# google-research/semivl

Measured on AMD Instinct MI355X. Metric: train images/sec (512^2, ViT-B/16), higher is better.
Workload: dtype f32 (fp32 in / out / accumulate everywhere; the MFMA products as split 16-bit terms with fp32 accumulation: the ViT's linears, in_proj weight gradients and fused attention and the decoder's 3x3 convolutions (tiled: forward, input and weight gradient; dilated: forward, input gradient) on fp16 x 2 ope; 1 GPU; SemiVL step, pascal N=21, vlm-vlg-aspp-s2p4-sk04-ftap-mcvitb, 512x512, bs=16/GPU labeled + 16/GPU unlabeled (BASELINE configs[1]); global_batch=32, parallelism=dp1

## Files before the change

include/semivl_hip.h:

```cpp
#ifndef SEMIVL_HIP_H_
#define SEMIVL_HIP_H_

#include <stddef.h>
#include <stdint.h>

#ifdef __cplusplus
extern "C" {
#endif

typedef void* svl_stream_t;

typedef enum svl_status {
  SVL_OK = 0,
  SVL_ERR_INVALID_ARG = -1,
  SVL_ERR_LAUNCH = -2,
  SVL_ERR_UNSUPPORTED = -3
} svl_status;

int svl_version(void);
int svl_stream_release(svl_stream_t stream);
int svl_stream_prepare(svl_stream_t stream);
int svl_stream_helper(svl_stream_t stream, void** helper);
int svl_shutdown(void);
int svl_num_stream_contexts(void);
int svl_last_error(char* buf, size_t len);
int svl_clock_probe(unsigned long long* out, int n_waves, unsigned long long ticks_100mhz, svl_stream_t stream);

enum {
  SVL_A_KCONTIG = 0,
  SVL_A_MCONTIG = 1,
  SVL_A_CONV = 2,
  SVL_A_PATCH = 3
};
enum {
  SVL_B_KCONTIG = 0,
  SVL_B_NCONTIG = 1,
  SVL_B_CONVW = 2,
  SVL_B_NC_GELU = 3,
  SVL_B_NC_LN = 4,
  SVL_B_PATCHT = 5
};
enum {
  SVL_ACT_NONE = 0,
  SVL_ACT_GELU = 1,
  SVL_ACT_RELU = 2,
  SVL_ACT_MUL_DGELU = 3,
  SVL_ACT_MUL_DRELU = 4
};
enum {
  SVL_OUT_STRIDED = 0,
  SVL_OUT_CONVT2X = 1,
  SVL_OUT_PATCH = 2
};

typedef struct svl_operand {
  const float* ptr;
  int64_t ld;
  int64_t bs_outer;
  int64_t bs_inner;
} svl_operand;

typedef struct svl_conv_geom {
  int H, W;
  int Ho, Wo;
  int stride;
  int C1, C2;
  int rep;
  int KH, KW, dil, pad, sign;
  const float* src2;
  int64_t ld2;
  int patch;
} svl_conv_geom;

typedef struct svl_gemm_desc {
  int a_mode, b_mode;
  int M, N, K;
  int batch;
  int batch_inner;
  int ksplit;
  svl_operand A, B;
  svl_conv_geom conv;
  float* C;
  int out_mode;
  int64_t ldc_m, ldc_n, c_bs_outer, c_bs_inner;
  int ct_H, ct_W, ct_Cout;
  float alpha;
  const float* bias;
  int bias_mod;
  int act;
  float* preact;
  const float* resid;
  int64_t ldr_m, ldr_n, r_bs_outer, r_bs_inner;
  int accumulate;
  const void* conv_w_planes;
  void* emu_ws;
  const float* b_stats;
  const float* b_gamma;
  const float* b_beta;
  const unsigned* a_amax;
  const unsigned* b_amax;
} svl_gemm_desc;

int svl_gemm_f32(const svl_gemm_desc* d, svl_stream_t stream);

int svl_set_gemm_emulation(int mode);
int svl_get_gemm_emulation(void);
int svl_set_conv_tiled(int on);
int svl_last_gemm_path(void);
int64_t svl_absmax_launches(void);

typedef struct svl_pgemm_desc {
  const void* A;
  const void* B;
  int64_t a_rows, b_rows;
  int m_off, M, N, K;
  float* C;
  int64_t ldc;
  void* planes_out;
  int64_t p_rows;
  const float* bias;
  int act;
  float* preact;
  const float* resid;
  int64_t ldr;
  int accumulate;
  int fmt;
  int p_fmt;
  const int32_t* a_sexp;
  const int32_t* b_sexp;
  const float* a_rnorm;
  const float* b_bound;
  int32_t* p_sexp;
} svl_pgemm_desc;
int64_t svl_planes_rows(int64_t rows);
int64_t svl_planes_bytes(int64_t rows, int K);
int svl_split_planes_bf16x3(const float* x, int64_t ld, int64_t k_stride, int64_t rows, int K, void* planes,
                            int64_t planes_rows, int64_t row_off, svl_stream_t stream);
int64_t svl_planes_bytes_fmt(int64_t rows, int K, int fmt);
int svl_split_planes_f16x2(const float* x, int64_t ld, int64_t k_stride, int64_t rows, int K, void* planes,
                           int64_t planes_rows, int64_t row_off, int32_t* sexp, float* rnorm, unsigned* tensor_amax,
                           svl_stream_t stream);
int svl_gemm_planes_f32(const svl_pgemm_desc* d, svl_stream_t stream);
int svl_conv3x3_wgrad_tiled_groups(int imgs, int H, int W, int Ct, int Co);
int svl_conv3x3_wgrad_tiled(const float* dy, int64_t lddy, int Co, const float* src1, int64_t ld1, int C1,
                            const float* src2, int64_t ld2, int C2, int rep, int imgs, int H, int W, float* slabs,
                            int groups, const float* gn_in, svl_stream_t stream);

int svl_reduce_slabs_f32(float* out, const float* slabs, int nslab, int64_t count, int accumulate,
                         svl_stream_t stream);


int svl_softmax_max_f32(const float* logits, int B, int N, int64_t HW, float* conf, int64_t* label,
                        svl_stream_t stream);

int svl_cutmix_f32(float* out, const float* a, const float* b, const float* box, int B, int C, int64_t HW,
                   svl_stream_t stream);
int svl_cutmix_i64(int64_t* out, const int64_t* a, const int64_t* b, const float* box, int B, int64_t HW,
                   svl_stream_t stream);

typedef struct svl_ce_desc {
  const float* logits;
  int B, N;
  int64_t HW;
  const int64_t* target;
  int use_ignore_t;
  const float* conf;
  const int64_t* ign;
  float conf_thresh;
  int all_pixels;
  const int64_t* mc_target;
  float* partials;
  float* dlogits;
  const float* gscale;
  const float* img_weight;
} svl_ce_desc;
int64_t svl_ce_num_blocks(int B, int N, int64_t HW);
int svl_ce_fused_f32(const svl_ce_desc* d, svl_stream_t stream);
int svl_ce_finalize(const float* partials, int64_t nblocks, double* sums , svl_stream_t stream);

typedef struct svl_ce_up_desc {
  const float* logits;
  int B, N;
  int h, w, H, W;
  int align_corners;
  const int64_t* target;
  int use_ignore_t;
  const float* conf;
  const int64_t* ign;
  float conf_thresh;
  int all_pixels;
  const int64_t* mc_target;
  float* partials;
  float* dlogits;
  const float* gscale;
  const float* img_weight;
} svl_ce_up_desc;
int64_t svl_ce_up_num_blocks(int B, int N, int h, int w, int H, int W, int align_corners);
int svl_ce_up_fused_f32(const svl_ce_up_desc* d, svl_stream_t stream);
int svl_softmax_max_up_f32(const float* logits, int B, int N, int h, int w, int H, int W, int align_corners, float* conf,
                           int64_t* label, svl_stream_t stream);

int svl_semivl_gscale(const int64_t* counts, double numel_u, float lam, const double* factors, const int64_t* mc_counts,
                      float* gscale, svl_stream_t stream);
int svl_inv_count_f32(const int64_t* count, float* out, svl_stream_t stream);
int64_t svl_conf_avg_ws_doubles(int B);
int svl_conf_avg_factor(const float* conf, const int64_t* ign, int B, int64_t HW, double* factor, double* workspace,
                        svl_stream_t stream);
int svl_conf_ratio_f32(const float* conf, const int64_t* ign, int B, int64_t HW, float thresh, float* ratio,
                       double* workspace, svl_stream_t stream);
int svl_semivl_loss(const double* sums, double numel_u, float lam, const double* factors, const int64_t* mc_counts,
                    float* out, svl_stream_t stream);
int svl_softmax_planes_f32(const float* logits, int B, int N, int64_t HW, float* out, svl_stream_t stream);

int svl_target_prob_f32(const float* logits, int B, int N, int64_t HW, const int64_t* target, float* prob,
                        svl_stream_t stream);
int svl_target_prob_up_f32(const float* logits, int B, int N, int h, int w, int H, int W, int align_corners,
                           const int64_t* target, float* prob, svl_stream_t stream);
int64_t svl_ohem_ws_bytes(int64_t n);
int svl_ohem_threshold_f32(const float* prob, int64_t n, int64_t k, const int64_t* num_valid, int64_t min_kept,
                           float thresh, void* ws, float* threshold, svl_stream_t stream);
int svl_ohem_relabel_i64(const int64_t* target, const float* prob, int64_t n, const float* threshold, int64_t* out,
                         int64_t* count, svl_stream_t stream);

int svl_count_valid_i64(const int64_t* map, int64_t n, int64_t* count, svl_stream_t stream);

int svl_maskclip_labels(const float* dense, int B, int N, int h, int w, int H, int W, float scale,
                        float thresh, const int64_t* ign, int64_t* out, svl_stream_t stream);

int svl_concept_max_f32(const float* pred, int B, int NC, int64_t HW, const int* concept_offsets, int N,
                        float* out, svl_stream_t stream);

int svl_iou_hist_i64(const int64_t* pred, const int64_t* target, int64_t n, int K, int ignore_index, int64_t* hist,
                     svl_stream_t stream);


int svl_layernorm_fwd(const float* x, const float* gamma, const float* beta, float eps, int64_t rows, int C,
                      float* y, float* stats, svl_stream_t stream);
int svl_layernorm_fwd_planes(const float* x, const float* gamma, const float* beta, float eps, int64_t rows, int C,
                             float* y, float* stats, void* planes, int64_t planes_rows, svl_stream_t stream);
int svl_layernorm_fwd_planes_f16x2(const float* x, const float* gamma, const float* beta, float eps, int64_t rows, int C,
                                   float* y, float* stats, void* planes, int64_t planes_rows, int32_t* sexp, float* rnorm,
                                   svl_stream_t stream);
int svl_layernorm_fwd_pack_f16x2(const float* x, const float* gamma, const float* beta, float eps, int64_t rows, int C,
                                 float* y, float* stats, void* planes, int64_t planes_rows, int64_t row_off, int32_t* sexp,
                                 float* rnorm, int row_rnorm, unsigned* tensor_amax, svl_stream_t stream);
int svl_layernorm_bwd_pack_f16x2(const float* dy, const float* x, const float* stats, const float* gamma, int64_t rows, int C,
                                 const float* dx_add, float* dx, void* planes, int64_t planes_rows, int64_t row_off,
                                 int32_t* sexp, float* rnorm, unsigned* tensor_amax, svl_stream_t stream);
int svl_layernorm_bwd_parts(int64_t rows);
int svl_layernorm_bwd(const float* dy, const float* x, const float* stats, const float* gamma, int64_t rows,
                      int C, const float* dx_add, float* dx, float* dgamma_part, float* dbeta_part,
                      svl_stream_t stream);
int svl_softmax_rows_fwd(float* s, int64_t rows, int cols, int64_t ld, float scale, svl_stream_t stream);
int svl_softmax_rows_bwd(float* dp, const float* p, int64_t rows, int cols, int64_t ld, float scale,
                         svl_stream_t stream);

int svl_l2norm_fwd(const float* x, int64_t rows, int C, float eps, float* y, float* inv_norm, svl_stream_t stream);
int svl_l2norm_bwd(const float* dy, const float* y, const float* inv_norm, int64_t rows, int C, float* dx,
                   svl_stream_t stream);

int64_t svl_colsum_ws_floats(int64_t rows, int C);
int svl_colsum_f32(const float* x, int64_t rows, int C, int64_t ld, float* out, int accumulate, float* ws,
                   svl_stream_t stream);

int svl_eltwise_f32(int mode, const float* a, const float* b, float* out, int64_t n, svl_stream_t stream);
int svl_chanmask_f32(const float* x, const float* mask, float scale, int64_t rows, int rows_per_img, int C,
                     float* out, svl_stream_t stream);
int svl_fill_f32(float* p, float v, int64_t n, svl_stream_t stream);
int svl_bernoulli_f32(float* p, int64_t n, float keep_prob, uint64_t seed, uint64_t offset, svl_stream_t stream);
int svl_affine_planes_f32(const float* x, int64_t planes, int C, int64_t HW, const float* k4, float* y, svl_stream_t stream);
int svl_copy2d_f32(const float* src, int64_t sgrp, int64_t src_go, int64_t src_ld, float* dst, int64_t dgrp,
                   int64_t dst_go, int64_t dst_ld, int64_t rows, int C, int accumulate, svl_stream_t stream);
int svl_permute4_f32(const float* src, float* dst, int64_t n0, int64_t n1, int64_t n2, int64_t n3, int64_t s0, int64_t s1,
                     int64_t s2, int64_t s3, svl_stream_t stream);
int svl_bound2_f32(const float* rnorm, int64_t rows, const float* bias, int64_t nbias, float* out2, svl_stream_t stream);
int svl_permute_rows_f32(const float* src, int64_t outer, int A, int B, int C, float* dst, svl_stream_t stream);

int svl_groupnorm_fwd(const float* x, int64_t ldx, const float* gamma, const float* beta, float eps, int imgs,
                      int64_t HW, int C, int G, int relu, float* y, int64_t ldy, float* stats, svl_stream_t stream);
int64_t svl_conv3x3_gn_ws_doubles(int imgs, int H, int W, int N);
int svl_conv3x3_gn_f32(const float* src1, int64_t ld1, int C1, const float* src2, int64_t ld2, int C2, int rep,
                       const float* w, int imgs, int H, int W, int N, float* out, int64_t ldo, float eps, double* ws,
                       float* stats, const float* gn_in, const void* w_planes, svl_stream_t stream);
int64_t svl_conv3x3_weight_planes_bytes(int N, int Ct);
int svl_conv3x3_weight_planes(const float* w, int N, int Ct, void* planes, svl_stream_t stream);
int svl_groupnorm_scale_shift(const float* stats, const float* gamma, const float* beta, int imgs, int C, int G, float* scsh,
                              svl_stream_t stream);
int svl_groupnorm_apply(const float* x, int64_t ldx, const float* gamma, const float* beta, int imgs, int64_t HW, int C, int G,
                        int relu, const float* stats, float* y, int64_t ldy, svl_stream_t stream);
int svl_groupnorm_bwd(const float* dy, int64_t lddy, const float* x, int64_t ldx, const float* y, int64_t ldy,
                      const float* stats, const float* gamma, const float* beta, int imgs, int64_t HW, int C, int G,
                      int relu, float* dx, int64_t lddx, float* chan_sums, svl_stream_t stream);
int64_t svl_conv3x3_gnb_ws_doubles(int imgs, int H, int W, int N);
int svl_conv3x3_dgrad_gnb_f32(const float* dy, int64_t lddy, int C1, const float* w, int imgs, int H, int W, int N, float* out,
                              int64_t ldo, int accumulate, const float* gnb_x, const float* gnb_table, const float* gnb_stats,
                              double* ws, float* chan_sums, const void* w_planes, svl_stream_t stream);
int svl_groupnorm_bwd_apply(const float* dy, int64_t lddy, const float* x, int64_t ldx, const float* stats, const float* gamma,
                            const float* beta, int imgs, int64_t HW, int C, int G, int relu, const float* chan_sums, float* dx,
                            int64_t lddx, svl_stream_t stream);


int svl_attention_fwd(const float* qkv, int B, int T, int H, float* out, float* lse, void* out_planes,
                      int64_t planes_rows, svl_stream_t stream);
int svl_attention_bwd(const float* qkv, const float* out, const float* dout, const float* lse, int B, int T, int H,
                      float* dsum_ws, float* dqkv, void* dqkv_planes, int64_t planes_rows, svl_stream_t stream);
int64_t svl_attention_h2_ws_bytes(int B, int T, int H, int backward);
int svl_attention_h2_tr_sets(int on);
int svl_attention_bwd_h2_sets(const float* qkv, const float* out, const float* dout, const float* lse, int B, int T, int H,
                              float* dsum_ws, float* dqkv, const void* sets, int64_t sets_bytes, void* ws, int64_t ws_bytes,
                              svl_stream_t stream);
int svl_attention_fwd_h2(const float* qkv, int B, int T, int H, float* out, float* lse, void* out_planes,
                         int64_t planes_rows, void* ws, int64_t ws_bytes, svl_stream_t stream);
int svl_attention_bwd_h2(const float* qkv, const float* out, const float* dout, const float* lse, int B, int T, int H,
                         float* dsum_ws, float* dqkv, void* dqkv_planes, int64_t planes_rows, void* ws, int64_t ws_bytes,
                         svl_stream_t stream);

typedef struct svl_seqattn_desc {
  int groups, inner, seq, heads;
  int64_t outer_stride, inner_stride, seq_stride;
  const float* qkv;
  float* out;
  float* probs;
  const float* dout;
  float* dqkv;
  float* dscores;
} svl_seqattn_desc;
int svl_seqattn_fwd(const svl_seqattn_desc* d, svl_stream_t stream);
int svl_seqattn_bwd(const svl_seqattn_desc* d, svl_stream_t stream);

int svl_conv_cout1_fwd(const float* x, int64_t ldx, int imgs, int H, int W, int C, int KH, int KW, int dil, int pad,
                       const float* w, const float* bias, const float* gn_in, float* y, svl_stream_t stream);
int svl_conv_cout1_wgrad_blocks(int imgs, int H, int W);
int svl_conv_cout1_wgrad(const float* dy, const float* x, int64_t ldx, int imgs, int H, int W, int C, int dil, int pad,
                         const float* gn_in, float* slabs, svl_stream_t stream);
int svl_tap_gather(const float* T, int imgs, int H, int W, int KH, int KW, int dil, int pad, int sign, float* out,
                   svl_stream_t stream);

int svl_bilinear_nhwc_fwd(const float* x, int64_t ldx, int imgs, int h, int w, int C, int align_corners, int rep,
                          int H, int W, float* y, int64_t ldy, int accumulate, svl_stream_t stream);
int svl_sum_rep_f32(const float* src, int64_t ld, int64_t groups, int rep, int64_t rows, int C, float* out,
                    svl_stream_t stream);
int svl_bilinear_nhwc_bwd(const float* dy, int64_t lddy, int imgs, int h, int w, int C, int align_corners, int rep,
                          int H, int W, float* dx, int64_t lddx, int accumulate, svl_stream_t stream);
int svl_bilinear_planes_fwd(const float* x, int64_t planes, int h, int w, int align_corners, int H, int W, float* y,
                            svl_stream_t stream);
int svl_bilinear_planes_bwd(const float* dy, int64_t planes, int h, int w, int align_corners, int H, int W,
                            float* dx, svl_stream_t stream);
int svl_avgpool_cat_fwd(const float* x, int imgs, int H, int W, int C, int PH, int PW, const float* text, int Ct,
                        int nclass, float* y, svl_stream_t stream);
int svl_avgpool_cat_bwd(const float* dy, int imgs, int H, int W, int C, int PH, int PW, int Ct, float* dx,
                        int accumulate, svl_stream_t stream);
int svl_avgpool_cat_bwd_text(const float* dy, int imgs, int64_t HWp, int C, int Ct, int nclass, float* part, float* dtext,
                             svl_stream_t stream);

int svl_adamw_step(float* p, const float* g, float* m, float* v, const int64_t* seg_off, const float* seg_lr,
                   const float* seg_wd, int nseg, int64_t total, float beta1, float beta2, float eps, int step,
                   float gscale, float* ema, float ema_decay, svl_stream_t stream);
int svl_sgd_step(float* p, const float* g, float* m, const int64_t* seg_off, const float* seg_lr, const float* seg_wd,
                 int nseg, int64_t total, float momentum, float dampening, int nesterov, int step, float gscale,
                 float* ema, float ema_decay, svl_stream_t stream);

int64_t svl_bn_ws_doubles(int64_t rows, int C);
int svl_bn_stats(const float* x, int64_t ldx, int64_t rows, int C, double* sums, double* ws, svl_stream_t stream);
int svl_bn_finalize(const double* sums, double count, float eps, float momentum, float* running_mean, float* running_var,
                    int C, float* mean, float* invstd, svl_stream_t stream);
int svl_bn_eval_invstd(const float* running_var, float eps, int C, float* invstd, svl_stream_t stream);
int svl_bn_apply(const float* x, int64_t ldx, int64_t rows, int C, const float* mean, const float* invstd,
                 const float* gamma, const float* beta, const float* resid, int64_t ldr, int relu, float* y, int64_t ldy,
                 svl_stream_t stream);
int svl_bn_bwd_reduce(const float* dy, int64_t lddy, const float* x, int64_t ldx, const float* y, int64_t ldy,
                      const float* mean, const float* invstd, const float* remask_gamma, const float* remask_beta,
                      int64_t rows, int C, double* sums, double* ws, svl_stream_t stream);
int svl_bn_bwd_apply(const float* dy, int64_t lddy, const float* x, int64_t ldx, const float* y, int64_t ldy,
                     const float* mean, const float* invstd, const float* gamma, const float* remask_beta,
                     const double* sums, double count, int64_t rows, int C, float* dx, int64_t lddx, float* dres,
                     int64_t lddr, svl_stream_t stream);
int svl_maxpool3x3s2_fwd(const float* x, int imgs, int H, int W, int C, float* y, unsigned char* idx,
                         svl_stream_t stream);
int svl_maxpool3x3s2_bwd(const float* dy, const unsigned char* idx, int imgs, int H, int W, int C, float* dx,
                         svl_stream_t stream);

int svl_gap_tokens_fwd(const float* x, int64_t ldx, int imgs, int64_t HW, int C, float* pool, int64_t ldp,
                       svl_stream_t stream);
int svl_gap_tokens_bwd(const float* dpool, int64_t ldp, int imgs, int64_t HW, int C, float* dx, int64_t lddx,
                       int accumulate, svl_stream_t stream);
int svl_bcast_rows_fwd(const float* v, int64_t ldv, int imgs, int64_t HW, int C, float* dst, int64_t ldd, int c_off,
                       svl_stream_t stream);
int svl_bcast_rows_bwd(const float* dy, int64_t lddy, int c_off, int imgs, int64_t HW, int C, float* dv, int64_t ldv,
                       svl_stream_t stream);

int svl_aug_resample_u8(const unsigned char* src, int H, int W, int C, int rh, int rw, int x0, int y0, int OH, int OW,
                        int flip, int mode, int fill, unsigned char* dst, svl_stream_t stream);
int svl_aug_to_float(const unsigned char* src, int npix, const float* mean3, const float* std3, float* dst,
                     svl_stream_t stream);
int svl_aug_mask_i64(const unsigned char* src, int npix, int from, int to, int64_t* dst, svl_stream_t stream);
int svl_aug_photometric_u8(unsigned char* img, int npix, int op, float factor, unsigned long long* scratch,
                           svl_stream_t stream);
int svl_aug_gaussian_blur_u8(const unsigned char* src, int H, int W, float sigma, unsigned char* tmp, unsigned char* dst,
                             svl_stream_t stream);

int svl_lora_merge_f32(const float* W, int64_t ldw, float* Weff, int64_t ldo, int nblk, int rows, int E, int r, float s,
                       const float* const* A, const float* const* B, int64_t ldb, svl_stream_t stream);
int64_t svl_lora_wgrad_ws_floats(int rows, int E, int r);
int svl_lora_wgrad_f32(const float* dW, int64_t lddw, const float* A, const float* B, int64_t ldb, int rows, int E, int r,
                       float s, float* dB, int accumulate_b, float* dA, int accumulate_a, float* ws, svl_stream_t stream);

int svl_prompt_rows_fwd_f32(const float* src, float* dst, const float* emb, const float* mask, float scale, int B, int T,
                            int P, int E, svl_stream_t stream);
int svl_prompt_rows_bwd_f32(float* dx, float* dx_out, float* demb, const float* mask, float scale, int accumulate, int B,
                            int T, int P, int E, svl_stream_t stream);

int svl_droppath_fwd_f32(const float* branch, const float* resid, const float* mask, float scale, float* out, int B, int T,
                         int E, svl_stream_t stream);
int svl_droppath_bwd_f32(const float* dout, const float* mask, float scale, float* dbranch, int B, int T, int E,
                         svl_stream_t stream);

#ifdef __cplusplus
}
#endif
#endif
```

semivl_amd/csrc/attention.hip:

```cpp
#include "attn_shared.h"
#include "attn_h2.h"

namespace {

__device__ __forceinline__ void tile_gload(float4 (&rg)[4], const float* base, long ld, int row0, int T, int tid) {
#pragma unroll
  for (int p = 0; p < 4; ++p) {
    const int f = tid + 256 * p;
    const int row = row0 + (f >> 4), c4 = (f & 15) << 2;
    rg[p] = (row < T) ? *reinterpret_cast<const float4*>(base + (long)row * ld + c4) : make_float4(0.f, 0.f, 0.f, 0.f);
  }
}
template <int LD>
__device__ __forceinline__ void tile_sstore(float* S, const float4 (&rg)[4], int tid, float mul) {
#pragma unroll
  for (int p = 0; p < 4; ++p) {
    const int f = tid + 256 * p;
    const int row = f >> 4, c = (f & 15) << 2;
    *reinterpret_cast<float4*>(S + row * LD + c) = make_float4(rg[p].x * mul, rg[p].y * mul, rg[p].z * mul, rg[p].w * mul);
  }
}

__device__ __forceinline__ float4 ld4(const float* p) { return *reinterpret_cast<const float4*>(p); }
__device__ __forceinline__ void row_gload32(float (&r)[32], const float* p, float mul) {
// ... 443 lines not shown
__global__ __launch_bounds__(256) void attn_bwd_dkv_rows_kernel(const AttnP p, int row0) {
  __shared__ __attribute__((aligned(16))) float kv[D];
  __shared__ __attribute__((aligned(16))) float vv[D];
  __shared__ float wp[ROWS_MAX_T];
  __shared__ float wd[ROWS_MAX_T];
  __shared__ float red[256];
  const int tid = threadIdx.x, sub = tid & 15, grp = tid >> 4;
  const int z = blockIdx.y, b = z / p.H, h = z - b * p.H, kj = row0 + blockIdx.x;
  const float* head = p.qkv + (long)b * p.T * p.ld + h * D;
  const float* dhead = p.dout + (long)b * p.T * p.E + h * D;
  if (tid < D) {
    kv[tid] = head[p.E + (long)kj * p.ld + tid] * p.scale;
    vv[tid] = head[2 * p.E + (long)kj * p.ld + tid];
  }
  __syncthreads();
  for (int i0 = 0; i0 < p.T; i0 += 16) {
    const int i = i0 + grp, ic = min(i, p.T - 1);
    const float sc = dot16(kv, head + (long)ic * p.ld, sub), dp = dot16(vv, dhead + (long)ic * p.E, sub);
    if (i < p.T && sub == 0) {
      const float pv = expf(sc - p.lse[(long)z * p.T + i]);
      wp[i] = pv;
      wd[i] = pv * (dp - p.dsum[(long)z * p.T + i]);
    }
  }
  __syncthreads();
  const float dv = weighted_rowsum(wp, dhead, p.E, p.T, red, tid);
  const float dk = weighted_rowsum(wd, head, p.ld, p.T, red, tid);
  if (tid < D) {
    float* row = p.dqkv + ((long)b * p.T + kj) * p.ld + h * D;
    row[p.E + tid] = dk * p.scale;
    row[2 * p.E + tid] = dv;
  }
}

__host__ inline int rows_split(int T, int* nb, int BQ = 128) {
  const int full = T / BQ, r = T - full * BQ;
  const bool use = r > 0 && r <= 4 && full > 0 && T <= ROWS_MAX_T;
  *nb = use ? full : (T + BQ - 1) / BQ;
  return use ? r : 0;
}

int check(const float* qkv, int B, int T, int H, const char* who) {
  SVL_CHECK_ARG(qkv && B > 0 && T > 0 && H > 0 && (long)B * H <= 65535, "%s: bad args", who);
  SVL_CHECK_ARG(((uintptr_t)qkv & 15) == 0, "%s: qkv must be 16-byte aligned", who);
  return SVL_OK;
}

int no_planes(const void* planes, const char* who) {
  if (!planes) return SVL_OK;
  svl_set_error("%s: planes outputs were retired with the bf16 x 6 attention kernels (pass null; pack the fp32 result)", who);
  return SVL_ERR_UNSUPPORTED;
}

}

extern "C" int svl_attention_fwd(const float* qkv, int B, int T, int H, float* out, float* lse, void* out_planes,
                                 int64_t planes_rows, svl_stream_t stream) {
  int rc = check(qkv, B, T, H, "svl_attention_fwd");
  if (rc) return rc;
  SVL_CHECK_ARG(out, "svl_attention_fwd: out missing");
  (void)planes_rows;
  rc = no_planes(out_planes, "svl_attention_fwd");
  if (rc) return rc;
  AttnP p;
  memset(&p, 0, sizeof(p));
  p.qkv = qkv; p.out = out; p.lse = lse; p.B = B; p.T = T; p.H = H; p.E = (long)H * D; p.ld = 3 * p.E; p.scale = 0.125f;
  hipStream_t st = (hipStream_t)stream;
  int nb = 0;
  const int r = rows_split(T, &nb, 128);
  if (r > 0) {
    hipStream_t aux = nullptr;
    rc = svl_fork(st, &aux);
    if (rc) return rc;
    hipLaunchKernelGGL(attn_fwd_rows_kernel, dim3(r, B * H), dim3(256), 0, aux, p, nb * 128);
    SVL_LAUNCH_CHECK("svl_attention_fwd/rows");
  }
  hipLaunchKernelGGL(attn_fwd_kernel, dim3(nb, B * H), dim3(256), 0, st, p);
  SVL_LAUNCH_CHECK("svl_attention_fwd");
  return r > 0 ? svl_join(st) : SVL_OK;
}

extern "C" int svl_attention_bwd(const float* qkv, const float* out, const float* dout, const float* lse, int B, int T,
                                 int H, float* dsum_ws, float* dqkv, void* dq_planes, int64_t planes_rows,
                                 svl_stream_t stream) {
  int rc = check(qkv, B, T, H, "svl_attention_bwd");
  if (rc) return rc;
  SVL_CHECK_ARG(out && dout && lse && dsum_ws && dqkv, "svl_attention_bwd: null args");
  (void)planes_rows;
  rc = no_planes(dq_planes, "svl_attention_bwd");
  if (rc) return rc;
  hipStream_t st = (hipStream_t)stream;
  AttnP p;
  memset(&p, 0, sizeof(p));
  p.qkv = qkv; p.dout = dout; p.lse = const_cast<float*>(lse); p.dsum = dsum_ws; p.dqkv = dqkv;
  p.B = B; p.T = T; p.H = H; p.E = (long)H * D; p.ld = 3 * p.E; p.scale = 0.125f;
  const long groups = (long)B * T * H;
  hipLaunchKernelGGL(attn_dsum_kernel, dim3((unsigned)((groups * 16 + 255) / 256)), dim3(256), 0, st, dout, out, dsum_ws,
                     B, T, H, p.E);
  SVL_LAUNCH_CHECK("svl_attention_bwd/dsum");
  int nb = 0;
  const int r = rows_split(T, &nb, 128);
  if (r > 0) {
    hipStream_t aux = nullptr;
    rc = svl_fork(st, &aux);
    if (rc) return rc;
    hipLaunchKernelGGL(attn_bwd_dkv_rows_kernel, dim3(r, B * H), dim3(256), 0, aux, p, nb * 128);
    SVL_LAUNCH_CHECK("svl_attention_bwd/dkv_rows");
    hipLaunchKernelGGL(attn_bwd_dq_rows_kernel, dim3(r, B * H), dim3(256), 0, aux, p, nb * 128);
    SVL_LAUNCH_CHECK("svl_attention_bwd/dq_rows");
  }
  hipLaunchKernelGGL(attn_bwd_dkv_kernel, dim3(nb, B * H), dim3(256), 0, st, p);
  SVL_LAUNCH_CHECK("svl_attention_bwd/dkv");
  hipLaunchKernelGGL(attn_bwd_dq_kernel, dim3(nb, B * H), dim3(256), 0, st, p);
  SVL_LAUNCH_CHECK("svl_attention_bwd/dq");
  return r > 0 ? svl_join(st) : SVL_OK;
}

extern "C" int64_t svl_attention_h2_ws_bytes(int B, int T, int H, int backward) {
  if (B <= 0 || T <= 0 || H <= 0 || backward < 0 || backward > 2) return 0;
  return svl_attn_h2::ws_bytes(B, T, H, backward, svl_attn_h2::tr_sets(-1));
}

extern "C" int svl_attention_h2_tr_sets(int on) { return svl_attn_h2::tr_sets(on); }

extern "C" int svl_attention_fwd_h2(const float* qkv, int B, int T, int H, float* out, float* lse, void* out_planes,
                                    int64_t planes_rows, void* ws, int64_t ws_bytes, svl_stream_t stream) {
  int rc = check(qkv, B, T, H, "svl_attention_fwd_h2");
  if (rc) return rc;
  SVL_CHECK_ARG(out, "svl_attention_fwd_h2: out missing");
  (void)planes_rows;
  rc = no_planes(out_planes, "svl_attention_fwd_h2");
  if (rc) return rc;
  AttnP p;
  memset(&p, 0, sizeof(p));
  p.qkv = qkv; p.out = out; p.lse = lse; p.B = B; p.T = T; p.H = H; p.E = (long)H * D; p.ld = 3 * p.E; p.scale = 0.125f;
  hipStream_t st = (hipStream_t)stream;
  int nb = 0;
  const int r = rows_split(T, &nb, FQ);
  const int tr = svl_attn_h2::tr_sets(-1);
  rc = svl_attn_h2::fwd_pack(p, ws, ws_bytes, tr, st);
  if (rc) return rc;
  if (r > 0) {
    hipStream_t aux = nullptr;
    rc = svl_fork(st, &aux);
    if (rc) return rc;
    rc = svl_attn_h2::fwd_tail(p, nb * FQ, ws, tr, aux);
    if (rc) return rc;
  }
  rc = svl_attn_h2::fwd(p, nb, ws, ws_bytes, tr, st);
  if (rc) return rc;
  return r > 0 ? svl_join(st) : SVL_OK;
}

namespace {
int bwd_h2(const char* who, const float* qkv, const float* out, const float* dout, const float* lse, int B, int T, int H,
           float* dsum_ws, float* dqkv, void* dq_planes, const void* sets, int64_t sets_bytes, void* ws, int64_t ws_bytes,
           svl_stream_t stream) {
  int rc = check(qkv, B, T, H, who);
  if (rc) return rc;
  SVL_CHECK_ARG(out && dout && lse && dsum_ws && dqkv, "%s: null args", who);
  rc = no_planes(dq_planes, who);
  if (rc) return rc;
  hipStream_t st = (hipStream_t)stream;
  AttnP p;
  memset(&p, 0, sizeof(p));
  p.qkv = qkv; p.dout = dout; p.lse = const_cast<float*>(lse); p.dsum = dsum_ws; p.dqkv = dqkv;
  p.B = B; p.T = T; p.H = H; p.E = (long)H * D; p.ld = 3 * p.E; p.scale = 0.125f;
  const int tr = svl_attn_h2::tr_sets(-1);
  rc = svl_attn_h2::bwd_prepare(p, out, dsum_ws, ws, ws_bytes, sets, sets_bytes, tr, st);
  if (rc) return rc;
  int nb = 0;
  const int r = rows_split(T, &nb, FQ);
  if (r > 0) {
    hipStream_t aux = nullptr;
    rc = svl_fork(st, &aux);
    if (rc) return rc;
    rc = svl_attn_h2::bwd_tail(p, nb * FQ, ws, sets, tr, aux);
    if (rc) return rc;
  }
  rc = svl_attn_h2::bwd_main(p, nb, ws, sets, tr, st);
  if (rc) return rc;
  return r > 0 ? svl_join(st) : SVL_OK;
}
}

extern "C" int svl_attention_bwd_h2(const float* qkv, const float* out, const float* dout, const float* lse, int B, int T,
                                    int H, float* dsum_ws, float* dqkv, void* dq_planes, int64_t planes_rows, void* ws,
                                    int64_t ws_bytes, svl_stream_t stream) {
  (void)planes_rows;
  return bwd_h2("svl_attention_bwd_h2", qkv, out, dout, lse, B, T, H, dsum_ws, dqkv, dq_planes, nullptr, 0, ws, ws_bytes, stream);
}

extern "C" int svl_attention_bwd_h2_sets(const float* qkv, const float* out, const float* dout, const float* lse, int B, int T,
                                         int H, float* dsum_ws, float* dqkv, const void* sets, int64_t sets_bytes, void* ws,
                                         int64_t ws_bytes, svl_stream_t stream) {
  SVL_CHECK_ARG(sets, "svl_attention_bwd_h2_sets: sets missing");
  return bwd_h2("svl_attention_bwd_h2_sets", qkv, out, dout, lse, B, T, H, dsum_ws, dqkv, nullptr, sets, sets_bytes, ws, ws_bytes,
                stream);
}
```

semivl_amd/csrc/attn_h2.h:

```cpp
#pragma once
#include "attn_shared.h"

namespace svl_attn_h2 {

int tr_sets(int on);
long ws_bytes(int B, int T, int H, int mode, int tr);
int fwd(const AttnP& p, int nb, void* ws, long wsb, int tr, hipStream_t st);
int bwd_prepare(const AttnP& p, const float* out, float* dsum_ws, void* ws, long wsb, const void* sets, long setsb, int tr,
                hipStream_t st);
int bwd_main(const AttnP& p, int nb, void* ws, const void* sets, int tr, hipStream_t st);
int fwd_pack(const AttnP& p, void* ws, long wsb, int tr, hipStream_t st);
int fwd_tail(const AttnP& p, int row0, void* ws, int tr, hipStream_t aux);
int bwd_tail(const AttnP& p, int row0, void* ws, const void* sets, int tr, hipStream_t aux);

}
```

semivl_amd/csrc/attn_h2.hip:

```cpp
#include "attn_h2.h"
#include <atomic>

namespace {

typedef _Float16 f16x8 __attribute__((ext_vector_type(8)));
typedef _Float16 f16x2 __attribute__((ext_vector_type(2)));

struct H2W {
  const char *q_rm, *k_rm, *v_rm, *do_rm, *q_tr, *k_tr, *v_tr, *do_tr;
  const int* exps;
  const float* nrm;
  const float* ld;
  int Tp;
};

__device__ __forceinline__ void glds16(const char* base_, unsigned lane_off, unsigned lds_dst_) {
  const unsigned long long bv = (unsigned long long)base_;
  const unsigned b_hi = (unsigned)__builtin_amdgcn_readfirstlane((int)(bv >> 32));
  const unsigned b_lo = (unsigned)__builtin_amdgcn_readfirstlane((int)(unsigned)bv);
  const char* base = (const char*)(((unsigned long long)b_hi << 32) | (unsigned long long)b_lo);
  const unsigned lds_dst = __builtin_amdgcn_readfirstlane(lds_dst_);
  unsigned keep;
  asm volatile("s_mov_b32 %0, m0\n\ts_mov_b32 m0, %3\n\ts_nop 3\n\tglobal_load_lds_dwordx4 %2, %1\n\ts_mov_b32 m0, %0"
               : "=&s"(keep)
// ... 57 lines not shown
  h[0] = __builtin_bit_cast(f16x8, w0);
  h[1] = __builtin_bit_cast(f16x8, w1);
}
__device__ __forceinline__ void frag2(f16x8 (&a)[2], const char* chunk0) {
  a[0] = *reinterpret_cast<const f16x8*>(chunk0);
  a[1] = *reinterpret_cast<const f16x8*>(chunk0 + 1024);
}
typedef short s16x4 __attribute__((__vector_size__(4 * sizeof(short))));
typedef short s16x8 __attribute__((__vector_size__(8 * sizeof(short))));
struct TrLane {
  unsigned rm[2];
  unsigned tr[2];
};
__device__ __forceinline__ TrLane tr_lane(int lane) {
  const int hh = lane >> 5, r = lane & 31, g = (lane >> 4) & 1, q = (lane >> 2) & 3, p = lane & 3;
  TrLane t;
  t.rm[0] = (unsigned)(hh * 32 + (r ^ (4 * hh))) * 16u;
  t.rm[1] = (unsigned)(hh * 32 + (r ^ (4 * hh + 8))) * 16u;
  t.tr[0] = (unsigned)(g * 2048 + ((p & 1) * 32 + ((4 * hh + q) ^ (4 * (p & 1) + 8 * g))) * 16 + (p >> 1) * 8);
  t.tr[1] = t.tr[0] ^ 128u;
  return t;
}
typedef __attribute__((address_space(3))) char lchar;
__device__ __forceinline__ const lchar* tr_base(const char* img, unsigned off) {
  const lchar* b = (const lchar*)(img + off);
  asm("" : "+v"(b));
  return b;
}
__device__ __forceinline__ f16x8 tr_read8(const lchar* a0, const lchar* a1) {
  typedef __attribute__((address_space(3))) s16x4 lds4;
  const s16x4 lo = __builtin_amdgcn_ds_read_tr16_b64_v4i16((lds4*)a0);
  const s16x4 hi = __builtin_amdgcn_ds_read_tr16_b64_v4i16((lds4*)a1);
  return __builtin_bit_cast(f16x8, (s16x8)__builtin_shufflevector(lo, hi, 0, 1, 2, 3, 4, 5, 6, 7));
}
__device__ __forceinline__ void frag2(f16x8 (&a)[2], const lchar* chunk0) {
  typedef __attribute__((address_space(3))) f16x8 lds8;
  a[0] = *reinterpret_cast<const lds8*>(chunk0);
  a[1] = *reinterpret_cast<const lds8*>(chunk0 + 1024);
}
__device__ __forceinline__ void frag2_tr(f16x8 (&a)[2], const lchar* t0, const lchar* t1, int kgl, int rbd) {
  const int o = kgl * 256 + rbd * 4096;
  a[0] = tr_read8(t0 + o, t1 + o);
  a[1] = tr_read8(t0 + o + 1024, t1 + o + 1024);
}
__device__ __forceinline__ int ds_exp(float nrm_do, float nrm_v) {
  const float bt = 2.f * nrm_do * nrm_v;
  int g = bt > 0.f ? __builtin_amdgcn_frexp_expf(bt) : 0;
  return g < -100 ? -100 : (g > 100 ? 100 : g);
}

struct PackP {
  const float* src[4];
  long ld[4];
  char* rm[4];
  char* tr[4];
  int which[4];
  int* exps;
  float* nrm;
  const int* exps_in;
  const float* nrm_in;
  int B, T, H, Tp;
};

__global__ __launch_bounds__(256) void attn_pack_kernel(const PackP p) {
  __shared__ __attribute__((aligned(16))) float tile[64 * LDP];
  __shared__ float red[4];
  const int tid = threadIdx.x, z = blockIdx.x, w = p.which[blockIdx.y];
  const int b = z / p.H, h = z - b * p.H;
  const long ld = p.ld[w];
  const float* src = p.src[w] + (long)b * p.T * ld + h * D;
  const int r16 = tid >> 4, c4 = (tid & 15) << 2;
  const int nrb = p.Tp >> 5;
  char* rm = p.rm[w] ? p.rm[w] + (long)z * nrb * 8192 : nullptr;
  char* tr = p.tr[w] ? p.tr[w] + (long)z * p.Tp * 256 : nullptr;
  const int lane = tid & 63, cq = tid >> 6, hh = lane >> 5, r = lane & 31;
  auto rows = [&](int r0, float4 (&v)[4]) __attribute__((always_inline)) {
#pragma unroll
    for (int i = 0; i < 4; ++i) {
      const int row = r0 + 16 * i + r16;
      v[i] = row < p.T ? *reinterpret_cast<const float4*>(src + (long)row * ld + c4) : make_float4(0.f, 0.f, 0.f, 0.f);
    }
  };
  auto amax4 = [](const float4& a) { return fmaxf(fmaxf(fabsf(a.x), fabsf(a.y)), fmaxf(fabsf(a.z), fabsf(a.w))); };
  auto exp_of = [](float mx) {
    const int e = mx > 0.f ? __builtin_amdgcn_frexp_expf(mx) - 15 : 0;
    return e < -100 ? -100 : (e > 100 ? 100 : e);
  };
  float4 v[4];
  rows(0, v);
  float m0 = fmaxf(fmaxf(amax4(v[0]), amax4(v[1])), fmaxf(amax4(v[2]), amax4(v[3])));
  m0 = block_max_256(m0, red);
  int e = exp_of(m0) + 3;
  float mx = 0.f, nr = 0.f;
  for (int attempt = 0; attempt < 2; ++attempt) {
    if (attempt) rows(0, v);
    mx = 0.f;
    nr = 0.f;
    for (int r0 = 0; r0 < p.Tp; r0 += 64) {
#pragma unroll
      for (int i = 0; i < 4; ++i) {
        mx = fmaxf(mx, amax4(v[i]));
        float ss = v[i].x * v[i].x + v[i].y * v[i].y + v[i].z * v[i].z + v[i].w * v[i].w;
#pragma unroll
        for (int o = 8; o > 0; o >>= 1) ss += __shfl_xor(ss, o, 64);
        nr = fmaxf(nr, ss);
        *reinterpret_cast<float4*>(&tile[(16 * i + r16) * LDP + c4]) =
            make_float4(__builtin_amdgcn_ldexpf(v[i].x, -e), __builtin_amdgcn_ldexpf(v[i].y, -e),
                        __builtin_amdgcn_ldexpf(v[i].z, -e), __builtin_amdgcn_ldexpf(v[i].w, -e));
      }
      if (r0 + 64 < p.Tp) rows(r0 + 64, v);
      __syncthreads();
#pragma unroll
      for (int half = 0; half < 2; ++half) {
        const int rb = (r0 >> 5) + half;
        const float* th = tile + half * 32 * LDP;
        if (rm) {
          const float* t = th + r * LDP + 16 * cq + 4 * hh;
          const float4 u = *reinterpret_cast<const float4*>(t), q = *reinterpret_cast<const float4*>(t + 8);
          const float x[8] = {u.x, u.y, u.z, u.w, q.x, q.y, q.z, q.w};
          f16x8 hp[2];
          split2x8<true>(x, hp);
          char* c = rm + (long)((rb * 4 + cq) * 2) * 1024 + lane * 16;
          *reinterpret_cast<f16x8*>(c) = hp[0];
          *reinterpret_cast<f16x8*>(c + 1024) = hp[1];
        }
        if (tr) {
          const int kgl = cq >> 1, rbd = cq & 1;
          const float* t = th + (16 * kgl + 4 * hh) * LDP + 32 * rbd + r;
          float x[8];
#pragma unroll
          for (int j = 0; j < 8; ++j) x[j] = t[((j & 3) + 8 * (j >> 2)) * LDP];
          f16x8 hp[2];
          split2x8<true>(x, hp);
          char* c = tr + (long)(((2 * rb + kgl) * 2 + rbd) * 2) * 1024 + lane * 16;
          *reinterpret_cast<f16x8*>(c) = hp[0];
          *reinterpret_cast<f16x8*>(c + 1024) = hp[1];
        }
      }
      __syncthreads();
    }
    mx = block_max_256(mx, red);
    const int ex = exp_of(mx);
    if (ex <= e && ex >= e - 3) break;
    e = ex;
  }
  nr = block_max_256(nr, red);
  if (tid == 0) {
    p.exps[z * 4 + w] = e;
    p.nrm[z * 4 + w] = sqrtf(nr);
  }
  if (p.exps_in && tid < 3) {
    p.exps[z * 4 + tid] = p.exps_in[z * 4 + tid];
    p.nrm[z * 4 + tid] = p.nrm_in[z * 4 + tid];
  }
}

__global__ __launch_bounds__(256) void attn_ld_kernel(const float* __restrict__ dout, const float* __restrict__ out,
                                                      const float* __restrict__ lse, const float* __restrict__ nrm,
                                                      float* __restrict__ dsum, float* __restrict__ ld, int B, int T, int H,
                                                      int Tp, long E) {
  const long total = (long)B * H * Tp;
  const long g = ((long)blockIdx.x * 256 + threadIdx.x) >> 4;
  const int sub = threadIdx.x & 15;
  if (g >= total) return;
  const int z = (int)(g / Tp), t = (int)(g - (long)z * Tp);
  const int b = z / H, h = z - b * H;
  float s = 0.f;
  if (t < T) {
    const long off = ((long)b * T + t) * E + h * D + sub * 4;
    const float4 a = *reinterpret_cast<const float4*>(dout + off), c = *reinterpret_cast<const float4*>(out + off);
    s = a.x * c.x + a.y * c.y + a.z * c.z + a.w * c.w;
  }
#pragma unroll
  for (int o = 8; o > 0; o >>= 1) s += __shfl_xor(s, o, 64);
  if (sub == 0) {
    float2 v = make_float2(-INFINITY, 0.f);
    if (t < T) {
      dsum[(long)z * T + t] = s;
      v.x = -lse[(long)z * T + t] * LOG2E;
      v.y = __builtin_amdgcn_ldexpf(s, 14 - ds_exp(nrm[z * 4 + 3], nrm[z * 4 + 2]));
    }
    *reinterpret_cast<float2*>(ld + ((long)z * Tp + t) * 2) = v;
  }
}

constexpr int STG_F = 32 * 1024;

template <int V>
__global__ __launch_bounds__(512) void attn_fwd_h2_kernel(const AttnP p, const H2W w) {
  constexpr bool MIX = (V & 1) != 0;
  constexpr bool RM = (V & 4) != 0;
  extern __shared__ __attribute__((aligned(1024))) char sm[];
  const int tid = threadIdx.x, lane = tid & 63, l31 = lane & 31, hi = lane >> 5;
  const int wave = __builtin_amdgcn_readfirstlane(tid >> 6);
  int rb_, z;
  attn_block(p, FQ, rb_, z);
  const int b = z / p.H, h = z - b * p.H;
  const int q0 = rb_ * FQ + wave * 32;
  const int qi = q0 + l31;
  const bool wave_active = q0 < p.T;
  const int off = wave >= 4 ? 1 : 0;
  const int nkt = w.Tp >> 6;
  const long rmz = (long)(w.Tp >> 5) * 8192, trz = (long)w.Tp * 256;
  const char* ksrc = w.k_rm + z * rmz;
  const char* vsrc = RM ? w.v_rm + z * rmz : w.v_tr + z * trz;
  const unsigned lane16 = lane * 16;
  const TrLane tl = tr_lane(lane);
  const unsigned lane_v = RM ? (wave & 1 ? tl.rm[1] : tl.rm[0]) : lane16;
  const unsigned sm_base = (unsigned)(uintptr_t)(__attribute__((address_space(3))) char*)sm;
  f16x8 qf[2][4];
  {
    const char* qs = w.q_rm + z * rmz + (long)(min(q0, w.Tp - 32) >> 5) * 8192 + lane16;
#pragma unroll
    for (int kg = 0; kg < 4; ++kg)
#pragma unroll
      for (int pl = 0; pl < 2; ++pl) qf[pl][kg] = *reinterpret_cast<const f16x8*>(qs + (kg * 2 + pl) * 1024);
  }
  const int eq = w.exps[z * 4], ek = w.exps[z * 4 + 1], ev = w.exps[z * 4 + 2];
  const float c = __builtin_amdgcn_ldexpf(LOG2E, eq + ek - 3);
  auto issue_part = [&](int tile, int part, int stage) __attribute__((always_inline)) {
    const int tc = min(tile, nkt - 1);
    const char* s = (part ? vsrc : ksrc) + (long)tc * 16384 + wave * 2048;
    const unsigned dst = sm_base + stage * STG_F + part * 16384 + wave * 2048;
    const unsigned lo = part ? lane_v : lane16;
    glds16(s, lo, dst);
    glds16(s + 1024, lo, dst + 1024);
  };
  f32x16 o0, o1, s0, s1;
#pragma unroll
  for (int r = 0; r < 16; ++r) { o0[r] = 0.f; o1[r] = 0.f; s0[r] = 0.f; s1[r] = 0.f; }
  float m2s = -INFINITY, l = 0.f;
  issue_part(0, 0, 0);
  issue_part(0, 1, 0);
  issue_part(1, 0, 1);
  issue_part(1, 1, 1);
  wait_vm<6>();
  interval_barrier();

  const bool short_last = p.T - (nkt - 1) * 64 <= 32;
  auto phase1 = [&](int kt, auto last_c) __attribute__((always_inline)) {
    constexpr bool LAST = decltype(last_c)::value;
    const char* Ks = sm + (kt % 3) * STG_F + lane16;
#pragma unroll
    for (int r = 0; r < 16; ++r) { s0[r] = 0.f; s1[r] = 0.f; }
    if (LAST && short_last) {
#pragma unroll
      for (int kg = 0; kg < 4; ++kg) {
        f16x8 a0[2], bq[2] = {qf[0][kg], qf[1][kg]};
        frag2(a0, Ks + (kg * 2) * 1024);
        s0 = mfma_h(a0[1], bq[0], s0);
        s0 = mfma_h(a0[0], bq[1], s0);
        s0 = mfma_h(a0[0], bq[0], s0);
      }
      return;
    }
#pragma unroll
    for (int kg = 0; kg < 4; ++kg) {
      f16x8 a0[2], a1[2], bq[2] = {qf[0][kg], qf[1][kg]};
      frag2(a0, Ks + (kg * 2) * 1024);
      frag2(a1, Ks + ((4 + kg) * 2) * 1024);
      H2_PAIR(s0, a0, s1, a1, bq)
    }
  };
  auto phase2 = [&](int kt, auto last_c) __attribute__((always_inline)) {
    constexpr bool LAST = decltype(last_c)::value;
    const char* Vt = sm + (kt % 3) * STG_F + 16384 + lane16;
    const lchar* Vt0 = RM ? tr_base(sm + (kt % 3) * STG_F + 16384, tl.tr[0]) : nullptr;
    const lchar* Vt1 = RM ? tr_base(sm + (kt % 3) * STG_F + 16384, tl.tr[1]) : nullptr;
    if (LAST) {
      const int j0 = kt * 64;
#pragma unroll
      for (int r = 0; r < 16; ++r) {
        const int key = j0 + crow(r, hi);
        if (key >= p.T) s0[r] = -INFINITY;
        if (key + 32 >= p.T) s1[r] = -INFINITY;
      }
    }
    auto max3c = [](float a, float b, float c) { return __builtin_fmaxf(__builtin_fmaxf(a, b), c); };
    float ma = max3c(s0[0], s0[1], s0[2]), mb = max3c(s1[0], s1[1], s1[2]);
#pragma unroll
    for (int r = 3; r < 15; r += 2) {
      ma = max3c(ma, s0[r], s0[r + 1]);
      mb = max3c(mb, s1[r], s1[r + 1]);
    }
    float mloc = max3c(ma, mb, fmaxf(s0[15], s1[15]));
    mloc = fmaxf(mloc, __shfl_xor(mloc, 32, 64));
    const float mloc2 = mloc * c;
    const bool raise = mloc2 > m2s + (7.f + RESCALE_LOG2);
    if (__any(raise)) {
      const float mnew = raise ? mloc2 - 7.f : m2s;
      const float alpha = __builtin_amdgcn_exp2f(m2s - mnew);
      l *= alpha;
#pragma unroll
      for (int r = 0; r < 16; ++r) { o0[r] *= alpha; o1[r] *= alpha; }
      m2s = mnew;
    }
    float sum0 = 0.f, sum1 = 0.f;
    const int ntp = (LAST && short_last) ? 2 : 4;
#pragma unroll
    for (int tp = 0; tp < 4; ++tp) {
      if (tp >= ntp) break;
      float x[8];
#pragma unroll
      for (int j = 0; j < 8; ++j) {
        x[j] = __builtin_amdgcn_exp2f(fmaf((tp < 2) ? s0[8 * (tp & 1) + j] : s1[8 * (tp & 1) + j], c, -m2s));
        if (j & 1) sum1 += x[j]; else sum0 += x[j];
// ... 721 lines not shown
      H2_2(dv0, pa[t], o0, dv1, pa[t], o1)
      __builtin_amdgcn_sched_barrier(0);
      frag2(q0f, Qt + lane16 + ((t * 2) * 2) * 1024);
      frag2(q1f, Qt + lane16 + ((t * 2 + 1) * 2) * 1024);
      H2_2(dk0, sa2[t], q0f, dk1, sa2[t], q1f)
      __builtin_amdgcn_sched_barrier(0);
    }
  }
  __shared__ float cmb[TAILW][32][16];
  if (hi == 0 && wave != 0) {
    float* c_ = cmb[wave][l31];
#pragma unroll
    for (int r = 0; r < 4; ++r) { c_[r] = dk0[r]; c_[4 + r] = dk1[r]; c_[8 + r] = dv0[r]; c_[12 + r] = dv1[r]; }
  }
  __syncthreads();
  if (wave != 0) return;
  if (hi == 0) {
#pragma unroll
    for (int w_ = 1; w_ < TAILW; ++w_) {
      const float* c_ = cmb[w_][l31];
#pragma unroll
      for (int r = 0; r < 4; ++r) { dk0[r] += c_[r]; dk1[r] += c_[4 + r]; dv0[r] += c_[8 + r]; dv1[r] += c_[12 + r]; }
    }
  }
  const float fk = __builtin_amdgcn_ldexpf(1.f, gs - 14 + eq - 3);
  const float fv = __builtin_amdgcn_ldexpf(1.f, edo - 14);
#pragma unroll
  for (int r = 0; r < 16; ++r) { dk0[r] *= fk; dk1[r] *= fk; dv0[r] *= fv; dv1[r] *= fv; }
#pragma unroll
  for (int r = 0; r < 16; ++r) {
    const int key = k0 + crow(r, hi);
    if (key < p.T) {
      float* row = p.dqkv + ((long)b * p.T + key) * p.ld + h * D;
      row[p.E + l31] = dk0[r];
      row[p.E + 32 + l31] = dk1[r];
      row[2 * p.E + l31] = dv0[r];
      row[2 * p.E + 32 + l31] = dv1[r];
    }
  }
}

struct Layout {
  long set;
  long exps, nrm, ld, total;
  int Tp;
};
Layout layout(int B, int T, int H, int mode, int tr) {
  Layout l;
  l.Tp = (T + 63) / 64 * 64;
  l.set = (long)B * H * l.Tp * 256;
  const long nset = mode == 0 ? 3 : mode == 2 ? 1 : tr ? 7 : 4;
  l.exps = nset * l.set;
  l.nrm = l.exps + (((long)B * H * 16 + 1023) & ~1023L);
  l.ld = l.nrm + (((long)B * H * 16 + 1023) & ~1023L);
  l.total = l.ld + (mode ? (((long)B * H * l.Tp * 8 + 1023) & ~1023L) + 1024 : 0);
  return l;
}

std::atomic<int> g_tr{-1};

template <typename K>
int set_lds(K kernel, std::atomic<uint64_t>& mask, int bytes) {
  int dev = 0;
  (void)hipGetDevice(&dev);
  const uint64_t bit = 1ull << (dev & 63);
  if (mask.load(std::memory_order_acquire) & bit) return SVL_OK;
  SVL_HIP_CHECK(hipFuncSetAttribute(reinterpret_cast<const void*>(kernel), hipFuncAttributeMaxDynamicSharedMemorySize, bytes));
  mask.fetch_or(bit, std::memory_order_acq_rel);
  return SVL_OK;
}

H2W views(const Layout& l, char* ws, int mode, int tr, const char* sets = nullptr) {
  H2W w;
  memset(&w, 0, sizeof(w));
  w.Tp = l.Tp;
  if (mode == 2) {
    w.q_rm = sets;
    w.k_rm = sets + l.set;
    w.v_rm = sets + 2 * l.set;
    w.do_rm = ws;
  } else {
    w.q_rm = ws;
    w.k_rm = ws + l.set;
    if (mode == 1) {
      w.v_rm = ws + 2 * l.set;
      w.do_rm = ws + 3 * l.set;
      if (tr) {
        w.q_tr = ws + 4 * l.set;
        w.k_tr = ws + 5 * l.set;
        w.do_tr = ws + 6 * l.set;
      }
    } else if (tr) {
      w.v_tr = ws + 2 * l.set;
    } else {
      w.v_rm = ws + 2 * l.set;
    }
  }
  w.exps = reinterpret_cast<const int*>(ws + l.exps);
  w.nrm = reinterpret_cast<const float*>(ws + l.nrm);
  w.ld = reinterpret_cast<const float*>(ws + l.ld);
  return w;
}

int check_ws(const AttnP& p, const void* ws, long wsb, int mode, int tr, const char* who) {
  const Layout l = layout(p.B, p.T, p.H, mode, tr);
  SVL_CHECK_ARG(ws && ((uintptr_t)ws & 1023) == 0 && wsb >= l.total, "%s: workspace of %ld bytes (1 KiB aligned) needed, got %ld",
                who, l.total, wsb);
  return SVL_OK;
}

}

namespace svl_attn_h2 {

int tr_sets(int on) {
  int cur = g_tr.load(std::memory_order_acquire);
  if (cur < 0) {
    const char* e = getenv("SVL_ATTN_TR_SETS");
    int expect = -1;
    g_tr.compare_exchange_strong(expect, e && *e && *e != '0' ? 1 : 0);
    cur = g_tr.load(std::memory_order_acquire);
  }
  if (on >= 0) g_tr.store(on ? 1 : 0, std::memory_order_release);
  return cur;
}

long ws_bytes(int B, int T, int H, int mode, int tr) { return layout(B, T, H, mode, tr).total; }

int fwd_pack(const AttnP& p, void* ws_, long wsb, int tr, hipStream_t st) {
  int rc = check_ws(p, ws_, wsb, 0, tr, "svl_attention_fwd_h2");
  if (rc) return rc;
  const Layout l = layout(p.B, p.T, p.H, 0, tr);
  char* ws = static_cast<char*>(ws_);
  const H2W w = views(l, ws, 0, tr);
  PackP q;
  memset(&q, 0, sizeof(q));
  for (int i = 0; i < 3; ++i) {
    q.src[i] = p.qkv + i * p.E;
    q.ld[i] = p.ld;
    q.which[i] = i;
  }
  q.rm[0] = const_cast<char*>(w.q_rm);
  q.rm[1] = const_cast<char*>(w.k_rm);
  q.rm[2] = const_cast<char*>(w.v_rm);
  q.tr[2] = const_cast<char*>(w.v_tr);
  q.exps = const_cast<int*>(w.exps);
  q.nrm = const_cast<float*>(w.nrm);
  q.B = p.B; q.T = p.T; q.H = p.H; q.Tp = l.Tp;
  hipLaunchKernelGGL(attn_pack_kernel, dim3(p.B * p.H, 3), dim3(256), 0, st, q);
  SVL_LAUNCH_CHECK("svl_attention_fwd_h2/pack");
  return SVL_OK;
}

#define SVL_LAUNCH_V(KERN, VV, LDS)                                   \
    rc = set_lds(KERN<VV>, mask, LDS);                                  \
    if (rc) return rc;                                                  \
    hipLaunchKernelGGL(KERN<VV>, grid, dim3(512), LDS, st, p, w);

int fwd(const AttnP& p, int nb, void* ws_, long wsb, int tr, hipStream_t st) {
  (void)wsb;
  if (nb <= 0) return SVL_OK;
  const Layout l = layout(p.B, p.T, p.H, 0, tr);
  const H2W w = views(l, static_cast<char*>(ws_), 0, tr);
  int rc = SVL_OK;
  const dim3 grid(nb * p.B * p.H);
  if (tr) {
    static std::atomic<uint64_t> mask;
    SVL_LAUNCH_V(attn_fwd_h2_kernel, 3, 3 * STG_F)
  } else {
    static std::atomic<uint64_t> mask;
    SVL_LAUNCH_V(attn_fwd_h2_kernel, 7, 3 * STG_F)
  }
  SVL_LAUNCH_CHECK("svl_attention_fwd_h2");
  return SVL_OK;
}

int bwd_prepare(const AttnP& p, const float* out, float* dsum_ws, void* ws_, long wsb, const void* sets, long setsb, int tr,
                hipStream_t st) {
  const int mode = sets ? 2 : 1;
  int rc = check_ws(p, ws_, wsb, mode, tr, "svl_attention_bwd_h2");
  if (rc) return rc;
  if (sets) {
    SVL_CHECK_ARG(!tr, "svl_attention_bwd_h2_sets: kept sets are row-major sets only (the tr switch is on)");
    rc = check_ws(p, sets, setsb, 0, 0, "svl_attention_bwd_h2_sets (sets)");
    if (rc) return rc;
  }
  const Layout l = layout(p.B, p.T, p.H, mode, tr);
  char* ws = static_cast<char*>(ws_);
  const H2W w = views(l, ws, mode, tr, static_cast<const char*>(sets));
  PackP q;
  memset(&q, 0, sizeof(q));
  for (int i = 0; i < 3; ++i) {
    q.src[i] = p.qkv + i * p.E;
    q.ld[i] = p.ld;
  }
  q.src[3] = p.dout;
  q.ld[3] = p.E;
  q.rm[3] = const_cast<char*>(w.do_rm);
  q.tr[3] = const_cast<char*>(w.do_tr);
  if (sets) {
    const Layout lf = layout(p.B, p.T, p.H, 0, 0);
    q.which[0] = 3;
    q.exps_in = reinterpret_cast<const int*>(static_cast<const char*>(sets) + lf.exps);
    q.nrm_in = reinterpret_cast<const float*>(static_cast<const char*>(sets) + lf.nrm);
  } else {
    for (int i = 0; i < 4; ++i) q.which[i] = i;
    q.rm[0] = const_cast<char*>(w.q_rm);
    q.rm[1] = const_cast<char*>(w.k_rm);
    q.rm[2] = const_cast<char*>(w.v_rm);
    q.tr[0] = const_cast<char*>(w.q_tr);
    q.tr[1] = const_cast<char*>(w.k_tr);
  }
  q.exps = const_cast<int*>(w.exps);
  q.nrm = const_cast<float*>(w.nrm);
  q.B = p.B; q.T = p.T; q.H = p.H; q.Tp = l.Tp;
  hipLaunchKernelGGL(attn_pack_kernel, dim3(p.B * p.H, sets ? 1 : 4), dim3(256), 0, st, q);
  SVL_LAUNCH_CHECK("svl_attention_bwd_h2/pack");
  const long groups = (long)p.B * p.H * l.Tp;
  hipLaunchKernelGGL(attn_ld_kernel, dim3((unsigned)((groups * 16 + 255) / 256)), dim3(256), 0, st, p.dout, out, p.lse, w.nrm,
                     dsum_ws, const_cast<float*>(w.ld), p.B, p.T, p.H, l.Tp, p.E);
  SVL_LAUNCH_CHECK("svl_attention_bwd_h2/dsum");
  return SVL_OK;
}

int fwd_tail(const AttnP& p, int row0, void* ws_, int tr, hipStream_t aux) {
  const Layout l = layout(p.B, p.T, p.H, 0, tr);
  const H2W w = views(l, static_cast<char*>(ws_), 0, tr);
  const dim3 grid(p.B * p.H, (p.T - row0 + 31) / 32);
  if (tr) hipLaunchKernelGGL((attn_fwd_tail_h2_kernel<true, false>), grid, dim3(64 * TAILW), 0, aux, p, w, row0);
  else hipLaunchKernelGGL((attn_fwd_tail_h2_kernel<true, true>), grid, dim3(64 * TAILW), 0, aux, p, w, row0);
  SVL_LAUNCH_CHECK("svl_attention_fwd_h2/tail");
  return SVL_OK;
}

int bwd_tail(const AttnP& p, int row0, void* ws_, const void* sets, int tr, hipStream_t aux) {
  const int mode = sets ? 2 : 1;
  const Layout l = layout(p.B, p.T, p.H, mode, tr);
  const H2W w = views(l, static_cast<char*>(ws_), mode, tr, static_cast<const char*>(sets));
  const dim3 grid(p.B * p.H, (p.T - row0 + 31) / 32);
  if (tr) {
    hipLaunchKernelGGL((attn_dkv_tail_h2_kernel<true, false>), grid, dim3(64 * TAILW), 0, aux, p, w, row0);
    hipLaunchKernelGGL((attn_dq_tail_h2_kernel<true, false>), grid, dim3(64 * TAILW), 0, aux, p, w, row0);
  } else {
    hipLaunchKernelGGL((attn_dkv_tail_h2_kernel<true, true>), grid, dim3(64 * TAILW), 0, aux, p, w, row0);
    hipLaunchKernelGGL((attn_dq_tail_h2_kernel<true, true>), grid, dim3(64 * TAILW), 0, aux, p, w, row0);
  }
  SVL_LAUNCH_CHECK("svl_attention_bwd_h2/tail");
  return SVL_OK;
}

int bwd_main(const AttnP& p, int nb, void* ws_, const void* sets, int tr, hipStream_t st) {
  if (nb <= 0) return SVL_OK;
  const int mode = sets ? 2 : 1;
  const Layout l = layout(p.B, p.T, p.H, mode, tr);
  const H2W w = views(l, static_cast<char*>(ws_), mode, tr, static_cast<const char*>(sets));
  int rc = SVL_OK;
  const dim3 grid(nb * p.B * p.H);
  if (tr) {
    static std::atomic<uint64_t> mask;
    SVL_LAUNCH_V(attn_dkv_h2_kernel, 3, 3 * STG_K)
  } else {
    static std::atomic<uint64_t> mask;
    SVL_LAUNCH_V(attn_dkv_h2_kernel, 7, 3 * STG_K_RM)
  }
  SVL_LAUNCH_CHECK("svl_attention_bwd_h2/dkv");
  if (tr) {
    static std::atomic<uint64_t> mask;
    SVL_LAUNCH_V(attn_dq_h2_kernel, 3, 3 * STG_Q)
  } else {
    static std::atomic<uint64_t> mask;
    SVL_LAUNCH_V(attn_dq_h2_kernel, 7, 3 * STG_Q_RM)
  }
  SVL_LAUNCH_CHECK("svl_attention_bwd_h2/dq");
  return SVL_OK;
}

}
```

semivl_amd/csrc/gemm_planes.hip:

```cpp
#include "gemm_planes_impl.h"

int svl_planes_launch_h2(const PlanesP& p, hipStream_t st);

namespace {

__global__ __launch_bounds__(256) void pack_planes_kernel(const float* __restrict__ x, long ld, long ks, long rows, int K,
                                                          char* __restrict__ planes, long p_ks, long row_off) {
  const long nkg = K >> 4;
  const long rows32 = (rows + 31) & ~31L;
  const long total = rows32 * nkg * 2;
  const bool fast = ks == 1 && (ld & 3) == 0 && ((reinterpret_cast<uintptr_t>(x) & 15) == 0);
  for (long i = (long)blockIdx.x * blockDim.x + threadIdx.x; i < total; i += (long)gridDim.x * blockDim.x) {
    const int r31 = (int)(i & 31), h = (int)((i >> 5) & 1);
    const long t = i >> 6;
    const long kg = t % nkg, rb = t / nkg;
    const long r = rb * 32 + r31;
    float v[8];
    if (r < rows) {
      const float* src = x + r * ld + (kg * 16 + 4 * h) * ks;
      if (fast) {
        const float4 f0 = *reinterpret_cast<const float4*>(src), f1 = *reinterpret_cast<const float4*>(src + 8);
        v[0] = f0.x; v[1] = f0.y; v[2] = f0.z; v[3] = f0.w; v[4] = f1.x; v[5] = f1.y; v[6] = f1.z; v[7] = f1.w;
      } else {
#pragma unroll
        for (int q = 0; q < 4; ++q) { v[q] = src[q * ks]; v[4 + q] = src[(8 + q) * ks]; }
      }
    } else {
#pragma unroll
      for (int q = 0; q < 8; ++q) v[q] = 0.f;
    }
    bf16x8 h0, h1, h2;
    split3x8(v, h0, h1, h2);
    const long rr = row_off + r;
    char* q = planes + kg * p_ks + (rr >> 5) * (3 * CH) + (h * 32 + (int)(rr & 31)) * 16;
    *reinterpret_cast<bf16x8*>(q) = h0;
    *reinterpret_cast<bf16x8*>(q + CH) = h1;
    *reinterpret_cast<bf16x8*>(q + 2 * CH) = h2;
  }
}

}


extern "C" int64_t svl_planes_rows(int64_t rows) { return rows <= 0 ? -1 : (rows + 255) / 256 * 256; }

extern "C" int64_t svl_planes_bytes(int64_t rows, int K) {
  if (rows <= 0 || K <= 0 || (K & 15)) return -1;
  return (int64_t)(K >> 4) * svl_planes_rows(rows) * 96;
}

extern "C" int64_t svl_planes_bytes_fmt(int64_t rows, int K, int fmt) {
  if (rows <= 0 || K <= 0 || (K & 15) || fmt < 0 || fmt > 1) return -1;
  return (int64_t)(K >> 4) * svl_planes_rows(rows) * (fmt == 1 ? 64 : 96);
}

extern "C" int svl_split_planes_bf16x3(const float* x, int64_t ld, int64_t k_stride, int64_t rows, int K, void* planes,
                                       int64_t planes_rows, int64_t row_off, svl_stream_t stream) {
  SVL_CHECK_ARG(x && planes && rows > 0 && K > 0 && (K & 15) == 0 && k_stride >= 1 && planes_rows >= row_off + rows &&
                    row_off >= 0 && (planes_rows & 255) == 0 && (row_off & 31) == 0,
                "svl_split_planes_bf16x3: bad args (K %% 16, planes_rows %% 256, row_off %% 32 must be 0)");
  const long total = ((rows + 31) & ~31L) * (K >> 4) * 2;
  long grid = (total + 255) / 256;
  if (grid > 256 * 64) grid = 256 * 64;
  hipLaunchKernelGGL(pack_planes_kernel, dim3((unsigned)grid), dim3(256), 0, (hipStream_t)stream, x, (long)ld,
                     (long)k_stride, (long)rows, K, (char*)planes, (long)planes_rows * 96, (long)row_off);
  SVL_LAUNCH_CHECK("svl_split_planes_bf16x3");
  return SVL_OK;
}

extern "C" int svl_gemm_planes_f32(const svl_pgemm_desc* d, svl_stream_t stream) {
  SVL_CHECK_ARG(d, "svl_gemm_planes_f32: null desc");
  SVL_CHECK_ARG(d->A && d->B && d->M > 0 && d->N > 0 && d->K > 0 && (d->K & 15) == 0 && d->m_off >= 0 &&
                    (d->m_off & 31) == 0 && (d->a_rows & 255) == 0 && (d->b_rows & 255) == 0 &&
                    d->a_rows >= d->m_off + d->M && d->b_rows >= d->N,
                "svl_gemm_planes_f32: bad operands (K %% 16 == 0, m_off %% 32 == 0, plane buffers padded to 256 rows)");
  SVL_CHECK_ARG(d->C || d->planes_out, "svl_gemm_planes_f32: no output");
  SVL_CHECK_ARG(!d->planes_out || ((d->N & 15) == 0 && (d->p_rows & 255) == 0 && d->p_rows >= d->m_off + d->M),
                "svl_gemm_planes_f32: planes_out needs N %% 16 == 0 and p_rows (%% 256 == 0) >= rows");
  SVL_CHECK_ARG(d->act >= SVL_ACT_NONE && d->act <= SVL_ACT_MUL_DRELU, "svl_gemm_planes_f32: bad act");
  SVL_CHECK_ARG(!(d->act == SVL_ACT_MUL_DGELU || d->act == SVL_ACT_MUL_DRELU) || d->resid,
                "svl_gemm_planes_f32: MUL_D* needs the saved pre-activation in resid");
  SVL_CHECK_ARG(!d->accumulate || d->C, "svl_gemm_planes_f32: accumulate needs C");
  SVL_CHECK_ARG((d->fmt == 0 || d->fmt == 1) && (d->p_fmt == 0 || d->p_fmt == 1), "svl_gemm_planes_f32: fmt / p_fmt must be 0 (bf16 x 3) or 1 (fp16 x 2)");
  SVL_CHECK_ARG(!(d->planes_out && d->p_fmt == 1) || (d->fmt == 1 && d->a_rnorm && d->b_bound && d->p_sexp && !d->resid) ||
                    (d->fmt == 1 && d->a_rnorm && d->b_bound && d->p_sexp && (d->act == SVL_ACT_MUL_DGELU || d->act == SVL_ACT_MUL_DRELU)),
                "svl_gemm_planes_f32: an fp16 x 2 planes output needs fp16 x 2 operands, a_rnorm, b_bound, p_sexp and no residual add "
                "(its row scales come from the bound |A_m| max|B_n| + max|bias|)");
  SVL_CHECK_ARG(d->a_rows - d->m_off >= (int64_t)(d->M + 255) / 256 * 256 || (d->m_off % 256) == 0,
                "svl_gemm_planes_f32: A plane buffer too short for the last row band");
  PlanesP p;
  const long mo = d->m_off;
  const int np = d->fmt == 1 ? 2 : 3, pnp = d->p_fmt == 1 ? 2 : 3;
  p.A = (const char*)d->A + (mo >> 5) * (np * CH);
  p.B = (const char*)d->B;
  p.a_ks = d->a_rows * 32 * np; p.b_ks = d->b_rows * 32 * np;
  p.a_se = d->a_sexp ? d->a_sexp + mo : nullptr; p.b_se = d->b_sexp;
  p.a_rn = d->a_rnorm ? d->a_rnorm + mo : nullptr; p.b_bd = d->b_bound;
  p.p_se = d->p_sexp ? d->p_sexp + mo : nullptr; p.p_np = pnp;
  p.epi_fast = 1;
  p.b_rb = (int)(d->b_rows / 32);
  p.M = d->M; p.N = d->N; p.K = d->K;
  p.C = d->C ? d->C + mo * d->ldc : nullptr; p.ldc = d->ldc;
  p.P = d->planes_out ? (char*)d->planes_out + (mo >> 5) * (pnp * CH) : nullptr; p.p_ks = d->p_rows * 32 * pnp;
  p.bias = d->bias; p.act = d->act;
  p.preact = d->preact ? d->preact + mo * d->ldc : nullptr;
  p.resid = d->resid ? d->resid + mo * d->ldr : nullptr; p.ldr = d->ldr;
  p.accumulate = d->accumulate;
  return np == 2 ? svl_planes_launch_h2(p, (hipStream_t)stream) : launch<3>(p, (hipStream_t)stream);
}
```

semivl_amd/csrc/gemm_planes_impl.h:

```cpp
#pragma once
#include "svl_common.h"
#include "planes_split_h2.h"
#include <atomic>
#include <type_traits>

struct PlanesP {
  const char* A;
  const char* B;
  long a_ks, b_ks;
  const int* a_se;
  const int* b_se;
  const float* a_rn;
  const float* b_bd;
  int* p_se;
  int p_np;
  int epi_fast;
  int b_rb;
  int M, N, K;
  float* C;
  long ldc;
  char* P;
  long p_ks;
  const float* bias;
  int act;
  float* preact;
  const float* resid;
  long ldr;
  int accumulate;
  int tiles_n, full_m, tail_rows;
  int rcnt[8], fstart[8];
  int panel;
#ifdef SVL_X6P_TIMING
  unsigned long long* dbg;
#endif
};
#ifdef SVL_X6P_TIMING
#define X6P_STAMP(slot)                                                                      \
  do {                                                                                       \
    if (p.dbg && lane == 0 && (wave & 3) == 0) {                                             \
      p.dbg[((long)blockIdx.x * 2 + (wave >> 2)) * 8 + (slot)] = wall_clock64();            \
      p.dbg[((long)blockIdx.x * 2 + (wave >> 2)) * 8 + 4 + (slot)] = clock64();             \
    }                                                                                        \
  } while (0)
#else
#define X6P_STAMP(slot) do {} while (0)
#endif

namespace {

typedef __bf16 bf16x8 __attribute__((ext_vector_type(8)));
typedef int i32x4 __attribute__((ext_vector_type(4)));
typedef unsigned int u32x4 __attribute__((ext_vector_type(4)));

constexpr int BM = 256;
constexpr int CH = 1024;
constexpr int NSTAGE = 3;

template <int I, int N_, typename F>
__device__ __forceinline__ void static_for(F&& f) {
  if constexpr (I < N_) {
    f(std::integral_constant<int, I>{});
    static_for<I + 1, N_>(f);
  }
}

template <int NP> struct FragOf;
template <> struct FragOf<3> { typedef bf16x8 T; };
template <> struct FragOf<2> { typedef f16x8 T; };
template <int NP>
__device__ __forceinline__ f32x16 mfma16(const typename FragOf<NP>::T& x, const typename FragOf<NP>::T& y, const f32x16& c) {
  if constexpr (NP == 3) return __builtin_amdgcn_mfma_f32_32x32x16_bf16(x, y, c, 0, 0, 0);
  else return __builtin_amdgcn_mfma_f32_32x32x16_f16(x, y, c, 0, 0, 0);
}


__device__ __forceinline__ void glds16(const char* base_, unsigned lane_off, unsigned lds_dst_) {
  const unsigned long long bv = (unsigned long long)base_;
  const unsigned b_hi = (unsigned)__builtin_amdgcn_readfirstlane((int)(bv >> 32));
  const unsigned b_lo = (unsigned)__builtin_amdgcn_readfirstlane((int)(unsigned)bv);
  const char* base = (const char*)(((unsigned long long)b_hi << 32) | (unsigned long long)b_lo);
  const unsigned lds_dst = __builtin_amdgcn_readfirstlane(lds_dst_);
  unsigned keep;
  asm volatile("s_mov_b32 %0, m0\n\ts_mov_b32 m0, %3\n\ts_nop 3\n\tglobal_load_lds_dwordx4 %2, %1\n\ts_mov_b32 m0, %0"
               : "=&s"(keep)
               : "s"(base), "v"(lane_off), "s"(lds_dst)
               : "memory");
}

template <int N_>
__device__ __forceinline__ void wait_vm() {
  static_assert(N_ >= 0 && N_ < 64, "vmcnt");
  asm volatile("s_waitcnt vmcnt(%0)" ::"n"(N_) : "memory");
}

__device__ __forceinline__ void split3x8(const float (&x)[8], bf16x8& h0, bf16x8& h1, bf16x8& h2) {
#pragma unroll
  for (int j = 0; j < 8; ++j) {
    float v = x[j];
    h0[j] = (__bf16)v;
    v -= (float)h0[j];
    h1[j] = (__bf16)v;
    v -= (float)h1[j];
    h2[j] = (__bf16)v;
  }
}


struct TileRef { int m0, rows, tn; };
__device__ __forceinline__ TileRef tile_of_block(const PlanesP& p) {
  TileRef t;
  const int lin = (int)blockIdx.x, x = lin & 7, idx = lin >> 3;
  const int rc = p.rcnt[x];
  if (idx < rc) {
    t.m0 = p.full_m * BM;
    t.rows = p.tail_rows;
    t.tn = idx * 8 + x;
  } else {
    const int f = p.fstart[x] + idx - rc;
    const int gsz = p.full_m * p.panel;
    const int cg = f / gsz, r = f - cg * gsz;
    const int w = min(p.panel, p.tiles_n - cg * p.panel);
    const int tm = r / w;
    t.tn = cg * p.panel + (r - tm * w);
    t.m0 = tm * BM;
    t.rows = BM;
  }
  return t;
}

enum { EPI_LIGHT = 0, EPI_GELU = 1, EPI_DGELU = 2 };

template <int NP, int TM, int TN, int EPI>
__device__ __forceinline__ void x6p_epilogue(const PlanesP& p, f32x16 (&acc)[TM][TN], int m0, int mvalid, int wm, int nw,
                                             char* wl, int lane) {
  const int l31 = lane & 31, hi = lane >> 5;
  constexpr int WC = TN * 32;
  constexpr int RS = WC * 4 + 16;
  constexpr int LPR = WC / 4;
  static_assert((32 * LPR) % 64 == 0, "readback steps must be whole wave instructions");
  const bool vec = (p.ldc % 4 == 0) && (reinterpret_cast<uintptr_t>(p.C) % 16 == 0) &&
                   (reinterpret_cast<uintptr_t>(p.preact) % 16 == 0);
  const bool rvec = p.resid && (p.ldr % 4 == 0) && (reinterpret_cast<uintptr_t>(p.resid) % 16 == 0);

  auto store_rows = [&](float* dst, const f32x16 (&o)[TN], int mloc, bool accumulate) __attribute__((always_inline)) {
    static_for<0, TN>([&](auto J) {
      constexpr int j = decltype(J)::value;
      static_for<0, 4>([&](auto G) {
        constexpr int g = decltype(G)::value;
        f32x4 q = {o[j][4 * g], o[j][4 * g + 1], o[j][4 * g + 2], o[j][4 * g + 3]};
        *reinterpret_cast<f32x4*>(wl + l31 * RS + (j * 32 + 8 * g + 4 * hi) * 4) = q;
      });
    });
#pragma unroll
    for (int it = 0; it < 32 * LPR / 64; ++it) {
      const int idx = it * 64 + lane, row = idx / LPR, rc4 = (idx - row * LPR) * 4;
      const f32x4 q = *reinterpret_cast<const f32x4*>(wl + row * RS + rc4 * 4);
      const int n = nw + rc4;
      if (mloc + row < mvalid && n < p.N) {
        float* d = dst + (long)(m0 + mloc + row) * p.ldc + n;
        if (vec && n + 4 <= p.N) {
          f32x4 v = q;
          if (accumulate) v += *reinterpret_cast<const f32x4*>(d);
          *reinterpret_cast<f32x4*>(d) = v;
        } else {
#pragma unroll
          for (int e = 0; e < 4; ++e)
            if (n + e < p.N) d[e] = accumulate ? d[e] + q[e] : q[e];
        }
      }
    }
  };

  static_for<0, TM>([&](auto I) {
    constexpr int i = decltype(I)::value;
    const int mloc = (wm * TM + i) * 32;
    if (mloc < mvalid) {
      const int m = m0 + mloc + l31;
      const bool mok = mloc + l31 < mvalid;
      if constexpr (NP == 2) {
        const int ea = p.a_se ? p.a_se[m] : 0;
        static_for<0, TN>([&](auto J) {
          constexpr int j = decltype(J)::value;
          static_for<0, 4>([&](auto G) {
            constexpr int g = decltype(G)::value;
            const int n = nw + j * 32 + 8 * g + 4 * hi;
            i32x4 eb = {0, 0, 0, 0};
            if (p.b_se && n < p.N) eb = *reinterpret_cast<const i32x4*>(p.b_se + n);
#pragma unroll
            for (int e = 0; e < 4; ++e) acc[i][j][4 * g + e] = __builtin_amdgcn_ldexpf(acc[i][j][4 * g + e], ea + eb[e]);
          });
        });
      }
      if (p.bias) {
        static_for<0, TN>([&](auto J) {
          constexpr int j = decltype(J)::value;
          static_for<0, 4>([&](auto G) {
            constexpr int g = decltype(G)::value;
            const int n = nw + j * 32 + 8 * g + 4 * hi;
#pragma unroll
            for (int e = 0; e < 4; ++e) acc[i][j][4 * g + e] += n + e < p.N ? p.bias[n + e] : 0.f;
          });
        });
      }
      if (p.preact) store_rows(p.preact, acc[i], mloc, false);
      static_for<0, TN>([&](auto J) {
        constexpr int j = decltype(J)::value;
        static_for<0, 4>([&](auto G) {
          constexpr int g = decltype(G)::value;
          const int n = nw + j * 32 + 8 * g + 4 * hi;
          float rv[4] = {0.f, 0.f, 0.f, 0.f};
          if (p.resid && mok && n < p.N) {
            const float* rp = p.resid + (long)m * p.ldr + n;
            if (rvec && n + 4 <= p.N) {
              const f32x4 q = *reinterpret_cast<const f32x4*>(rp);
              rv[0] = q[0]; rv[1] = q[1]; rv[2] = q[2]; rv[3] = q[3];
            } else {
#pragma unroll
              for (int e = 0; e < 4; ++e) rv[e] = n + e < p.N ? rp[e] : 0.f;
            }
          }
#pragma unroll
          for (int e = 0; e < 4; ++e) {
            float v = acc[i][j][4 * g + e];
            if constexpr (EPI == EPI_GELU) v = gelu_erf(v) + rv[e];
            else if constexpr (EPI == EPI_DGELU) v *= gelu_erf_grad(rv[e]);
            else {
              if (p.act == SVL_ACT_RELU) v = fmaxf(v, 0.f);
              if (p.act == SVL_ACT_MUL_DRELU) v = rv[e] > 0.f ? v : 0.f;
              else v += rv[e];
            }
            acc[i][j][4 * g + e] = v;
          }
        });
      });
      if (p.C) store_rows(p.C, acc[i], mloc, p.accumulate != 0);
      if (p.P) {
        int eo = 0;
        if (p.p_np == 2) {
          float bound = p.a_rn[m] * p.b_bd[0] + p.b_bd[1];
          if constexpr (EPI == EPI_DGELU) bound *= 1.13f;
          eo = scale_exp_of(bound);
          if (nw == 0 && hi == 0) p.p_se[m] = eo;
        }
        static_for<0, TN>([&](auto J) {
          constexpr int j = decltype(J)::value;
          static_for<0, 2>([&](auto G2) {
            constexpr int g2 = decltype(G2)::value;
            const int nb = nw + j * 32 + 16 * g2;
            if (nb < p.N) {
              float o8[8];
#pragma unroll
              for (int e = 0; e < 8; ++e) o8[e] = acc[i][j][8 * g2 + e];
              if (p.p_np == 2) {
                f16x8 h0, h1;
                split2x8(o8, eo, h0, h1);
                char* q = p.P + (long)(nb >> 4) * p.p_ks + (long)((m0 + mloc) >> 5) * (2 * CH) + lane * 16;
                *reinterpret_cast<f16x8*>(q) = h0;
                *reinterpret_cast<f16x8*>(q + CH) = h1;
              } else {
                bf16x8 h0, h1, h2;
                split3x8(o8, h0, h1, h2);
                char* q = p.P + (long)(nb >> 4) * p.p_ks + (long)((m0 + mloc) >> 5) * (3 * CH) + lane * 16;
                *reinterpret_cast<bf16x8*>(q) = h0;
                *reinterpret_cast<bf16x8*>(q + CH) = h1;
                *reinterpret_cast<bf16x8*>(q + 2 * CH) = h2;
              }
            }
          });
        });
      }
    }
  });
}


template <int NP, int TM, int TN, int EPI>
__device__ __forceinline__ void x6p_epilogue_fast(const PlanesP& p, f32x16 (&acc)[TM][TN], int m0, int mvalid, int wm, int nw,
                                                  char* wl, int lane) {
  const int l31 = lane & 31, hi = lane >> 5;
  constexpr int WC = TN * 32, RS = WC * 4 + 16, LPR = WC / 4, NIT = 32 * LPR / 64;
  const int mw = m0 + wm * TM * 32;
  const int rows_w = mvalid - wm * TM * 32;
  float* lb = reinterpret_cast<float*>(wl + 32 * RS);
  int* le = reinterpret_cast<int*>(lb + WC);
#pragma unroll
  for (int c = lane; c < WC; c += 64) {
    const bool ok = nw + c < p.N;
    lb[c] = (p.bias && ok) ? p.bias[nw + c] : 0.f;
    if constexpr (NP == 2) le[c] = (p.b_se && ok) ? p.b_se[nw + c] : 0;
  }
  int ea[TM];
  static_for<0, TM>([&](auto I) { ea[decltype(I)::value] = (NP == 2 && p.a_se) ? p.a_se[mw + decltype(I)::value * 32 + l31] : 0; });
  int eo[TM];
  static_for<0, TM>([&](auto I) { eo[decltype(I)::value] = 0; });
  if (p.P && p.p_np == 2) {
    const float bd0 = p.b_bd[0], bd1 = p.b_bd[1];
    static_for<0, TM>([&](auto I) {
      constexpr int i = decltype(I)::value;
      float bound = p.a_rn[mw + i * 32 + l31] * bd0 + bd1;
      if constexpr (EPI == EPI_DGELU) bound *= 1.13f;
      eo[i] = scale_exp_of(bound);
    });
  }
  auto resid4 = [&](int i, int j, int g) __attribute__((always_inline)) {
    f32x4 r = {0.f, 0.f, 0.f, 0.f};
    const int n = nw + 4 * hi + j * 32 + 8 * g;
    if (i * 32 + l31 < rows_w && n < p.N) r = *reinterpret_cast<const f32x4*>(p.resid + (long)(mw + i * 32 + l31) * p.ldr + n);
    return r;
  };
  auto store_rows = [&](float* dst, const f32x16 (&o)[TN], int i, bool accumulate) __attribute__((always_inline)) {
    static_for<0, TN>([&](auto J) {
      constexpr int j = decltype(J)::value;
      static_for<0, 4>([&](auto G) {
        constexpr int g = decltype(G)::value;
        f32x4 q = {o[j][4 * g], o[j][4 * g + 1], o[j][4 * g + 2], o[j][4 * g + 3]};
        *reinterpret_cast<f32x4*>(wl + l31 * RS + (j * 32 + 8 * g + 4 * hi) * 4) = q;
      });
    });
    constexpr int HB = NIT > 4 ? 4 : NIT;
    static_for<0, NIT / HB>([&](auto H) {
      constexpr int h0 = decltype(H)::value * HB;
      f32x4 q[HB];
      float* d[HB];
      bool ok[HB];
#pragma unroll
      for (int it = 0; it < HB; ++it) {
        const int idx = (h0 + it) * 64 + lane, row = idx / LPR, c4 = (idx - row * LPR) * 4;
        q[it] = *reinterpret_cast<const f32x4*>(wl + row * RS + c4 * 4);
        d[it] = dst + (long)(mw + i * 32 + row) * p.ldc + nw + c4;
        ok[it] = nw + c4 < p.N && i * 32 + row < rows_w;
      }
      if (accumulate) {
#pragma unroll
        for (int it = 0; it < HB; ++it)
          if (ok[it]) q[it] += *reinterpret_cast<const f32x4*>(d[it]);
      }
#pragma unroll
      for (int it = 0; it < HB; ++it)
        if (ok[it]) *reinterpret_cast<f32x4*>(d[it]) = q[it];
    });
  };

  constexpr bool RES = EPI != EPI_GELU;
  f32x4 rv[TN][4];
  static_for<0, TN>([&](auto J) {
    static_for<0, 4>([&](auto G) {
      rv[decltype(J)::value][decltype(G)::value] = (RES && p.resid) ? resid4(0, decltype(J)::value, decltype(G)::value) : f32x4{0.f, 0.f, 0.f, 0.f};
    });
  });
  static_for<0, TM>([&](auto I) {
    constexpr int i = decltype(I)::value;
    if (i * 32 < rows_w) {
      __builtin_amdgcn_sched_barrier(0);
      static_for<0, TN>([&](auto J) {
        constexpr int j = decltype(J)::value;
        static_for<0, 4>([&](auto G) {
          constexpr int g = decltype(G)::value;
          const int c = j * 32 + 8 * g + 4 * hi;
          if constexpr (NP == 2) {
            const i32x4 eb = *reinterpret_cast<const i32x4*>(le + c);
#pragma unroll
            for (int e = 0; e < 4; ++e) acc[i][j][4 * g + e] = __builtin_amdgcn_ldexpf(acc[i][j][4 * g + e], ea[i] + eb[e]);
          }
          const f32x4 b4 = *reinterpret_cast<const f32x4*>(lb + c);
#pragma unroll
          for (int e = 0; e < 4; ++e) acc[i][j][4 * g + e] += b4[e];
        });
      });
      __builtin_amdgcn_sched_barrier(0);
      if (p.preact) store_rows(p.preact, acc[i], i, false);
      __builtin_amdgcn_sched_barrier(0);
      static_for<0, TN>([&](auto J) {
        constexpr int j = decltype(J)::value;
        static_for<0, 4>([&](auto G) {
          constexpr int g = decltype(G)::value;
          const f32x4 r4 = RES ? rv[j][g] : f32x4{0.f, 0.f, 0.f, 0.f};
          if constexpr (RES && i + 1 < TM) {
            if (p.resid) rv[j][g] = resid4(i + 1, j, g);
          }
#pragma unroll
          for (int e = 0; e < 4; ++e) {
            float v = acc[i][j][4 * g + e];
            const float r = r4[e];
            if constexpr (EPI == EPI_GELU) v = gelu_erf(v) + r;
            else if constexpr (EPI == EPI_DGELU) v *= gelu_erf_grad(r);
            else {
              if (p.act == SVL_ACT_RELU) v = fmaxf(v, 0.f);
              if (p.act == SVL_ACT_MUL_DRELU) v = r > 0.f ? v : 0.f;
              else v += r;
            }
            acc[i][j][4 * g + e] = v;
          }
          if constexpr (EPI == EPI_DGELU) __builtin_amdgcn_sched_barrier(0);
        });
      });
      __builtin_amdgcn_sched_barrier(0);
      if (p.C) store_rows(p.C, acc[i], i, p.accumulate != 0);
      __builtin_amdgcn_sched_barrier(0);
      if (p.P) {
        if (p.p_np == 2 && nw == 0 && hi == 0) p.p_se[mw + i * 32 + l31] = eo[i];
        static_for<0, TN>([&](auto J) {
          constexpr int j = decltype(J)::value;
          static_for<0, 2>([&](auto G2) {
            constexpr int g2 = decltype(G2)::value;
            const int nb = nw + j * 32 + 16 * g2;
            if (nb < p.N) {
              float o8[8];
#pragma unroll
              for (int e = 0; e < 8; ++e) o8[e] = acc[i][j][8 * g2 + e];
              if (p.p_np == 2) {
                f16x8 h0, h1;
                split2x8(o8, eo[i], h0, h1);
                char* q = p.P + (long)(nb >> 4) * p.p_ks + (long)((mw + i * 32) >> 5) * (2 * CH) + lane * 16;
                *reinterpret_cast<f16x8*>(q) = h0;
                *reinterpret_cast<f16x8*>(q + CH) = h1;
              } else {
                bf16x8 h0, h1, h2;
                split3x8(o8, h0, h1, h2);
                char* q = p.P + (long)(nb >> 4) * p.p_ks + (long)((mw + i * 32) >> 5) * (3 * CH) + lane * 16;
                *reinterpret_cast<bf16x8*>(q) = h0;
                *reinterpret_cast<bf16x8*>(q + CH) = h1;
                *reinterpret_cast<bf16x8*>(q + 2 * CH) = h2;
              }
            }
          });
        });
      }
    }
  });
}


template <int NP> constexpr int prod_a(int t) {
  return NP == 3 ? (t == 0 ? 2 : (t == 2 || t == 3) ? 1 : 0) : (t == 0 ? 1 : 0);
}
template <int NP> constexpr int prod_b(int t) {
  return NP == 3 ? (t == 1 ? 2 : (t == 2 || t == 4) ? 1 : 0) : (t == 1 ? 1 : 0);
}

template <int NP, int BN, int EPI, bool EF>
__global__ __launch_bounds__(512) void gemm_x6p_kernel(const PlanesP p) {
  extern __shared__ __attribute__((aligned(1024))) char sm[];
  constexpr int WN = BN == 192 ? 2 : 4, WM = 8 / WN;
  constexpr int TM = BM / 32 / WM, TN = BN / 32 / WN;
  constexpr int NCHA = BM / 32 * NP, NCHB = BN / 32 * NP, NCH = NCHA + NCHB;
  constexpr int STAGE = NCH * CH;
  constexpr int CPW = (NCH + 7) / 8;
  constexpr bool EVEN = NCH % 8 == 0;
  static_assert(NSTAGE * STAGE <= 160 * 1024 && 8 * (32 * (TN * 128 + 16) + TN * 32 * 8) <= 160 * 1024, "LDS");

  const int tid = threadIdx.x, lane = tid & 63, l31 = lane & 31, hi = lane >> 5;
  const int wave = __builtin_amdgcn_readfirstlane(tid >> 6);
  const int grp = wave >> 2, wm = wave / WN, wq = wave % WN;

  X6P_STAMP(0);
  const TileRef tr = tile_of_block(p);
  const int m0 = tr.m0, n0 = tr.tn * BN, mvalid = tr.rows;
  const int nblk = (mvalid + 31) >> 5;
  const int vb = min(TM, max(0, nblk - wm * TM));

  const char* a_src = p.A + (long)(m0 >> 5) * (NP * CH);
  const char* b_src = p.B + (long)tr.tn * (NCHB * CH);
  const unsigned lane16 = lane * 16;
  const unsigned sm_base = (unsigned)(uintptr_t)(__attribute__((address_space(3))) char*)sm;
  const int nk = p.K >> 4;

  auto issue = [&](int kg, int st) __attribute__((always_inline)) {
    const char* ak = a_src + (long)kg * p.a_ks;
    const char* bk = b_src + (long)kg * p.b_ks;
    const unsigned dst = sm_base + st * STAGE;
    static_for<0, CPW>([&](auto I) {
      constexpr int i = decltype(I)::value;
      const int c = wave + 8 * i;
      if (EVEN || i + 1 < CPW || c < NCH) {
        const char* s;
        if constexpr (8 * i + 7 < NCHA) {
          const int rb = c / NP;
          s = ak + (rb < nblk ? c : c - NP * rb) * CH;
        } else {
          static_assert(8 * i >= NCHA, "A / B chunk boundary must fall on a multiple of 8");
          const int cb = c - NCHA, rb = cb / NP;
          s = bk + (tr.tn * (BN / 32) + rb < p.b_rb ? cb : cb - NP * rb) * CH;
        }
        glds16(s, lane16, dst + c * CH);
      }
    });
  };
  const bool short_wave = !EVEN && wave >= NCH % 8;
  auto wait_older = [&]() __attribute__((always_inline)) {
    if constexpr (EVEN) wait_vm<CPW>();
    else {
      if (short_wave) wait_vm<CPW - 1>();
      else wait_vm<CPW>();
    }
  };

  f32x16 acc[TM][TN];
  static_for<0, TM>([&](auto I) {
    static_for<0, TN>([&](auto J) {
#pragma unroll
      for (int r = 0; r < 16; ++r) acc[decltype(I)::value][decltype(J)::value][r] = 0.f;
    });
  });

  const int fa = lane * 16 + wm * (TM * NP * CH);
  const int fb = lane * 16 + NCHA * CH + wq * (TN * NP * CH);

  issue(0, 0);
  if (nk > 1) {
    issue(1, 1);
    wait_older();
  } else {
    wait_vm<0>();
  }
  __builtin_amdgcn_s_barrier();
  X6P_STAMP(1);
  if (grp == 1) __builtin_amdgcn_s_barrier();
  __builtin_amdgcn_sched_barrier(0);

  constexpr int NPROD = NP == 3 ? 6 : 3;
  auto kloop = [&](auto FULLT) __attribute__((always_inline)) {
    constexpr bool FULL = decltype(FULLT)::value;
    typedef typename FragOf<NP>::T frag;
    frag a[NP][TM], b[NP][TN];
    int st = 0;
    for (int kg = 0; kg < nk; ++kg) {
      const char* S = sm + st * STAGE;
      {
        static_for<0, NP>([&](auto P) {
          constexpr int pl = decltype(P)::value;
          static_for<0, TN>([&](auto J) {
            b[pl][decltype(J)::value] = *reinterpret_cast<const frag*>(S + fb + (decltype(J)::value * NP + pl) * CH);
          });
        });
        static_for<0, NP>([&](auto P) {
          constexpr int pl = decltype(P)::value;
          static_for<0, TM>([&](auto I) {
            a[pl][decltype(I)::value] = *reinterpret_cast<const frag*>(S + fa + (decltype(I)::value * NP + pl) * CH);
          });
        });
      }
      if (kg + 2 < nk) {
        int st2 = st + 2;
        if (st2 >= NSTAGE) st2 -= NSTAGE;
        issue(kg + 2, st2);
        wait_older();
      } else {
        wait_vm<0>();
      }
      asm volatile("s_waitcnt lgkmcnt(0)" ::: "memory");
      __builtin_amdgcn_sched_barrier(0);
      __builtin_amdgcn_s_barrier();
      __builtin_amdgcn_sched_barrier(0);
      __builtin_amdgcn_s_setprio(1);
      if constexpr (FULL) {
        static_for<0, NPROD>([&](auto T) {
          constexpr int t = decltype(T)::value;
          constexpr int PA = prod_a<NP>(t), PB = prod_b<NP>(t);
          static_for<0, TM>([&](auto I) {
            static_for<0, TN>([&](auto J) {
              constexpr int i = decltype(I)::value, j = decltype(J)::value;
              acc[i][j] = mfma16<NP>(b[PB][j], a[PA][i], acc[i][j]);
            });
          });
        });
      } else {
        static_for<0, TM>([&](auto I) {
          constexpr int i = decltype(I)::value;
          if (i < vb) {
            static_for<0, NPROD>([&](auto T) {
              constexpr int t = decltype(T)::value;
              constexpr int PA = prod_a<NP>(t), PB = prod_b<NP>(t);
              static_for<0, TN>([&](auto J) {
                constexpr int j = decltype(J)::value;
                acc[i][j] = mfma16<NP>(b[PB][j], a[PA][i], acc[i][j]);
              });
            });
          }
        });
      }
      __builtin_amdgcn_s_setprio(0);
      __builtin_amdgcn_sched_barrier(0);
      __builtin_amdgcn_s_barrier();
      __builtin_amdgcn_sched_barrier(0);
      st = st + 1 == NSTAGE ? 0 : st + 1;
    }
  };
  if (vb == TM) kloop(std::true_type{});
  else kloop(std::false_type{});
  if (grp == 0) __builtin_amdgcn_s_barrier();
  X6P_STAMP(2);

  const int nw = n0 + wq * (TN * 32);
  char* wl = sm + wave * (32 * (TN * 128 + 16) + TN * 32 * 8);
  if constexpr (EF) x6p_epilogue_fast<NP, TM, TN, EPI>(p, acc, m0, mvalid, wm, nw, wl, lane);
  else x6p_epilogue<NP, TM, TN, EPI>(p, acc, m0, mvalid, wm, nw, wl, lane);
#ifdef SVL_X6P_TIMING
  asm volatile("s_waitcnt vmcnt(0)" ::: "memory");
#endif
  X6P_STAMP(3);
}


inline uint64_t attr_bit() {
  int dev = 0;
  (void)hipGetDevice(&dev);
  return 1ull << (dev & 63);
}
inline bool attr_needed(std::atomic<uint64_t>& mask) { return !(mask.load(std::memory_order_acquire) & attr_bit()); }

template <int NP, int BN, int EPI, bool EF>
int launch_kernel(const PlanesP& q, long blocks, hipStream_t st) {
  constexpr int TN_ = BN / 32 / (BN == 192 ? 2 : 4);
  constexpr size_t stages = (size_t)NSTAGE * ((BM + BN) / 32 * NP) * CH, scratch = (size_t)8 * (32 * (TN_ * 128 + 16) + TN_ * 32 * 8);
  constexpr size_t lds = stages > scratch ? stages : scratch;
  static std::atomic<uint64_t> mask{0};
  if (attr_needed(mask)) {
    SVL_HIP_CHECK(hipFuncSetAttribute(reinterpret_cast<const void*>(gemm_x6p_kernel<NP, BN, EPI, EF>),
                                      hipFuncAttributeMaxDynamicSharedMemorySize, (int)lds));
    mask.fetch_or(attr_bit(), std::memory_order_acq_rel);
  }
  hipLaunchKernelGGL((gemm_x6p_kernel<NP, BN, EPI, EF>), dim3((unsigned)blocks), dim3(512), lds, st, q);
  SVL_LAUNCH_CHECK("svl_gemm_planes_f32");
  return SVL_OK;
}

template <int NP, int BN, bool EF>
int launch_tile(PlanesP q, hipStream_t st) {
  q.tiles_n = (q.N + BN - 1) / BN;
  q.full_m = q.M / BM;
  q.tail_rows = q.M % BM;
  const long nf = (long)q.full_m * q.tiles_n, nr = q.tail_rows ? q.tiles_n : 0, total = nf + nr;
  if (total <= 0 || total > 0x7fffffffL) {
    svl_set_error("svl_gemm_planes_f32: bad tile count %ld", total);
    return SVL_ERR_INVALID_ARG;
  }
  const int pw = 6;
  q.panel = pw < q.tiles_n ? pw : q.tiles_n;
  long fs = 0;
  for (int x = 0; x < 8; ++x) {
    const long blocks = (total - x + 7) / 8, rag = nr > x ? (nr - x + 7) / 8 : 0;
    q.rcnt[x] = (int)rag;
    q.fstart[x] = (int)fs;
    fs += blocks - rag;
  }
  if (q.act == SVL_ACT_GELU) return launch_kernel<NP, BN, EPI_GELU, EF>(q, total, st);
  if (q.act == SVL_ACT_MUL_DGELU) return launch_kernel<NP, BN, EPI_DGELU, EF>(q, total, st);
  return launch_kernel<NP, BN, EPI_LIGHT, EF>(q, total, st);
}

template <int NP>
int launch(const PlanesP& q, hipStream_t st) {
  auto cost = [&](int bn) {
    const long tiles = (long)(q.M / BM) * ((q.N + bn - 1) / bn);
    const long rounds = tiles > 0 ? (tiles + 255) / 256 : 1;
    return (double)rounds * bn * (bn == 128 ? 1.15 : bn == 192 ? 1.04 : 1.0);
  };
  int bn = 0;
  {
    bn = 256;
    if (q.N <= 128) bn = 128;
    else {
      if (cost(192) < cost(bn)) bn = 192;
      if (cost(128) < cost(bn)) bn = 128;
    }
  }
  const bool al16 = ((reinterpret_cast<uintptr_t>(q.C) | reinterpret_cast<uintptr_t>(q.preact) | reinterpret_cast<uintptr_t>(q.resid)) & 15) == 0;
  const bool ef = q.epi_fast && al16 && (q.N & 3) == 0 && (q.ldc & 3) == 0 && (!q.resid || (q.ldr & 3) == 0) &&
                  !(q.act == SVL_ACT_GELU && q.resid);
  if (!ef) return launch_tile<NP, 128, false>(q, st);
  if (bn == 128) return launch_tile<NP, 128, true>(q, st);
  if (bn == 192) return launch_tile<NP, 192, true>(q, st);
  return launch_tile<NP, 256, true>(q, st);
}

}
```

semivl_amd/lib.py:

```python
import ctypes as C
import os
import subprocess

import torch

_HERE = os.path.dirname(os.path.abspath(__file__))
LIB_PATH = os.path.join(_HERE, "libsemivl_hip.so")
CSRC = os.path.join(_HERE, "csrc")

c_f32p = C.c_void_p
c_i64p = C.c_void_p


class Operand(C.Structure):
    _fields_ = [("ptr", C.c_void_p), ("ld", C.c_int64), ("bs_outer", C.c_int64), ("bs_inner", C.c_int64)]


class ConvGeom(C.Structure):
    _fields_ = [("H", C.c_int), ("W", C.c_int), ("Ho", C.c_int), ("Wo", C.c_int), ("stride", C.c_int),
                ("C1", C.c_int), ("C2", C.c_int), ("rep", C.c_int),
                ("KH", C.c_int), ("KW", C.c_int), ("dil", C.c_int), ("pad", C.c_int), ("sign", C.c_int),
                ("src2", C.c_void_p), ("ld2", C.c_int64), ("patch", C.c_int)]


class GemmDesc(C.Structure):
    _fields_ = [("a_mode", C.c_int), ("b_mode", C.c_int), ("M", C.c_int), ("N", C.c_int), ("K", C.c_int),
                ("batch", C.c_int), ("batch_inner", C.c_int), ("ksplit", C.c_int),
                ("A", Operand), ("B", Operand), ("conv", ConvGeom),
                ("C", C.c_void_p), ("out_mode", C.c_int),
                ("ldc_m", C.c_int64), ("ldc_n", C.c_int64), ("c_bs_outer", C.c_int64), ("c_bs_inner", C.c_int64),
                ("ct_H", C.c_int), ("ct_W", C.c_int), ("ct_Cout", C.c_int),
                ("alpha", C.c_float), ("bias", C.c_void_p), ("bias_mod", C.c_int), ("act", C.c_int),
                ("preact", C.c_void_p), ("resid", C.c_void_p),
                ("ldr_m", C.c_int64), ("ldr_n", C.c_int64), ("r_bs_outer", C.c_int64), ("r_bs_inner", C.c_int64),
                ("accumulate", C.c_int), ("conv_w_planes", C.c_void_p), ("emu_ws", C.c_void_p),
                ("b_stats", C.c_void_p), ("b_gamma", C.c_void_p), ("b_beta", C.c_void_p),
                ("a_amax", C.c_void_p), ("b_amax", C.c_void_p)]


class PGemmDesc(C.Structure):
    _fields_ = [("A", C.c_void_p), ("B", C.c_void_p), ("a_rows", C.c_int64), ("b_rows", C.c_int64),
                ("m_off", C.c_int), ("M", C.c_int), ("N", C.c_int), ("K", C.c_int),
                ("C", C.c_void_p), ("ldc", C.c_int64), ("planes_out", C.c_void_p), ("p_rows", C.c_int64),
                ("bias", C.c_void_p), ("act", C.c_int), ("preact", C.c_void_p), ("resid", C.c_void_p),
                ("ldr", C.c_int64), ("accumulate", C.c_int),
                ("fmt", C.c_int), ("p_fmt", C.c_int), ("a_sexp", C.c_void_p), ("b_sexp", C.c_void_p),
                ("a_rnorm", C.c_void_p), ("b_bound", C.c_void_p), ("p_sexp", C.c_void_p)]


class CeDesc(C.Structure):
    _fields_ = [("logits", C.c_void_p), ("B", C.c_int), ("N", C.c_int), ("HW", C.c_int64),
                ("target", C.c_void_p), ("use_ignore_t", C.c_int), ("conf", C.c_void_p), ("ign", C.c_void_p),
                ("conf_thresh", C.c_float), ("all_pixels", C.c_int), ("mc_target", C.c_void_p), ("partials", C.c_void_p),
                ("dlogits", C.c_void_p), ("gscale", C.c_void_p), ("img_weight", C.c_void_p)]


class CeUpDesc(C.Structure):
    _fields_ = [("logits", C.c_void_p), ("B", C.c_int), ("N", C.c_int), ("h", C.c_int), ("w", C.c_int), ("H", C.c_int),
                ("W", C.c_int), ("align_corners", C.c_int), ("target", C.c_void_p), ("use_ignore_t", C.c_int),
                ("conf", C.c_void_p), ("ign", C.c_void_p), ("conf_thresh", C.c_float), ("all_pixels", C.c_int),
                ("mc_target", C.c_void_p), ("partials", C.c_void_p), ("dlogits", C.c_void_p), ("gscale", C.c_void_p),
                ("img_weight", C.c_void_p)]


class SeqAttnDesc(C.Structure):
    _fields_ = [("groups", C.c_int), ("inner", C.c_int), ("seq", C.c_int), ("heads", C.c_int),
                ("outer_stride", C.c_int64), ("inner_stride", C.c_int64), ("seq_stride", C.c_int64),
                ("qkv", C.c_void_p), ("out", C.c_void_p), ("probs", C.c_void_p),
                ("dout", C.c_void_p), ("dqkv", C.c_void_p), ("dscores", C.c_void_p)]


_I, _L, _F, _D, _P = C.c_int, C.c_int64, C.c_float, C.c_double, C.c_void_p
SIGNATURES = {
    "svl_version": (_I, []),
    "svl_last_error": (_I, [C.c_char_p, C.c_size_t]),
    "svl_gemm_f32": (_I, [C.POINTER(GemmDesc), _P]),
    "svl_set_gemm_emulation": (_I, [_I]),
    "svl_get_gemm_emulation": (_I, []),
    "svl_set_conv_tiled": (_I, [_I]),
    "svl_planes_rows": (_L, [_L]),
    "svl_planes_bytes": (_L, [_L, _I]),
    "svl_split_planes_bf16x3": (_I, [_P, _L, _L, _L, _I, _P, _L, _L, _P]),
    "svl_planes_bytes_fmt": (_L, [_L, _I, _I]),
    "svl_split_planes_f16x2": (_I, [_P, _L, _L, _L, _I, _P, _L, _L, _P, _P, _P, _P]),
    "svl_gemm_planes_f32": (_I, [C.POINTER(PGemmDesc), _P]),
    "svl_conv3x3_wgrad_tiled_groups": (_I, [_I, _I, _I, _I, _I]),
    "svl_conv3x3_wgrad_tiled": (_I, [_P, _L, _I, _P, _L, _I, _P, _L, _I, _I, _I, _I, _I, _P, _I, _P, _P]),
    "svl_reduce_slabs_f32": (_I, [_P, _P, _I, _L, _I, _P]),
    "svl_softmax_max_f32": (_I, [_P, _I, _I, _L, _P, _P, _P]),
    "svl_cutmix_f32": (_I, [_P, _P, _P, _P, _I, _I, _L, _P]),
    "svl_cutmix_i64": (_I, [_P, _P, _P, _P, _I, _L, _P]),
    "svl_ce_num_blocks": (_L, [_I, _I, _L]),
    "svl_ce_fused_f32": (_I, [C.POINTER(CeDesc), _P]),
    "svl_ce_finalize": (_I, [_P, _L, _P, _P]),
    "svl_ce_up_num_blocks": (_L, [_I, _I, _I, _I, _I, _I, _I]),
    "svl_ce_up_fused_f32": (_I, [C.POINTER(CeUpDesc), _P]),
    "svl_softmax_max_up_f32": (_I, [_P, _I, _I, _I, _I, _I, _I, _I, _P, _P, _P]),
    "svl_semivl_gscale": (_I, [_P, _D, _F, _P, _P, _P, _P]),
    "svl_semivl_loss": (_I, [_P, _D, _F, _P, _P, _P, _P]),
    "svl_inv_count_f32": (_I, [_P, _P, _P]),
    "svl_conf_ratio_f32": (_I, [_P, _P, _I, _L, _F, _P, _P, _P]),
    "svl_conf_avg_ws_doubles": (_L, [_I]),
    "svl_conf_avg_factor": (_I, [_P, _P, _I, _L, _P, _P, _P]),
    "svl_stream_release": (_I, [_P]),
    "svl_stream_prepare": (_I, [_P]),
    "svl_stream_helper": (_I, [_P, C.POINTER(C.c_void_p)]),
    "svl_last_gemm_path": (_I, []),
    "svl_absmax_launches": (_L, []),
    "svl_shutdown": (_I, []),
    "svl_num_stream_contexts": (_I, []),
    "svl_clock_probe": (_I, [_P, _I, C.c_uint64, _P]),
    "svl_bernoulli_f32": (_I, [_P, _L, _F, C.c_uint64, C.c_uint64, _P]),
    "svl_softmax_planes_f32": (_I, [_P, _I, _I, _L, _P, _P]),
    "svl_count_valid_i64": (_I, [_P, _L, _P, _P]),
    "svl_target_prob_f32": (_I, [_P, _I, _I, _L, _P, _P, _P]),
    "svl_target_prob_up_f32": (_I, [_P, _I, _I, _I, _I, _I, _I, _I, _P, _P, _P]),
    "svl_ohem_ws_bytes": (_L, [_L]),
    "svl_ohem_threshold_f32": (_I, [_P, _L, _L, _P, _L, _F, _P, _P, _P]),
    "svl_ohem_relabel_i64": (_I, [_P, _P, _L, _P, _P, _P, _P]),
    "svl_maskclip_labels": (_I, [_P, _I, _I, _I, _I, _I, _I, _F, _F, _P, _P, _P]),
    "svl_concept_max_f32": (_I, [_P, _I, _I, _L, _P, _I, _P, _P]),
    "svl_iou_hist_i64": (_I, [_P, _P, _L, _I, _I, _P, _P]),
    "svl_layernorm_fwd": (_I, [_P, _P, _P, _F, _L, _I, _P, _P, _P]),
    "svl_layernorm_fwd_planes": (_I, [_P, _P, _P, _F, _L, _I, _P, _P, _P, _L, _P]),
    "svl_layernorm_fwd_planes_f16x2": (_I, [_P, _P, _P, _F, _L, _I, _P, _P, _P, _L, _P, _P, _P]),
    "svl_layernorm_fwd_pack_f16x2": (_I, [_P, _P, _P, _F, _L, _I, _P, _P, _P, _L, _L, _P, _P, _I, _P, _P]),
    "svl_layernorm_bwd_pack_f16x2": (_I, [_P, _P, _P, _P, _L, _I, _P, _P, _P, _L, _L, _P, _P, _P, _P]),
    "svl_layernorm_bwd_parts": (_I, [_L]),
    "svl_layernorm_bwd": (_I, [_P, _P, _P, _P, _L, _I, _P, _P, _P, _P, _P]),
    "svl_softmax_rows_fwd": (_I, [_P, _L, _I, _L, _F, _P]),
    "svl_softmax_rows_bwd": (_I, [_P, _P, _L, _I, _L, _F, _P]),
    "svl_l2norm_fwd": (_I, [_P, _L, _I, _F, _P, _P, _P]),
    "svl_l2norm_bwd": (_I, [_P, _P, _P, _L, _I, _P, _P]),
    "svl_colsum_ws_floats": (_L, [_L, _I]),
    "svl_colsum_f32": (_I, [_P, _L, _I, _L, _P, _I, _P, _P]),
    "svl_eltwise_f32": (_I, [_I, _P, _P, _P, _L, _P]),
    "svl_chanmask_f32": (_I, [_P, _P, _F, _L, _I, _I, _P, _P]),
    "svl_fill_f32": (_I, [_P, _F, _L, _P]),
    "svl_affine_planes_f32": (_I, [_P, _L, _I, _L, _P, _P, _P]),
    "svl_permute_rows_f32": (_I, [_P, _L, _I, _I, _I, _P, _P]),
    "svl_permute4_f32": (_I, [_P, _P, _L, _L, _L, _L, _L, _L, _L, _L, _P]),
    "svl_bound2_f32": (_I, [_P, _L, _P, _L, _P, _P]),
    "svl_copy2d_f32": (_I, [_P, _L, _L, _L, _P, _L, _L, _L, _L, _I, _I, _P]),
    "svl_groupnorm_fwd": (_I, [_P, _L, _P, _P, _F, _I, _L, _I, _I, _I, _P, _L, _P, _P]),
    "svl_conv3x3_gn_ws_doubles": (_L, [_I, _I, _I, _I]),
    "svl_conv3x3_gn_f32": (_I, [_P, _L, _I, _P, _L, _I, _I, _P, _I, _I, _I, _I, _P, _L, _F, _P, _P, _P, _P, _P]),
    "svl_conv3x3_weight_planes_bytes": (_L, [_I, _I]),
    "svl_conv3x3_weight_planes": (_I, [_P, _I, _I, _P, _P]),
    "svl_groupnorm_scale_shift": (_I, [_P, _P, _P, _I, _I, _I, _P, _P]),
    "svl_groupnorm_apply": (_I, [_P, _L, _P, _P, _I, _L, _I, _I, _I, _P, _P, _L, _P]),
    "svl_groupnorm_bwd": (_I, [_P, _L, _P, _L, _P, _L, _P, _P, _P, _I, _L, _I, _I, _I, _P, _L, _P, _P]),
    "svl_conv3x3_gnb_ws_doubles": (_L, [_I, _I, _I, _I]),
    "svl_conv3x3_dgrad_gnb_f32": (_I, [_P, _L, _I, _P, _I, _I, _I, _I, _P, _L, _I, _P, _P, _P, _P, _P, _P, _P]),
    "svl_groupnorm_bwd_apply": (_I, [_P, _L, _P, _L, _P, _P, _P, _I, _L, _I, _I, _I, _P, _P, _L, _P]),
    "svl_bn_ws_doubles": (_L, [_L, _I]),
    "svl_bn_stats": (_I, [_P, _L, _L, _I, _P, _P, _P]),
    "svl_bn_finalize": (_I, [_P, _D, _F, _F, _P, _P, _I, _P, _P, _P]),
    "svl_bn_eval_invstd": (_I, [_P, _F, _I, _P, _P]),
    "svl_bn_apply": (_I, [_P, _L, _L, _I, _P, _P, _P, _P, _P, _L, _I, _P, _L, _P]),
    "svl_bn_bwd_reduce": (_I, [_P, _L, _P, _L, _P, _L, _P, _P, _P, _P, _L, _I, _P, _P, _P]),
    "svl_bn_bwd_apply": (_I, [_P, _L, _P, _L, _P, _L, _P, _P, _P, _P, _P, _D, _L, _I, _P, _L, _P, _L, _P]),
    "svl_maxpool3x3s2_fwd": (_I, [_P, _I, _I, _I, _I, _P, _P, _P]),
    "svl_maxpool3x3s2_bwd": (_I, [_P, _P, _I, _I, _I, _I, _P, _P]),
    "svl_aug_resample_u8": (_I, [_P, _I, _I, _I, _I, _I, _I, _I, _I, _I, _I, _I, _I, _P, _P]),
    "svl_aug_to_float": (_I, [_P, _I, C.POINTER(C.c_float), C.POINTER(C.c_float), _P, _P]),
    "svl_aug_mask_i64": (_I, [_P, _I, _I, _I, _P, _P]),
    "svl_aug_photometric_u8": (_I, [_P, _I, _I, _F, _P, _P]),
    "svl_aug_gaussian_blur_u8": (_I, [_P, _I, _I, _F, _P, _P, _P]),
    "svl_attention_fwd": (_I, [_P, _I, _I, _I, _P, _P, _P, _L, _P]),
    "svl_attention_bwd": (_I, [_P, _P, _P, _P, _I, _I, _I, _P, _P, _P, _L, _P]),
    "svl_attention_h2_ws_bytes": (_L, [_I, _I, _I, _I]),
    "svl_attention_fwd_h2": (_I, [_P, _I, _I, _I, _P, _P, _P, _L, _P, _L, _P]),
    "svl_attention_bwd_h2": (_I, [_P, _P, _P, _P, _I, _I, _I, _P, _P, _P, _L, _P, _L, _P]),
    "svl_attention_h2_tr_sets": (_I, [_I]),
    "svl_attention_bwd_h2_sets": (_I, [_P, _P, _P, _P, _I, _I, _I, _P, _P, _P, _L, _P, _L, _P]),
    "svl_conv_cout1_fwd": (_I, [_P, _L, _I, _I, _I, _I, _I, _I, _I, _I, _P, _P, _P, _P, _P]),
    "svl_conv_cout1_wgrad_blocks": (_I, [_I, _I, _I]),
    "svl_conv_cout1_wgrad": (_I, [_P, _P, _L, _I, _I, _I, _I, _I, _I, _P, _P, _P]),
    "svl_tap_gather": (_I, [_P, _I, _I, _I, _I, _I, _I, _I, _I, _P, _P]),
    "svl_seqattn_fwd": (_I, [C.POINTER(SeqAttnDesc), _P]),
    "svl_seqattn_bwd": (_I, [C.POINTER(SeqAttnDesc), _P]),
    "svl_bilinear_nhwc_fwd": (_I, [_P, _L, _I, _I, _I, _I, _I, _I, _I, _I, _P, _L, _I, _P]),
    "svl_sum_rep_f32": (_I, [_P, _L, _L, _I, _L, _I, _P, _P]),
    "svl_bilinear_nhwc_bwd": (_I, [_P, _L, _I, _I, _I, _I, _I, _I, _I, _I, _P, _L, _I, _P]),
    "svl_bilinear_planes_fwd": (_I, [_P, _L, _I, _I, _I, _I, _I, _P, _P]),
    "svl_bilinear_planes_bwd": (_I, [_P, _L, _I, _I, _I, _I, _I, _P, _P]),
    "svl_avgpool_cat_fwd": (_I, [_P, _I, _I, _I, _I, _I, _I, _P, _I, _I, _P, _P]),
    "svl_avgpool_cat_bwd": (_I, [_P, _I, _I, _I, _I, _I, _I, _I, _P, _I, _P]),
    "svl_avgpool_cat_bwd_text": (_I, [_P, _I, _L, _I, _I, _I, _P, _P, _P]),
    "svl_gap_tokens_fwd": (_I, [_P, _L, _I, _L, _I, _P, _L, _P]),
    "svl_gap_tokens_bwd": (_I, [_P, _L, _I, _L, _I, _P, _L, _I, _P]),
    "svl_bcast_rows_fwd": (_I, [_P, _L, _I, _L, _I, _P, _L, _I, _P]),
    "svl_bcast_rows_bwd": (_I, [_P, _L, _I, _I, _L, _I, _P, _L, _P]),
    "svl_adamw_step": (_I, [_P, _P, _P, _P, _P, _P, _P, _I, _L, _F, _F, _F, _I, _F, _P, _F, _P]),
    "svl_sgd_step": (_I, [_P, _P, _P, _P, _P, _P, _I, _L, _F, _F, _I, _I, _F, _P, _F, _P]),
    "svl_lora_merge_f32": (_I, [_P, _L, _P, _L, _I, _I, _I, _I, _F, _P, _P, _L, _P]),
    "svl_lora_wgrad_ws_floats": (_L, [_I, _I, _I]),
    "svl_lora_wgrad_f32": (_I, [_P, _L, _P, _P, _L, _I, _I, _I, _F, _P, _I, _P, _I, _P, _P]),
    "svl_prompt_rows_fwd_f32": (_I, [_P, _P, _P, _P, _F, _I, _I, _I, _I, _P]),
    "svl_prompt_rows_bwd_f32": (_I, [_P, _P, _P, _P, _F, _I, _I, _I, _I, _I, _P]),
    "svl_droppath_fwd_f32": (_I, [_P, _P, _P, _F, _P, _I, _I, _I, _P]),
    "svl_droppath_bwd_f32": (_I, [_P, _P, _F, _P, _I, _I, _I, _P]),
}

_lib = None


def build_library(force=False):
    if os.path.exists(LIB_PATH) and not force:
        srcs = [os.path.join(CSRC, f) for f in os.listdir(CSRC) if f.endswith((".hip", ".h"))]
        srcs.append(os.path.join(_HERE, "..", "include", "semivl_hip.h"))
        if all(os.path.getmtime(s) <= os.path.getmtime(LIB_PATH) for s in srcs):
            return LIB_PATH
    subprocess.run(["make", "-C", CSRC, "-j8"], check=True, stdout=subprocess.DEVNULL)
    return LIB_PATH


def load():
    global _lib
    if _lib is not None:
        return _lib
    if not os.path.exists(LIB_PATH):
        raise RuntimeError(
            f"semivl_amd: {LIB_PATH} is missing. Build it with `python -c 'import __graft_entry__ as g; g.build()'` "
            "or `make -C semivl_amd/csrc`. There is no fallback path.")
    lib = C.CDLL(LIB_PATH)
    for name, (res, args) in SIGNATURES.items():
        fn = getattr(lib, name)
        fn.restype = res
        fn.argtypes = args
    _lib = lib
    return lib


def last_error():
    buf = C.create_string_buffer(512)
    load().svl_last_error(buf, 512)
    return buf.value.decode()


def check(rc, what=""):
    if rc != 0:
        raise RuntimeError(f"semivl_hip {what} failed (status {rc}): {last_error()}")
```

semivl_amd/model/vit.py:

```python
import math

import torch
import torch.nn as nn
import torch.nn.functional as F

from .. import gradsync, ops


class _MHAParams(nn.Module):
    def __init__(self, dims):
        super().__init__()
        self.in_proj_weight = nn.Parameter(torch.empty(3 * dims, dims))
        self.in_proj_bias = nn.Parameter(torch.zeros(3 * dims))
        self.out_proj = nn.Linear(dims, dims)
        nn.init.xavier_uniform_(self.in_proj_weight)
        nn.init.constant_(self.out_proj.bias, 0.)


class _AttnParams(nn.Module):
    def __init__(self, dims):
        super().__init__()
        self.attn = _MHAParams(dims)


class _FFNParams(nn.Module):
    def __init__(self, dims, hidden):
        super().__init__()
        self.layers = nn.Sequential(nn.Sequential(nn.Linear(dims, hidden), nn.Identity(), nn.Identity()),
                                    nn.Linear(hidden, dims), nn.Identity())


class _LoRAParams(nn.Module):

    def __init__(self, dim, r, scaling=1., targets="qkvo"):
        super().__init__()
        self.dim, self.r, self.scaling, self.targets = dim, r, float(scaling), targets
        for t in "qkvo":
            if t in targets:
                setattr(self, "a_" + t, nn.Linear(dim, r, bias=False))
                setattr(self, "b_" + t, nn.Linear(r, dim, bias=False))
        self.reset_parameters()

    def reset_parameters(self):
        for t in "qkvo":
            if t in self.targets:
                nn.init.kaiming_uniform_(getattr(self, "a_" + t).weight, a=math.sqrt(5))
                nn.init.zeros_(getattr(self, "b_" + t).weight)

    def pair(self, t):
        if t not in self.targets:
            return None
        return getattr(self, "a_" + t).weight, getattr(self, "b_" + t).weight


class TransformerEncoderLayer(nn.Module):

    def __init__(self, embed_dims, num_heads, feedforward_channels, eps=1e-5, lora=None):
        super().__init__()
        self.embed_dims, self.num_heads, self.eps = embed_dims, num_heads, eps
        self.ln1 = nn.LayerNorm(embed_dims, eps=eps)
        self.attn = _AttnParams(embed_dims)
        self.lora = _LoRAParams(embed_dims, **lora) if lora is not None else None
        self.ln2 = nn.LayerNorm(embed_dims, eps=eps)
        self.ffn = _FFNParams(embed_dims, feedforward_channels)

    def plist(self):
        a, f = self.attn.attn, self.ffn.layers
        return dict(ln1w=self.ln1.weight, ln1b=self.ln1.bias, win=a.in_proj_weight, bin=a.in_proj_bias,
                    wout=a.out_proj.weight, bout=a.out_proj.bias, ln2w=self.ln2.weight, ln2b=self.ln2.bias,
                    w1=f[0][0].weight, b1=f[0][0].bias, w2=f[1].weight, b2=f[1].bias)

    def merged_plist(self):
        lo, a, p = self.lora, self.attn.attn, self.plist()
        pairs = [lo.pair(t) for t in "qkv"]
        with torch.no_grad():
            if any(pr is not None for pr in pairs):
                p["win"] = ops.lora_merge(a.in_proj_weight, pairs, lo.scaling)
            if "o" in lo.targets:
                p["wout"] = ops.lora_merge(a.out_proj.weight, [lo.pair("o")], lo.scaling)
        return p


class _PatchEmbedParams(nn.Module):
    def __init__(self, cin, dims, patch, bias):
        super().__init__()
        self.projection = nn.Conv2d(cin, dims, patch, stride=patch, bias=bias)


def sink_grad(param, grad_fn, shape=None):
    mg = getattr(param, "main_grad", None)
    if mg is not None:
        grad_fn(mg, True)
        return None
    out = ops.empty(*param.shape, device=param.device)
    grad_fn(out, False)
    return out


DROP_PATH_SITES = ("attn", "ffn", "ffn_v")


def block_forward(x, p, heads, eps, Bn, T, want_v, skip_x, save, dp=None):
    E = x.shape[1]
    D = E // heads
    pp = ops.planes_eligible(x.shape[0], E, E)
    if pp:
        y1, st1, y1a = ops.layernorm_fwd(x, p["ln1w"], p["ln1b"], eps, planes=True, want_y=save is not None)
    else:
        y1, st1 = ops.layernorm_fwd(x, p["ln1w"], p["ln1b"], eps)
        y1a = y1
    if skip_x:
        vproj = ops.linear(y1a, p["win"][2 * E:], p["bin"][2 * E:])
        qkv = None
    else:
        qkv = ops.linear(y1a, p["win"], p["bin"])
        vproj = qkv[:, 2 * E:]
    v = None
    if save is not None:
        save.update(x=x, y1=y1, st1=st1, qkv=qkv, vproj=vproj, want_v=want_v, skip_x=skip_x, eps=eps,
                    y1_amax=y1a.amax if pp else None,
                    dp=dp)
    dp = dp or {}

    def ffn(pre, want_pre, mask=None):
        if pp:
            _, st2_, y2a = ops.layernorm_fwd(pre, p["ln2w"], p["ln2b"], eps, planes=True, want_y=False)
        else:
            y2a, st2_ = ops.layernorm_fwd(pre, p["ln2w"], p["ln2b"], eps)
        h_pre_ = ops.empty(pre.shape[0], p["w1"].shape[0], device=x.device) if want_pre else None
        h_ = ops.linear(y2a, p["w1"], p["b1"], act=ops.ACT_GELU, preact=h_pre_, planes_only=True)
        if mask is not None:
            return ops.droppath_add(ops.linear(h_, p["w2"], p["b2"]), pre, mask, dp["keep"], Bn, T), st2_, h_pre_
        return ops.linear(h_, p["w2"], p["b2"], resid=pre), st2_, h_pre_

    if want_v:
        vo = ops.linear(ops.split_planes(vproj) if pp else vproj, p["wout"], p["bout"], resid=x)
        v, st2v, hv_pre = ffn(vo, save is not None, dp.get("ffn_v"))
        if save is not None:
            save.update(vo=vo, st2v=st2v, hv_pre=hv_pre)
    xo = None
    if not skip_x:
        o_p = None
        if D == 64 and pp and ops.attention_planes_ok():
            o, P, o_p, *sets = ops.attention_fwd(qkv, Bn, T, heads, want_lse=save is not None, planes=True,
                                                 want_out=save is not None, keep_sets=save is not None)
        elif D == 64:
            o, P, *sets = ops.attention_fwd(qkv, Bn, T, heads, want_lse=save is not None, keep_sets=save is not None)
        else:
            o, P = ops.vit_attention_fwd(qkv, Bn, T, heads, D)
            sets = []
        o_a = o_p if o_p is not None else (ops.split_planes(o) if pp else o)
        if dp.get("attn") is not None:
            x2 = ops.droppath_add(ops.linear(o_a, p["wout"], p["bout"]), x, dp["attn"], dp["keep"], Bn, T)
        else:
            x2 = ops.linear(o_a, p["wout"], p["bout"], resid=x)
        xo, st2, h_pre = ffn(x2, save is not None, dp.get("ffn"))
        if save is not None:
            save.update(o=o, P=P, x2=x2, st2=st2, h_pre=h_pre, sets=sets[0] if sets else None)
    return xo, v


FFN_LN_KEYS = ("ln1w", "ln1b", "ln2w", "ln2b", "w1", "b1", "w2", "b2")


def block_backward(dxo, dv, p, s, heads, Bn, T, want=frozenset(), dxo_p=None):
    x, y1 = s["x"], s["y1"]
    E = x.shape[1]
    D = E // heads
    pp = ops.planes_eligible(x.shape[0], E, E)
    g = {}
    dx_res = None
    dqkv = dqkv_p = dqkv_amax = None
    wout_parts = []
    need_h = "w1" in want or "b1" in want
    dp = s.get("dp") or {}

    def ffn_ln_bwd(dout, dout_p, pre_ln_in, st2, h_pre, mask=None):
        res = dout
        if mask is not None:
            dout = ops.droppath_scale(dout, mask, dp["keep"], Bn, T)
            dout_p = ops.split_planes(dout) if pp else None
        a_ = dout_p if dout_p is not None else dout
        dhp = ops.matmul_nn(a_, p["w2"], dact=ops.ACT_MUL_DGELU, z=h_pre, planes_only=not need_h)
        dy2 = ops.matmul_nn(dhp, p["w1"])
        if "w2" in want:
            g.setdefault("w2", []).append(("gelu", dout, h_pre))
        if "b2" in want:
            g.setdefault("b2", []).append(("sum", dout))
        if "w1" in want:
            g.setdefault("w1", []).append(("ln", dhp, pre_ln_in, st2))
        if "b1" in want:
            g.setdefault("b1", []).append(("sum", dhp))
        if "ln2w" in want or "ln2b" in want:
            r_ = ops.layernorm_bwd(dy2, pre_ln_in, st2, p["ln2w"], dx_add=res, want_wgrad=True, planes=pp)
            g.setdefault("ln2w", []).append(("add", r_[1]))
            g.setdefault("ln2b", []).append(("add", r_[2]))
            return r_[0], (r_[3] if pp else None)
        if pp:
            return ops.layernorm_bwd(dy2, pre_ln_in, st2, p["ln2w"], dx_add=res, planes=True)
        return ops.layernorm_bwd(dy2, pre_ln_in, st2, p["ln2w"], dx_add=res), None

    if not s["skip_x"] and dxo is not None:
        dx2, dx2p = ffn_ln_bwd(dxo, dxo_p, s["x2"], s["st2"], s["h_pre"], dp.get("ffn"))
        dbr, dbrp = dx2, dx2p
        if dp.get("attn") is not None:
            dbr = ops.droppath_scale(dx2, dp["attn"], dp["keep"], Bn, T)
            dbrp = ops.split_planes(dbr) if pp else None
        do = ops.matmul_nn(dbrp if dbrp is not None else dbr, p["wout"])
        wout_parts.append((dbr, s["o"]))
        if D == 64 and pp and ops.attention_planes_ok() and not (s["want_v"] and dv is not None):
            dqkv, dqkv_p = ops.attention_bwd(do, s["qkv"], s["o"], s["P"], Bn, T, heads, planes=True, sets=s.get("sets"))
            dqkv_amax = dqkv_p.amax
        elif D == 64:
            dqkv = ops.attention_bwd(do, s["qkv"], s["o"], s["P"], Bn, T, heads, sets=s.get("sets"))
        else:
            dqkv = ops.vit_attention_bwd(do, s["qkv"], s["P"], Bn, T, heads, D)
        dx_res = dx2
    dvproj = None
    if s["want_v"] and dv is not None:
        dvo, dvop = ffn_ln_bwd(dv, None, s["vo"], s["st2v"], s["hv_pre"], dp.get("ffn_v"))
        dvproj = ops.matmul_nn(dvop if dvop is not None else dvo, p["wout"])
        wout_parts.append((dvo, s["vproj"]))
        dx_res = dvo if dx_res is None else ops.add(dx_res, dvo)
    if dqkv is not None and dvproj is not None:
        rows = dqkv.shape[0]
        ops.copy2d(dvproj, 0, rows, 0, E, dqkv, 2 * E, rows, 0, 3 * E, rows, E, accumulate=True)
        dvproj = dqkv_amax = None
    g["wout_parts"] = wout_parts
    if dqkv is not None:
        g["in_full"] = (dqkv, y1, dqkv_amax, s.get("y1_amax"))
        dy1 = ops.matmul_nn(dqkv_p if dqkv_p is not None else dqkv, p["win"])
    elif dvproj is not None:
        g["in_v"] = (dvproj, y1)
        dy1 = ops.matmul_nn(dvproj, p["win"][2 * E:])
    else:
        return dx_res, None, g
    if "ln1w" in want or "ln1b" in want:
        r_ = ops.layernorm_bwd(dy1, x, s["st1"], p["ln1w"], dx_add=dx_res, want_wgrad=True, planes=pp)
        g["ln1w"], g["ln1b"] = [("add", r_[1])], [("add", r_[2])]
        return r_[0], (r_[3] if pp else None), g
    if pp:
        dx_in, dx_in_p = ops.layernorm_bwd(dy1, x, s["st1"], p["ln1w"], dx_add=dx_res, planes=True)
        return dx_in, dx_in_p, g
    return ops.layernorm_bwd(dy1, x, s["st1"], p["ln1w"], dx_add=dx_res), None, g


def ffn_ln_wgrads(p, g):
    out = {}
    for key, parts in g.items():
        if key not in FFN_LN_KEYS:
            continue

        def fn(dst, acc, parts=parts):
            for j, part in enumerate(parts):
                a_ = acc or j > 0
                if part[0] == "gelu":
                    ops.matmul_tn_gelu(part[1], part[2], out=dst, accumulate=a_)
                elif part[0] == "ln":
                    ops.matmul_tn_ln(part[1], part[2], part[3], p["ln2w"], p["ln2b"], out=dst, accumulate=a_)
                elif part[0] == "sum":
                    ops.colsum(part[1], out=dst, accumulate=a_)
                elif a_:
                    ops.add(dst, part[1], out=dst)
                else:
                    ops.eltwise(4, part[1], None, out=dst)
        out[key] = sink_grad(p[key], fn)
# ... 575 lines not shown
```

semivl_amd/ops.py:

```python
import collections
import ctypes as C
import os
import math
import weakref

import torch

from . import lib as L

A_KC, A_MC, A_CONV, A_PATCH = 0, 1, 2, 3
B_KC, B_NC, B_CONVW = 0, 1, 2
B_NC_GELU, B_NC_LN, B_PATCHT = 3, 4, 5
ACT_NONE, ACT_GELU, ACT_RELU, ACT_MUL_DGELU, ACT_MUL_DRELU = 0, 1, 2, 3, 4
OUT_STRIDED, OUT_CONVT2X, OUT_PATCH = 0, 1, 2


def _st():
    return C.c_void_p(torch.cuda.current_stream().cuda_stream)


PROFILE = None
PROFILE_SCOPE = None


# ... 248 lines not shown

PLANES_FMT = os.environ.get("SVL_PLANES_FMT", "h2")
assert PLANES_FMT in ("h2", "b3")


class Planes:
    __slots__ = ("buf", "rows", "K", "prow", "fmt", "sexp", "rnorm", "amax", "_bd")

    def __init__(self, rows, K, device=None, buf=None, fmt=None, sexp=None, rnorm=None):
        assert K % 16 == 0
        self.fmt = fmt or PLANES_FMT
        self.rows, self.K, self.prow = rows, K, planes_rows(rows)
        dev = device if device is not None else (buf.device if buf is not None else torch.cuda.current_device())
        self._bd = self.amax = None
        if self.fmt == "h2":
            self.buf = buf if buf is not None else torch.empty(K // 16 * self.prow * 32, dtype=torch.float16, device=dev)
            self.sexp = sexp if sexp is not None else torch.empty(self.prow, dtype=torch.int32, device=dev)
            self.rnorm = rnorm
        else:
            self.buf = buf if buf is not None else torch.empty(K // 16 * self.prow * 48, dtype=torch.bfloat16, device=dev)
            self.sexp = self.rnorm = None

    @property
    def shape(self):
        return (self.rows, self.K)

    def kslice(self, k0, k1):
        assert k0 % 16 == 0 and k1 % 16 == 0 and 0 <= k0 < k1 <= self.K
        per = self.prow * (32 if self.fmt == "h2" else 48)
        return Planes(self.rows, k1 - k0, buf=self.buf[k0 // 16 * per:k1 // 16 * per], fmt=self.fmt, sexp=self.sexp,
                      rnorm=self.rnorm)


ONEPASS = not os.environ.get("SVL_NO_ONEPASS")


def split_planes(x2d, out=None, row_off=0, transpose=False, fmt=None, want_amax=False):
    assert x2d.dim() == 2 and x2d.dtype == torch.float32
    if transpose:
        K, rows = x2d.shape
        assert x2d.stride(1) == 1
        ld, ks = 1, x2d.stride(0)
    else:
        rows, K = x2d.shape
        assert x2d.stride(1) == 1
        ld, ks = x2d.stride(0), 1
    if out is None:
        out = Planes(rows, K, device=x2d.device, fmt=fmt)
    assert out.K == K and out.rows >= row_off + rows and row_off % 32 == 0
    if out.fmt == "h2":
        if out.rnorm is None:
            out.rnorm = torch.empty(out.prow, dtype=torch.float32, device=x2d.device)
        if want_amax and ONEPASS and row_off == 0 and out.rows == rows:
            out.amax = torch.empty(1, dtype=torch.int32, device=x2d.device)
        L.check(L.load().svl_split_planes_f16x2(_p(x2d), ld, ks, rows, K, _p(out.buf), out.prow, row_off, _p(out.sexp),
                                                _p(out.rnorm), _p(out.amax), _st()), "svl_split_planes_f16x2")
        return out
    L.check(L.load().svl_split_planes_bf16x3(_p(x2d), ld, ks, rows, K, _p(out.buf), out.prow, row_off, _st()),
            "svl_split_planes_bf16x3")
    return out


WEIGHT_EPOCH = 0
_WPLANES = {}


class StreamCached:
    __slots__ = ("val", "ev", "seen")

    def __init__(self, val):
        self.val, self.ev, self.seen = val, None, None
        if torch.cuda.is_available():
            s = torch.cuda.current_stream()
            self.ev = torch.cuda.Event()
            self.ev.record(s)
            self.seen = {s.cuda_stream}

    @staticmethod
    def _tensors(v):
        if isinstance(v, torch.Tensor):
            yield v
        elif isinstance(v, (tuple, list)):
            for x in v:
                yield from StreamCached._tensors(x)
        elif hasattr(v, "buf"):
            yield v.buf
            for extra in (getattr(v, "sexp", None), getattr(v, "rnorm", None)):
                if extra is not None:
                    yield extra

    def get(self):
        if self.ev is not None:
            s = torch.cuda.current_stream()
            if s.cuda_stream not in self.seen:
                s.wait_event(self.ev)
                for t in self._tensors(self.val):
                    if t.is_cuda:
                        t.record_stream(s)
                self.seen.add(s.cuda_stream)
        return self.val


def weights_changed():
    global WEIGHT_EPOCH
    WEIGHT_EPOCH += 1


def weight_planes(W, transpose=False, fmt=None):
    fmt = fmt or PLANES_FMT

    def build():
        return split_planes(W.detach(), transpose=transpose, fmt=fmt)

    base = W._base if W._base is not None else W
    if not isinstance(base, torch.nn.Parameter):
        return build()
    key = (W.data_ptr(), tuple(W.shape), W.stride(0), transpose, fmt)
    ver = (base._version, WEIGHT_EPOCH if base.requires_grad else 0)
    hit = _WPLANES.get(key)
    if hit is not None and hit[0] == ver and hit[2]() is base:
        return hit[1].get()
    pl = build()
    if len(_WPLANES) > 4096:
        _WPLANES.clear()
    _WPLANES[key] = (ver, StreamCached(pl), weakref.ref(base))
    return pl


def _out_bound(B, bias):
    key = (None if bias is None else (bias.data_ptr(), bias._version, WEIGHT_EPOCH if bias.requires_grad else 0),
           torch.cuda.current_stream().cuda_stream)
    if B._bd is None:
        B._bd = {}
    hit = B._bd.get(key)
    if hit is not None:
        return hit
    bd = torch.empty(2, dtype=torch.float32, device=B.buf.device)
    bflat = bias.detach().view(-1) if bias is not None else None
    L.check(L.load().svl_bound2_f32(_p(B.rnorm), B.rows, _p(bflat), bflat.numel() if bflat is not None else 0, _p(bd), _st()),
            "svl_bound2_f32")
    if len(B._bd) > 8:
        B._bd.clear()
    B._bd[key] = bd
    return bd


def planes_eligible(M, N, K):
    return get_gemm_emulation() == 6 and PLANES_PATH and M >= 256 and N >= 256 and K >= 512 and K % 16 == 0


PLANES_PATH = not os.environ.get("SVL_GEMM_NO_PLANES")


def pgemm(A, B, M, N, out=None, planes_out=None, bias=None, act=ACT_NONE, preact=None, resid=None, accumulate=False,
          m_off=0):
    K = A.K
    assert B.K == K and A.rows >= m_off + M and B.rows >= N and A.fmt == B.fmt
    d = L.PGemmDesc()
    d.A, d.B, d.a_rows, d.b_rows = _p(A.buf), _p(B.buf), A.prow, B.prow
    d.m_off, d.M, d.N, d.K = m_off, M, N, K
    if out is not None:
        assert out.stride(1) == 1
        d.C, d.ldc = _p(out), out.stride(0)
    elif preact is not None:
        d.ldc = preact.stride(0)
    keep = None
    if A.fmt == "h2":
        d.fmt, d.a_sexp, d.b_sexp = 1, _p(A.sexp), _p(B.sexp)
    if planes_out is not None:
        d.planes_out, d.p_rows = _p(planes_out.buf), planes_out.prow
        if planes_out.fmt == "h2":
            assert A.fmt == "h2" and A.rnorm is not None
            keep = _out_bound(B, bias)
            d.p_fmt, d.a_rnorm, d.b_bound, d.p_sexp = 1, _p(A.rnorm), _p(keep), _p(planes_out.sexp)
    d.bias, d.act, d.preact = _p(bias), act, _p(preact)
    if resid is not None:
        assert resid.stride(1) == 1
        d.resid, d.ldr = _p(resid), resid.stride(0)
    d.accumulate = 1 if accumulate else 0
    e0 = _prof_begin()
    L.check(L.load().svl_gemm_planes_f32(C.byref(d), _st()), "svl_gemm_planes_f32")
    _prof_end("gemm_bf16x", e0, 2.0 * M * N * K, ("planes" if A.fmt == "b3" else "planes_h2", M, N, K, act))


def _planes_out_for(xa, M, N, resid, act):
    h2 = xa.fmt == "h2" and xa.rnorm is not None and (resid is None or act in (ACT_MUL_DGELU, ACT_MUL_DRELU))
    return Planes(M, N, device=xa.buf.device, fmt="h2" if h2 else "b3")


def linear(x, W, bias=None, act=ACT_NONE, resid=None, out=None, accumulate=False, preact=None, planes_only=False):
    M, K = x.shape
    N = W.shape[0]
    assert W.shape[1] == K and W.stride(1) == 1
    if isinstance(x, Planes) or planes_eligible(M, N, K):
        xa = x if isinstance(x, Planes) else split_planes(x)
        wb = weight_planes(W, fmt=xa.fmt)
        if preact is not None:
            assert out is None or preact.stride(0) == out.stride(0)
        if planes_only and N % 16 == 0 and out is None and not accumulate:
            po = _planes_out_for(xa, M, N, resid, act)
            pgemm(xa, wb, M, N, None, po, bias, act, preact, resid)
            return po
        if out is None:
            out = empty(M, N, device=xa.buf.device)
        pgemm(xa, wb, M, N, out, None, bias, act, preact, resid, accumulate)
        return out
    assert x.stride(1) == 1 and W.is_contiguous()
    if out is None:
        out = empty(M, N, device=x.device)
    gemm(A_KC, B_KC, M, N, K, Op(x, x.stride(0)), Op(W, K), out, ldc_m=out.stride(0), bias=bias, act=act,
         resid=resid, ldr_m=resid.stride(0) if resid is not None else None, accumulate=accumulate, preact=preact)
    return out


def copy2d(src, s_off, sgrp, src_go, src_ld, dst, d_off, dgrp, dst_go, dst_ld, rows, Cc, accumulate=False):
    if accumulate:
        assert dst_go != 0 or rows <= dgrp, "copy2d: accumulating rows of different groups land on one destination (dst_go 0)"
        assert dst_ld != 0 or dgrp == 1, "copy2d: accumulating rows of one group land on one destination (dst_ld 0)"
    L.check(L.load().svl_copy2d_f32(C.c_void_p(src.data_ptr() + 4 * s_off), sgrp, src_go, src_ld,
                                    C.c_void_p(dst.data_ptr() + 4 * d_off), dgrp, dst_go, dst_ld, rows, Cc,
                                    1 if accumulate else 0, _st()), "svl_copy2d_f32")


def matmul_nn(a, b, out=None, accumulate=False, dact=ACT_NONE, z=None, planes_only=False):
    M, K = a.shape
    N = b.shape[1]
    assert b.shape[0] == K and b.stride(1) == 1
    if isinstance(a, Planes) or planes_eligible(M, N, K):
        xa = a if isinstance(a, Planes) else split_planes(a)
        wb = weight_planes(b, transpose=True, fmt=xa.fmt)
        if dact != ACT_NONE:
            assert z is not None and z.shape == (M, N) and z.stride(1) == 1 and not accumulate
        if planes_only and N % 16 == 0 and out is None and not accumulate:
            po = _planes_out_for(xa, M, N, z if dact != ACT_NONE else None, dact)
            pgemm(xa, wb, M, N, None, po, None, dact, None, z if dact != ACT_NONE else None)
            return po
        if out is None:
            out = empty(M, N, device=xa.buf.device)
        pgemm(xa, wb, M, N, out, None, None, dact, None, z if dact != ACT_NONE else None, accumulate)
        return out
    assert a.stride(1) == 1
    if out is None:
        out = empty(M, N, device=a.device)
    if dact != ACT_NONE:
        assert z is not None and z.shape == (M, N) and z.stride(1) == 1 and not accumulate
        gemm(A_KC, B_NC, M, N, K, Op(a, a.stride(0)), Op(b, b.stride(0)), out, ldc_m=out.stride(0), act=dact, resid=z,
             ldr_m=z.stride(0))
        return out
    gemm(A_KC, B_NC, M, N, K, Op(a, a.stride(0)), Op(b, b.stride(0)), out, ldc_m=out.stride(0), accumulate=accumulate)
    return out


def _ksplit_plan(M, N, K, dense=False, emu_tiles=False):
    bm = 32 if M <= 32 else (64 if M <= 64 else 128)
    bn = 128 if (M <= 64 and N > 64) else (32 if N <= 32 else (64 if N <= 64 else 128))
    tiles = math.ceil(M / bm) * math.ceil(N / bn)
    slots = 768
    if emu_tiles or (dense and M >= 256 and N >= 96 and get_gemm_emulation()):
        tiles, slots = math.ceil(M / 128) * math.ceil(N / 128), 512
    s = max(1, min(slots // tiles if tiles <= slots else 1, K // 512 if K >= 1024 else 1, 512))
    ks = math.ceil(math.ceil(K / s) / 16) * 16
    s = math.ceil(K / ks)
    return s, ks


def matmul_tn(a, b, out=None, accumulate=False, a_amax=None, b_amax=None):
    K, M = a.shape
    N = b.shape[1]
    assert b.shape[0] == K and a.stride(1) == 1 and b.stride(1) == 1
    if out is None:
        out = empty(M, N, device=a.device)
        accumulate = False
    assert out.is_contiguous()
    s, ks = _ksplit_plan(M, N, K, dense=True)
    if s == 1:
        gemm(A_MC, B_NC, M, N, K, Op(a, a.stride(0)), Op(b, b.stride(0)), out, accumulate=accumulate, amax=(a_amax, b_amax))
        return out
    slabs = empty(s, M, N, device=a.device)
    gemm(A_MC, B_NC, M, N, K, Op(a, a.stride(0)), Op(b, b.stride(0)), slabs, batch=s, ksplit=ks, c_bso=M * N,
         amax=(a_amax, b_amax))
    reduce_slabs(out, slabs, accumulate)
    return out


def _matmul_tn_prod(a, N, b_op, b_mode, out, accumulate, conv=None, b_aux=None, a_amax=None):
    K, M = a.shape
    assert a.stride(1) == 1
    if out is None:
        out = empty(M, N, device=a.device)
        accumulate = False
    assert out.is_contiguous() and out.numel() == M * N
    s, ks = _ksplit_plan(M, N, K, dense=True)
    if s == 1:
        gemm(A_MC, b_mode, M, N, K, Op(a, a.stride(0)), b_op, out, accumulate=accumulate, conv=conv, b_aux=b_aux,
             amax=(a_amax, None))
        return out
    slabs = empty(s, M, N, device=a.device)
    gemm(A_MC, b_mode, M, N, K, Op(a, a.stride(0)), b_op, slabs, batch=s, ksplit=ks, c_bso=M * N, conv=conv, b_aux=b_aux,
         amax=(a_amax, None))
    reduce_slabs(out, slabs, accumulate)
    return out


def matmul_tn_gelu(a, h_pre, out=None, accumulate=False, a_amax=None):
    assert h_pre.shape[0] == a.shape[0] and h_pre.stride(1) == 1
    return _matmul_tn_prod(a, h_pre.shape[1], Op(h_pre, h_pre.stride(0)), B_NC_GELU, out, accumulate, a_amax=a_amax)


def matmul_tn_ln(a, x, stats, gamma, beta, out=None, accumulate=False):
    assert x.shape[0] == a.shape[0] and x.stride(1) == 1 and stats.is_contiguous()
    return _matmul_tn_prod(a, x.shape[1], Op(x, x.stride(0)), B_NC_LN, out, accumulate,
                           b_aux=(stats, gamma.contiguous(), beta.contiguous()))


def matmul_tn_patch(a, img, patch, out=None, accumulate=False):
    img = img.contiguous()
    Bn, Cin, H, W = img.shape
    g = conv_geom(H, W, Cin, patch, patch, patch=patch)
    assert a.shape[0] == Bn * ((H + patch - 1) // patch) * ((W + patch - 1) // patch)
    return _matmul_tn_prod(a, Cin * patch * patch, Op(img, 0), B_PATCHT, out, accumulate, conv=g)


def reduce_slabs(out, slabs, accumulate=False):
    L.check(L.load().svl_reduce_slabs_f32(_p(out), _p(slabs), slabs.shape[0], out.numel(), 1 if accumulate else 0,
                                          _st()), "svl_reduce_slabs_f32")


def lora_merge(W, pairs, s, out=None):
    n = len(pairs)
    rows, E = W.shape[0] // n, W.shape[1]
    assert W.dim() == 2 and W.shape[0] == rows * n and W.stride(1) == 1
    if out is None:
        out = empty(*W.shape, device=W.device)
    assert out.shape == W.shape and out.stride(1) == 1 and out.dtype == torch.float32
    Ap, Bp = (C.c_void_p * n)(), (C.c_void_p * n)()
    r, ldb = 1, 1
    for i, pr in enumerate(pairs):
        if pr is None:
            continue
        A, B = pr
        assert A.dim() == 2 and A.shape[1] == E and A.is_contiguous() and _chk(A) is A and _chk(B) is B
        assert tuple(B.shape) == (rows, A.shape[0]) and (B.stride(1) == 1 or A.shape[0] == 1)
        assert not any(Ap) or (r, ldb) == (A.shape[0], B.stride(0)), "lora_merge: the adapters of one call share r"
        r, ldb = A.shape[0], B.stride(0)
        Ap[i], Bp[i] = A.data_ptr(), B.data_ptr()
    e0 = _prof_begin()
# ... 194 lines not shown
    if want_wgrad:
        nparts = lib.svl_layernorm_bwd_parts(rows)
        dgp = empty(nparts, Cc, device=x.device)
        dbp = empty(nparts, Cc, device=x.device)
    L.check(lib.svl_layernorm_bwd(_p(dy), _p(x), _p(stats), _p(gamma), rows, Cc, _p(dx_add), _p(dx), _p(dgp), _p(dbp),
                                  _st()), "svl_layernorm_bwd")
    res = (dx, colsum(dgp), colsum(dbp)) if want_wgrad else (dx,)
    if planes:
        res = res + (split_planes(dx),)
    return res if len(res) > 1 else res[0]


def softmax_rows_fwd(s, rows, cols, ld, scale):
    L.check(L.load().svl_softmax_rows_fwd(_p(s), rows, cols, ld, float(scale), _st()), "svl_softmax_rows_fwd")


def softmax_rows_bwd(dp, p, rows, cols, ld, scale):
    L.check(L.load().svl_softmax_rows_bwd(_p(dp), _p(p), rows, cols, ld, float(scale), _st()), "svl_softmax_rows_bwd")


def l2norm_fwd(x, eps=0.0):
    rows, Cc = x.shape
    y = torch.empty_like(x)
    inv = empty(rows, device=x.device)
    L.check(L.load().svl_l2norm_fwd(_p(x), rows, Cc, float(eps), _p(y), _p(inv), _st()), "svl_l2norm_fwd")
    return y, inv


def l2norm_bwd(dy, y, inv):
    rows, Cc = y.shape
    dx = torch.empty_like(y)
    L.check(L.load().svl_l2norm_bwd(_p(dy), _p(y), _p(inv), rows, Cc, _p(dx), _st()), "svl_l2norm_bwd")
    return dx


def groupnorm_fwd(x, ldx, gamma, beta, eps, imgs, HW, Cc, G, relu, y, ldy):
    stats = empty(imgs, G, 2, device=x.device)
    L.check(L.load().svl_groupnorm_fwd(_p(x), ldx, _p(gamma), _p(beta), float(eps), imgs, HW, Cc, G, 1 if relu else 0,
                                       _p(y), ldy, _p(stats), _st()), "svl_groupnorm_fwd")
    return stats


UP_LOSS = not os.environ.get("SVL_NO_UP_LOSS")
GN_DEFER = True


def groupnorm_scale_shift(stats, gamma, beta, imgs, Cc, G):
    t = empty(imgs, 2, Cc, device=stats.device)
    L.check(L.load().svl_groupnorm_scale_shift(_p(stats), _p(gamma), _p(beta), imgs, Cc, G, _p(t), _st()),
            "svl_groupnorm_scale_shift")
    return t


def conv3x3_gn(x, ldx, imgs, H, W, C1, wf, Co, eps, src2=None, ld2=0, C2=0, rep=1, gn_in=None):
    if not (CONV_TILED and Co % 16 == 0):
        return None
    lib = L.load()
    ws = torch.empty(max(1, lib.svl_conv3x3_gn_ws_doubles(imgs, H, W, Co)), dtype=torch.float64, device=x.device)
    pre = empty(imgs * H * W, Co, device=x.device)
    stats = empty(imgs, Co // 16, 2, device=x.device)
    e0 = _prof_begin()
    rc = lib.svl_conv3x3_gn_f32(_p(x), ldx, C1, _p(src2), ld2, C2, rep, _p(wf), imgs, H, W, Co, _p(pre), Co, float(eps),
                                _p(ws), _p(stats), _p(gn_in), _p(w_planes_of(wf)), _st())
    if rc == -3:
        return None
    L.check(rc, "svl_conv3x3_gn_f32")
    if e0 is not None:
        x6 = get_gemm_emulation() == 6 and not os.environ.get("SVL_CONV_TILED_NO_EMU")
        K = 9 * (C1 + C2)
        _prof_end("gemm_bf16x" if x6 else "gemm", e0, 2.0 * imgs * H * W * Co * K, (A_CONV, B_KC, imgs * H * W, Co, K, 1))
    return pre, stats


def groupnorm_apply(x, ldx, gamma, beta, imgs, HW, Cc, G, relu, stats, y, ldy):
    L.check(L.load().svl_groupnorm_apply(_p(x), ldx, _p(gamma), _p(beta), imgs, HW, Cc, G, 1 if relu else 0, _p(stats),
                                         _p(y), ldy, _st()), "svl_groupnorm_apply")
    return y


def groupnorm_bwd(dy, lddy, x, ldx, y, ldy, stats, gamma, imgs, HW, Cc, G, relu, dx, lddx, beta=None):
    cs = empty(imgs, 2, Cc, device=x.device)
    L.check(L.load().svl_groupnorm_bwd(_p(dy), lddy, _p(x), ldx, _p(None if beta is not None else y), ldy, _p(stats),
                                       _p(gamma), _p(beta), imgs, HW, Cc, G, 1 if relu else 0, _p(dx), lddx, _p(cs),
                                       _st()), "svl_groupnorm_bwd")
    flat = cs.view(imgs, 2 * Cc)
    dbeta = colsum(flat, C_=Cc, ld=2 * Cc)
    dgamma = colsum(flat[:, Cc:], C_=Cc, ld=2 * Cc)
    return dgamma, dbeta


GN_BWD_FUSED = True


def conv3x3_dgrad_gnb(dy, lddy, imgs, H, W, Co, wd, Ci, gn_x, gn_stats, gn_gamma, gn_beta, G):
    if not (GN_BWD_FUSED and CONV_TILED and Ci % 16 == 0 and G * 16 == Ci and dy.is_cuda and get_gemm_emulation() == 6):
        return None
    lib = L.load()
    table = groupnorm_scale_shift(gn_stats, gn_gamma, gn_beta, imgs, Ci, G)
    ws = torch.empty(max(1, lib.svl_conv3x3_gnb_ws_doubles(imgs, H, W, Ci)), dtype=torch.float64, device=dy.device)
    dx = empty(imgs * H * W, Ci, device=dy.device)
    cs = empty(imgs, 2, Ci, device=dy.device)
    e0 = _prof_begin()
    rc = lib.svl_conv3x3_dgrad_gnb_f32(_p(dy), lddy, Co, _p(wd), imgs, H, W, Ci, _p(dx), Ci, 0, _p(gn_x), _p(table), _p(gn_stats),
                                       _p(ws), _p(cs), _p(w_planes_of(wd)), _st())
    if rc == -3:
        return None
    L.check(rc, "svl_conv3x3_dgrad_gnb_f32")
    _prof_end("gemm_bf16x", e0, 2.0 * imgs * H * W * Ci * 9 * Co, (A_CONV, B_KC, imgs * H * W, Ci, 9 * Co, 1))
    return dx, cs


def groupnorm_bwd_from_sums(dy, lddy, x, ldx, stats, gamma, beta, imgs, HW, Cc, G, relu, cs, dx, lddx):
    L.check(L.load().svl_groupnorm_bwd_apply(_p(dy), lddy, _p(x), ldx, _p(stats), _p(gamma), _p(beta), imgs, HW, Cc, G,
                                             1 if relu else 0, _p(cs), _p(dx), lddx, _st()), "svl_groupnorm_bwd_apply")
    flat = cs.view(imgs, 2 * Cc)
    dbeta = colsum(flat, C_=Cc, ld=2 * Cc)
    dgamma = colsum(flat[:, Cc:], C_=Cc, ld=2 * Cc)
    return dgamma, dbeta


def attention_h2():
    return get_gemm_emulation() == 6 and not os.environ.get("SVL_ATTN_NO_EMU")


def _attn_family():
    return "attention_bf16x" if (PROFILE is not None and attention_h2()) else "attention"


def attention_planes_ok():
    return attention_h2() and PLANES_PATH


def _attn_ws(Bn, T, H, backward, dev):
    n = L.load().svl_attention_h2_ws_bytes(Bn, T, H, int(backward))
    return torch.empty(n + 1024, dtype=torch.uint8, device=dev), n


def attention_tr_sets(on=None):
    return bool(L.load().svl_attention_h2_tr_sets(-1 if on is None else int(bool(on))))


def _ws_ptr(ws):
    return (ws.data_ptr() + 1023) // 1024 * 1024


def attention_fwd(qkv, Bn, T, H, want_lse=True, planes=False, want_out=True, keep_sets=False):
    E = H * 64
    if planes and not attention_planes_ok():
        raise RuntimeError("attention_fwd: planes outputs need emulation mode 6 (attention_planes_ok())")
    out = empty(Bn * T, E, device=qkv.device)
    lse = empty(Bn * H * T, device=qkv.device) if want_lse else None
    e0 = _prof_begin()
    sets = None
    if attention_h2():
        ws, n = _attn_ws(Bn, T, H, 0, qkv.device)
        L.check(L.load().svl_attention_fwd_h2(_p(qkv), Bn, T, H, _p(out), _p(lse), None, 0, _ws_ptr(ws), n, _st()),
                "svl_attention_fwd_h2")
        if keep_sets and not attention_tr_sets():
            sets = ws
    else:
        L.check(L.load().svl_attention_fwd(_p(qkv), Bn, T, H, _p(out), _p(lse), None, 0, _st()), "svl_attention_fwd")
    _prof_end(_attn_family(), e0, 4.0 * Bn * H * T * T * 64, ("fwd_h2" if attention_h2() else "fwd", Bn, T, H))
    if not planes:
        return (out, lse, sets) if keep_sets else (out, lse)
    op = split_planes(out)
    return ((out if want_out else None), lse, op) + ((sets,) if keep_sets else ())


def attention_bwd(dout, qkv, out, lse, Bn, T, H, planes=False, sets=None):
    if planes and not attention_planes_ok():
        raise RuntimeError("attention_bwd: planes outputs need emulation mode 6 (attention_planes_ok())")
    dqkv = torch.empty_like(qkv)
    ws = empty(Bn * H * T, device=qkv.device)
    e0 = _prof_begin()
    if attention_h2() and sets is not None and not attention_tr_sets():
        wsb, n = _attn_ws(Bn, T, H, 2, qkv.device)
        L.check(L.load().svl_attention_bwd_h2_sets(_p(qkv), _p(out), _p(dout), _p(lse), Bn, T, H, _p(ws), _p(dqkv), _ws_ptr(sets),
                                                   sets.numel() - (_ws_ptr(sets) - sets.data_ptr()), _ws_ptr(wsb), n, _st()),
                "svl_attention_bwd_h2_sets")
    elif attention_h2():
        wsb, n = _attn_ws(Bn, T, H, 1, qkv.device)
        L.check(L.load().svl_attention_bwd_h2(_p(qkv), _p(out), _p(dout), _p(lse), Bn, T, H, _p(ws), _p(dqkv), None, 0,
                                              _ws_ptr(wsb), n, _st()), "svl_attention_bwd_h2")
    else:
        L.check(L.load().svl_attention_bwd(_p(qkv), _p(out), _p(dout), _p(lse), Bn, T, H, _p(ws), _p(dqkv), None, 0, _st()),
                "svl_attention_bwd")
    _prof_end(_attn_family(), e0, 14.0 * Bn * H * T * T * 64, ("bwd_h2" if attention_h2() else "bwd", Bn, T, H))
    return (dqkv, split_planes(dqkv, want_amax=True)) if planes else dqkv


def vit_attention_fwd(qkv, Bn, T, H, D):
    E = H * D
    Tp = (T + 3) // 4 * 4
    dev = qkv.device
    P = empty(Bn * H, T, Tp, device=dev)
    gemm(A_KC, B_KC, T, T, D, Op(qkv, 3 * E, 0, T * 3 * E, D), Op(qkv, 3 * E, E, T * 3 * E, D), P, ldc_m=Tp,
         batch=Bn * H, batch_inner=H, c_bso=H * T * Tp, c_bsi=T * Tp)
    softmax_rows_fwd(P, Bn * H * T, T, Tp, 1.0 / math.sqrt(D))
    out = empty(Bn * T, E, device=dev)
    gemm(A_KC, B_NC, T, D, T, Op(P, Tp, 0, H * T * Tp, T * Tp), Op(qkv, 3 * E, 2 * E, T * 3 * E, D), out, ldc_m=E,
         batch=Bn * H, batch_inner=H, c_bso=T * E, c_bsi=D)
    return out, P


def vit_attention_bwd(dout, qkv, P, Bn, T, H, D):
    E = H * D
    Tp = P.shape[2]
    dev = qkv.device
    dqkv = empty(Bn * T, 3 * E, device=dev)
    bh = dict(batch=Bn * H, batch_inner=H)
    p_op = Op(P, Tp, 0, H * T * Tp, T * Tp)
    do_op = Op(dout, E, 0, T * E, D)
    gemm(A_MC, B_NC, T, D, T, p_op, do_op, dqkv, c_off=2 * E, ldc_m=3 * E, c_bso=T * 3 * E, c_bsi=D, **bh)
    dP = empty(Bn * H, T, Tp, device=dev)
    gemm(A_KC, B_KC, T, T, D, do_op, Op(qkv, 3 * E, 2 * E, T * 3 * E, D), dP, ldc_m=Tp, c_bso=H * T * Tp,
         c_bsi=T * Tp, **bh)
    softmax_rows_bwd(dP, P, Bn * H * T, T, Tp, 1.0 / math.sqrt(D))
    ds_op = Op(dP, Tp, 0, H * T * Tp, T * Tp)
    gemm(A_KC, B_NC, T, D, T, ds_op, Op(qkv, 3 * E, E, T * 3 * E, D), dqkv, c_off=0, ldc_m=3 * E, c_bso=T * 3 * E,
         c_bsi=D, **bh)
    gemm(A_MC, B_NC, T, D, T, ds_op, Op(qkv, 3 * E, 0, T * 3 * E, D), dqkv, c_off=E, ldc_m=3 * E, c_bso=T * 3 * E,
         c_bsi=D, **bh)
    return dqkv


def permute_rows(x, outer, A, Bd, Cc):
    out = empty(outer * A * Bd, Cc, device=x.device)
    L.check(L.load().svl_permute_rows_f32(_p(x), outer, A, Bd, Cc, _p(out), _st()), "svl_permute_rows_f32")
    return out


SEQATTN_MFMA_MIN = int(os.environ.get("SVL_SEQATTN_MFMA_MIN", "64"))


def seqattn_fwd(qkv, groups, inner, seq, heads, outer_stride, inner_stride, seq_stride):
    rows, E3 = qkv.shape
    E = E3 // 3
    out = empty(rows, E, device=qkv.device)
    probs = empty(groups, heads, seq, seq, device=qkv.device)
    d = L.SeqAttnDesc(groups, inner, seq, heads, outer_stride, inner_stride, seq_stride, _p(qkv), _p(out), _p(probs),
                      None, None, None)
    L.check(L.load().svl_seqattn_fwd(C.byref(d), _st()), "svl_seqattn_fwd")
    return out, probs


def seqattn_bwd(dout, qkv, probs, groups, inner, seq, heads, outer_stride, inner_stride, seq_stride):
    dqkv = torch.empty_like(qkv)
    ds = torch.empty_like(probs)
    d = L.SeqAttnDesc(groups, inner, seq, heads, outer_stride, inner_stride, seq_stride, _p(qkv), None, _p(probs),
                      _p(dout), _p(dqkv), _p(ds))
    L.check(L.load().svl_seqattn_bwd(C.byref(d), _st()), "svl_seqattn_bwd")
    return dqkv


_PACKS = {}


def cached_pack(W, tag, fn):
    base = W._base if W._base is not None else W
    if not isinstance(base, torch.nn.Parameter):
        return fn(W.detach())
    key = (W.data_ptr(), tuple(W.shape), tag)
    ver = (base._version, WEIGHT_EPOCH if base.requires_grad else 0)
    hit = _PACKS.get(key)
    if hit is not None and hit[0] == ver and hit[2]() is base:
        return hit[1].get()
    out = fn(W.detach())
    if len(_PACKS) > 4096:
        _PACKS.clear()
    _PACKS[key] = (ver, StreamCached(out), weakref.ref(base))
    return out


def conv3x3_weight_planes(pack, N, Ct):
    if not (pack.is_cuda and N in (32, 64, 128) and Ct % 16 == 0):
        return None
    lib = L.load()
    pl = torch.empty(lib.svl_conv3x3_weight_planes_bytes(N, Ct), dtype=torch.uint8, device=pack.device)
    L.check(lib.svl_conv3x3_weight_planes(_p(pack), N, Ct, _p(pl), _st()), "svl_conv3x3_weight_planes")
    return pl


def w_planes_of(pack):
    return getattr(pack, "_svl_planes", None)


def pack_conv_w(W):
    def build(w):
        Co, Ci, kh, kw = w.shape
        w = w.contiguous()
        cs = (Ci * kh * kw, kh * kw, kw, 1)
        wf = permute4(w, (Co, kh, kw, Ci), (cs[0], cs[2], cs[3], cs[1])).view(Co, kh * kw * Ci)
        wd = permute4(w, (Ci, kh, kw, Co), (cs[1], cs[2], cs[3], cs[0])).view(Ci, kh * kw * Co)
        out = [wf, wd]
        if kh == 3 and kw == 3:
            for pk, n, ct in ((wf, Co, Ci), (wd, Ci, Co)):
                pl = conv3x3_weight_planes(pk, n, ct)
                if pl is not None:
                    pk._svl_planes = pl
                    out.append(pl)
        return tuple(out)
    r = cached_pack(W, "conv", build)
    return r[0], r[1]


def unpack_conv_wgrad(dwf, Co, Ci, kh, kw):
    return permute4(dwf, (Co, Ci, kh, kw), (kh * kw * Ci, 1, kw * Ci, Ci))


CONV_TILED = not os.environ.get("SVL_CONV_NO_TILED")


def conv_out_size(H, W, KH, KW, dil, pad, stride):
    return (H + 2 * pad - dil * (KH - 1) - 1) // stride + 1, (W + 2 * pad - dil * (KW - 1) - 1) // stride + 1


def conv_fwd(x, ldx, imgs, H, W, C1, wf, Co, KH, KW, dil, pad, bias=None, act=ACT_NONE, out=None, ldo=None, src2=None,
             ld2=0, C2=0, rep=1, resid=None, ldr=None, stride=1):
    Ho, Wo = conv_out_size(H, W, KH, KW, dil, pad, stride) if stride != 1 else (H, W)
    M = imgs * Ho * Wo
    K = KH * KW * (C1 + C2)
    if out is None:
        out = empty(M, Co, device=x.device)
        ldo = Co
    g = conv_geom(H, W, C1, KH, KW, dil, pad, 1, C2, rep, src2, ld2, stride=stride, Ho=Ho, Wo=Wo)
    gemm(A_CONV, B_KC, M, Co, K, Op(x, ldx), Op(wf, K), out, ldc_m=ldo, bias=bias, act=act, conv=g, resid=resid,
         ldr_m=ldr, w_planes=w_planes_of(wf) if (KH, KW, pad, stride) == (3, 3, dil, 1) else None, emu_h2=EMU_H2_CONVFWD)
    return out


def conv_dgrad(dy, lddy, imgs, H, W, Co, wd, Ci, KH, KW, dil, pad, out=None, ldo=None, accumulate=False):
    M = imgs * H * W
    K = KH * KW * Co
    if out is None:
# ... 541 lines not shown
```

Baseline: 107.8 images/s.

## Write attention fp16x2 sets directly from the QKV projection GEMM epilogue

Adds an EPI_SETS epilogue to the planes GEMM. The QKV in_proj linear now writes the split fp16 x 2 attention operand sets, already in the attention kernel's packed row-major layout with per-head exponents. A new prepare kernel computes those exponents ahead of time from input row norms and per-slice weight/bias bounds. The attention forward then skips its own pack pass and the fp32 qkv tensor is never materialized, saving a full read and write of qkv. The cost is scale exponents taken from norm bounds rather than actual values, and the backward now receives a null qkv and relies on the sets.

```diff
diff --git a/include/semivl_hip.h b/include/semivl_hip.h
--- a/include/semivl_hip.h
+++ b/include/semivl_hip.h
@@ -131,6 +131,10 @@
   const float* a_rnorm;
   const float* b_bound;
   int32_t* p_sexp;
+  void* sets_out;
+  int sets_T, sets_H;
+  int sets_Tp;
+  const int32_t* sets_exps;
 } svl_pgemm_desc;
 int64_t svl_planes_rows(int64_t rows);
 int64_t svl_planes_bytes(int64_t rows, int K);
@@ -314,6 +318,10 @@
 int svl_attention_bwd_h2(const float* qkv, const float* out, const float* dout, const float* lse, int B, int T, int H,
                          float* dsum_ws, float* dqkv, void* dqkv_planes, int64_t planes_rows, void* ws, int64_t ws_bytes,
                          svl_stream_t stream);
+int svl_attn_slice_bounds_f32(const float* rnorm_w, const float* bias, int nslices, float* out4, svl_stream_t stream);
+int svl_attn_sets_prepare(const float* a_rnorm, const float* slice_bounds, int B, int T, int H, void* ws, int64_t ws_bytes,
+                          svl_stream_t stream);
+int svl_attention_fwd_h2_packed(int B, int T, int H, float* out, float* lse, void* ws, int64_t ws_bytes, svl_stream_t stream);
 
 typedef struct svl_seqattn_desc {
   int groups, inner, seq, heads;
diff --git a/semivl_amd/csrc/attention.hip b/semivl_amd/csrc/attention.hip
--- a/semivl_amd/csrc/attention.hip
+++ b/semivl_amd/csrc/attention.hip
@@ -619,11 +619,48 @@
   return r > 0 ? svl_join(st) : SVL_OK;
 }
 
+extern "C" int svl_attn_slice_bounds_f32(const float* rnorm_w, const float* bias, int nslices, float* out4, svl_stream_t stream) {
+  SVL_CHECK_ARG(rnorm_w && out4 && nslices > 0, "svl_attn_slice_bounds_f32: bad args");
+  return svl_attn_h2::slice_bounds(rnorm_w, bias, nslices, out4, (hipStream_t)stream);
+}
+
+extern "C" int svl_attn_sets_prepare(const float* a_rnorm, const float* slice_bounds, int B, int T, int H, void* ws,
+                                     int64_t ws_bytes, svl_stream_t stream) {
+  SVL_CHECK_ARG(a_rnorm && slice_bounds && B > 0 && T > 0 && H > 0 && (long)B * H <= 65535, "svl_attn_sets_prepare: bad args");
+  return svl_attn_h2::sets_prepare(a_rnorm, slice_bounds, B, T, H, ws, ws_bytes, svl_attn_h2::tr_sets(-1), (hipStream_t)stream);
+}
+
+extern "C" int svl_attention_fwd_h2_packed(int B, int T, int H, float* out, float* lse, void* ws, int64_t ws_bytes,
+                                           svl_stream_t stream) {
+  SVL_CHECK_ARG(B > 0 && T > 0 && H > 0 && (long)B * H <= 65535 && out, "svl_attention_fwd_h2_packed: bad args");
+  AttnP p;
+  memset(&p, 0, sizeof(p));
+  p.out = out; p.lse = lse; p.B = B; p.T = T; p.H = H; p.E = (long)H * D; p.ld = 3 * p.E; p.scale = 0.125f;
+  hipStream_t st = (hipStream_t)stream;
+  const int tr = svl_attn_h2::tr_sets(-1);
+  int rc = svl_attn_h2::fwd_packed_check(p, ws, ws_bytes, tr);
+  if (rc) return rc;
+  int nb = 0;
+  const int r = rows_split(T, &nb, FQ);
+  if (r > 0) {
+    hipStream_t aux = nullptr;
+    rc = svl_fork(st, &aux);
+    if (rc) return rc;
+    rc = svl_attn_h2::fwd_tail(p, nb * FQ, ws, tr, aux);
+    if (rc) return rc;
+  }
+  rc = svl_attn_h2::fwd(p, nb, ws, ws_bytes, tr, st);
+  if (rc) return rc;
+  return r > 0 ? svl_join(st) : SVL_OK;
+}
+
 namespace {
 int bwd_h2(const char* who, const float* qkv, const float* out, const float* dout, const float* lse, int B, int T, int H,
            float* dsum_ws, float* dqkv, void* dq_planes, const void* sets, int64_t sets_bytes, void* ws, int64_t ws_bytes,
            svl_stream_t stream) {
-  int rc = check(qkv, B, T, H, who);
+  int rc = SVL_OK;
+  if (sets && !qkv) SVL_CHECK_ARG(B > 0 && T > 0 && H > 0 && (long)B * H <= 65535, "%s: bad args", who);
+  else rc = check(qkv, B, T, H, who);
   if (rc) return rc;
   SVL_CHECK_ARG(out && dout && lse && dsum_ws && dqkv, "%s: null args", who);
   rc = no_planes(dq_planes, who);
diff --git a/semivl_amd/csrc/attn_h2.h b/semivl_amd/csrc/attn_h2.h
--- a/semivl_amd/csrc/attn_h2.h
+++ b/semivl_amd/csrc/attn_h2.h
@@ -12,5 +12,8 @@
 int fwd_pack(const AttnP& p, void* ws, long wsb, int tr, hipStream_t st);
 int fwd_tail(const AttnP& p, int row0, void* ws, int tr, hipStream_t aux);
 int bwd_tail(const AttnP& p, int row0, void* ws, const void* sets, int tr, hipStream_t aux);
+int slice_bounds(const float* rnorm_w, const float* bias, int nslices, float* out4, hipStream_t st);
+int sets_prepare(const float* a_rnorm, const float* slice_bounds, int B, int T, int H, void* ws, long wsb, int tr, hipStream_t st);
+int fwd_packed_check(const AttnP& p, const void* ws, long wsb, int tr);
 
 }
diff --git a/semivl_amd/csrc/attn_h2.hip b/semivl_amd/csrc/attn_h2.hip
--- a/semivl_amd/csrc/attn_h2.hip
+++ b/semivl_amd/csrc/attn_h2.hip
@@ -233,6 +233,62 @@
   if (p.exps_in && tid < 3) {
     p.exps[z * 4 + tid] = p.exps_in[z * 4 + tid];
     p.nrm[z * 4 + tid] = p.nrm_in[z * 4 + tid];
+  }
+}
+
+__global__ __launch_bounds__(64) void attn_slice_bounds_kernel(const float* __restrict__ rnorm_w, const float* __restrict__ bias,
+                                                               float* __restrict__ out4) {
+  const int s = blockIdx.x, l = threadIdx.x;
+  const float r = rnorm_w[s * 64 + l], bv = bias ? fabsf(bias[s * 64 + l]) : 0.f;
+  float mr = r, mb = bv;
+  double sr = (double)r * r, sb = (double)bv * bv;
+#pragma unroll
+  for (int o = 32; o > 0; o >>= 1) {
+    mr = fmaxf(mr, __shfl_xor(mr, o, 64));
+    mb = fmaxf(mb, __shfl_xor(mb, o, 64));
+    sr += __shfl_xor(sr, o, 64);
+    sb += __shfl_xor(sb, o, 64);
+  }
+  if (l == 0) {
+    out4[s * 4] = mr;
+    out4[s * 4 + 1] = mb;
+    out4[s * 4 + 2] = (float)(sqrt(sr) * (1.0 + 1e-6));
+    out4[s * 4 + 3] = (float)(sqrt(sb) * (1.0 + 1e-6));
+  }
+}
+
+__global__ __launch_bounds__(256) void attn_sets_prepare_kernel(const float* __restrict__ a_rnorm, const float* __restrict__ sb,
+                                                                char* __restrict__ ws, long set, int* __restrict__ exps,
+                                                                float* __restrict__ nrm, int T, int H, int Tp) {
+  __shared__ float red[4];
+  const int b = blockIdx.x, tid = threadIdx.x;
+  float a = 0.f;
+  for (int t = tid; t < T; t += 256) a = fmaxf(a, a_rnorm[(long)b * T + t]);
+  a = block_max_256(a, red);
+  for (int idx = tid; idx < 3 * H; idx += 256) {
+    const int w = idx / H, h = idx - w * H, z = b * H + h;
+    const float* s = sb + (long)idx * 4;
+    const double bound = (double)a * (double)s[0] + (double)s[1];
+    int e = 0;
+    if (bound > 0.0) {
+      (void)frexp(bound, &e);
+      e -= 15;
+    }
+    exps[z * 4 + w] = e < -100 ? -100 : (e > 100 ? 100 : e);
+    nrm[z * 4 + w] = (float)(((double)a * (double)s[2] + (double)s[3]) * (1.0 + 1e-6));
+    if (w == 0) {
+      exps[z * 4 + 3] = 0;
+      nrm[z * 4 + 3] = 0.f;
+    }
+  }
+  const int nz = Tp - T;
+  const long slice = (long)Tp * 256;
+  for (int idx = tid; idx < 3 * H * nz * 16; idx += 256) {
+    const int slot = idx & 15, r = idx >> 4, wh = r / nz, t = T + (r - wh * nz);
+    const int w = wh / H, h = wh - w * H;
+    const int kg = slot >> 2, pl = (slot >> 1) & 1, hh = slot & 1;
+    char* q = ws + w * set + (long)(b * H + h) * slice + (long)(((t >> 5) * 4 + kg) * 2 + pl) * 1024 + (hh * 32 + (t & 31)) * 16;
+    *reinterpret_cast<uint4*>(q) = make_uint4(0u, 0u, 0u, 0u);
   }
 }
 
@@ -1260,7 +1316,33 @@
   return SVL_OK;
 }
 
-#define SVL_LAUNCH_V(KERN, VV, LDS)                                   \
+int slice_bounds(const float* rnorm_w, const float* bias, int nslices, float* out4, hipStream_t st) {
+  hipLaunchKernelGGL(attn_slice_bounds_kernel, dim3(nslices), dim3(64), 0, st, rnorm_w, bias, out4);
+  SVL_LAUNCH_CHECK("svl_attn_slice_bounds_f32");
+  return SVL_OK;
+}
+
+int sets_prepare(const float* a_rnorm, const float* sb, int B, int T, int H, void* ws_, long wsb, int tr, hipStream_t st) {
+  SVL_CHECK_ARG(!tr, "svl_attn_sets_prepare: the GEMM writes row-major sets only (the tr switch is on)");
+  AttnP p;
+  memset(&p, 0, sizeof(p));
+  p.B = B; p.T = T; p.H = H;
+  int rc = check_ws(p, ws_, wsb, 0, 0, "svl_attn_sets_prepare");
+  if (rc) return rc;
+  const Layout l = layout(B, T, H, 0, 0);
+  char* ws = static_cast<char*>(ws_);
+  hipLaunchKernelGGL(attn_sets_prepare_kernel, dim3(B), dim3(256), 0, st, a_rnorm, sb, ws, l.set, reinterpret_cast<int*>(ws + l.exps),
+                     reinterpret_cast<float*>(ws + l.nrm), T, H, l.Tp);
+  SVL_LAUNCH_CHECK("svl_attn_sets_prepare");
+  return SVL_OK;
+}
+
+int fwd_packed_check(const AttnP& p, const void* ws, long wsb, int tr) {
+  SVL_CHECK_ARG(!tr, "svl_attention_fwd_h2_packed: supplied sets are row-major sets only (the tr switch is on)");
+  return check_ws(p, ws, wsb, 0, 0, "svl_attention_fwd_h2_packed");
+}
+
+#define SVL_LAUNCH_V(KERN, VV, LDS)                                 \
     rc = set_lds(KERN<VV>, mask, LDS);                                  \
     if (rc) return rc;                                                  \
     hipLaunchKernelGGL(KERN<VV>, grid, dim3(512), LDS, st, p, w);
@@ -1299,7 +1381,7 @@
   PackP q;
   memset(&q, 0, sizeof(q));
   for (int i = 0; i < 3; ++i) {
-    q.src[i] = p.qkv + i * p.E;
+    q.src[i] = p.qkv ? p.qkv + i * p.E : nullptr;
     q.ld[i] = p.ld;
   }
   q.src[3] = p.dout;
diff --git a/semivl_amd/csrc/gemm_planes.hip b/semivl_amd/csrc/gemm_planes.hip
--- a/semivl_amd/csrc/gemm_planes.hip
+++ b/semivl_amd/csrc/gemm_planes.hip
@@ -74,7 +74,18 @@
                     (d->m_off & 31) == 0 && (d->a_rows & 255) == 0 && (d->b_rows & 255) == 0 &&
                     d->a_rows >= d->m_off + d->M && d->b_rows >= d->N,
                 "svl_gemm_planes_f32: bad operands (K %% 16 == 0, m_off %% 32 == 0, plane buffers padded to 256 rows)");
-  SVL_CHECK_ARG(d->C || d->planes_out, "svl_gemm_planes_f32: no output");
+  SVL_CHECK_ARG(d->C || d->planes_out || d->sets_out, "svl_gemm_planes_f32: no output");
+  if (d->sets_out) {
+    const bool shape = d->sets_T > 0 && d->sets_H > 0 && d->M % d->sets_T == 0 && (int64_t)d->N == (int64_t)3 * d->sets_H * 64 &&
+                       d->sets_Tp == (d->sets_T + 63) / 64 * 64 && d->m_off == 0;
+    if (!(d->fmt == 1 && shape && d->sets_exps && !d->resid && !d->preact && !d->planes_out && !d->accumulate &&
+          d->act == SVL_ACT_NONE && ((uintptr_t)d->sets_out & 1023) == 0)) {
+      svl_set_error("svl_gemm_planes_f32: sets_out needs fmt = 1, m_off = 0, M %% sets_T == 0, N == 3 sets_H 64 (got M %d N %d T %d "
+                    "H %d Tp %d), sets_exps, act NONE and no resid / preact / planes_out / accumulate", d->M, d->N, d->sets_T,
+                    d->sets_H, d->sets_Tp);
+      return SVL_ERR_UNSUPPORTED;
+    }
+  }
   SVL_CHECK_ARG(!d->planes_out || ((d->N & 15) == 0 && (d->p_rows & 255) == 0 && d->p_rows >= d->m_off + d->M),
                 "svl_gemm_planes_f32: planes_out needs N %% 16 == 0 and p_rows (%% 256 == 0) >= rows");
   SVL_CHECK_ARG(d->act >= SVL_ACT_NONE && d->act <= SVL_ACT_MUL_DRELU, "svl_gemm_planes_f32: bad act");
@@ -106,5 +117,9 @@
   p.preact = d->preact ? d->preact + mo * d->ldc : nullptr;
   p.resid = d->resid ? d->resid + mo * d->ldr : nullptr; p.ldr = d->ldr;
   p.accumulate = d->accumulate;
+  p.S = (char*)d->sets_out;
+  p.s_exps = d->sets_exps;
+  p.s_T = d->sets_T; p.s_H = d->sets_H; p.s_Tp = d->sets_Tp;
+  p.s_set = d->sets_out ? (long)(d->M / d->sets_T) * d->sets_H * d->sets_Tp * 256 : 0;
   return np == 2 ? svl_planes_launch_h2(p, (hipStream_t)stream) : launch<3>(p, (hipStream_t)stream);
 }
diff --git a/semivl_amd/csrc/gemm_planes_impl.h b/semivl_amd/csrc/gemm_planes_impl.h
--- a/semivl_amd/csrc/gemm_planes_impl.h
+++ b/semivl_amd/csrc/gemm_planes_impl.h
@@ -30,6 +30,10 @@
   int tiles_n, full_m, tail_rows;
   int rcnt[8], fstart[8];
   int panel;
+  char* S;
+  long s_set;
+  const int* s_exps;
+  int s_T, s_H, s_Tp;
 #ifdef SVL_X6P_TIMING
   unsigned long long* dbg;
 #endif
@@ -128,7 +132,7 @@
   return t;
 }
 
-enum { EPI_LIGHT = 0, EPI_GELU = 1, EPI_DGELU = 2 };
+enum { EPI_LIGHT = 0, EPI_GELU = 1, EPI_DGELU = 2, EPI_SETS = 3 };
 
 template <int NP, int TM, int TN, int EPI>
 __device__ __forceinline__ void x6p_epilogue(const PlanesP& p, f32x16 (&acc)[TM][TN], int m0, int mvalid, int wm, int nw,
@@ -300,6 +304,27 @@
       float bound = p.a_rn[mw + i * 32 + l31] * bd0 + bd1;
       if constexpr (EPI == EPI_DGELU) bound *= 1.13f;
       eo[i] = scale_exp_of(bound);
+    });
+  }
+  constexpr bool SETS = EPI == EPI_SETS;
+  constexpr int NG = SETS ? TN * 2 : 1;
+  long s_off[SETS ? TM : 1];
+  int s_e[SETS ? TM : 1][NG];
+  if constexpr (SETS) {
+    const long slice = (long)p.s_Tp * 256;
+    const int E = p.s_H * 64;
+    static_for<0, TM>([&](auto I) {
+      constexpr int i = decltype(I)::value;
+      const bool ok = i * 32 + l31 < rows_w;
+      const int m = ok ? mw + i * 32 + l31 : 0;
+      const int b = m / p.s_T, t = m - b * p.s_T;
+      s_off[i] = ok ? (long)b * p.s_H * slice + (long)(t >> 5) * 8192 + (hi * 32 + (t & 31)) * 16 : -1;
+      static_for<0, NG>([&](auto G2) {
+        constexpr int c = decltype(G2)::value;
+        const int nb = nw + c * 16;
+        const int w = nb / E, h = (nb - w * E) >> 6;
+        s_e[i][c] = (ok && nb < p.N) ? p.s_exps[(b * p.s_H + h) * 4 + w] : 0;
+      });
     });
   }
   auto resid4 = [&](int i, int j, int g) __attribute__((always_inline)) {
@@ -426,6 +451,25 @@
           });
         });
       }
+      if constexpr (SETS) {
+        const int E = p.s_H * 64;
+        const long slice = (long)p.s_Tp * 256;
+        static_for<0, NG>([&](auto G2) {
+          constexpr int c = decltype(G2)::value;
+          const int nb = nw + c * 16;
+          if (nb < p.N && s_off[i] >= 0) {
+            const int w = nb / E, nh = nb - w * E;
+            float o8[8];
+#pragma unroll
+            for (int e = 0; e < 8; ++e) o8[e] = acc[i][c >> 1][8 * (c & 1) + e];
+            f16x8 h0, h1;
+            split2x8(o8, s_e[i][c], h0, h1);
+            char* q = p.S + (long)w * p.s_set + (long)(nh >> 6) * slice + s_off[i] + ((nh >> 4) & 3) * (2 * CH);
+            *reinterpret_cast<f16x8*>(q) = h0;
+            *reinterpret_cast<f16x8*>(q + CH) = h1;
+          }
+        });
+      }
     }
   });
 }
@@ -644,6 +688,11 @@
     q.fstart[x] = (int)fs;
     fs += blocks - rag;
   }
+  if (q.S) {
+    if constexpr (NP == 2 && EF) return launch_kernel<NP, BN, EPI_SETS, EF>(q, total, st);
+    svl_set_error("svl_gemm_planes_f32: sets_out needs fp16 x 2 operands and 16-byte aligned outputs");
+    return SVL_ERR_UNSUPPORTED;
+  }
   if (q.act == SVL_ACT_GELU) return launch_kernel<NP, BN, EPI_GELU, EF>(q, total, st);
   if (q.act == SVL_ACT_MUL_DGELU) return launch_kernel<NP, BN, EPI_DGELU, EF>(q, total, st);
   return launch_kernel<NP, BN, EPI_LIGHT, EF>(q, total, st);
diff --git a/semivl_amd/lib.py b/semivl_amd/lib.py
--- a/semivl_amd/lib.py
+++ b/semivl_amd/lib.py
@@ -45,7 +45,9 @@
                 ("bias", C.c_void_p), ("act", C.c_int), ("preact", C.c_void_p), ("resid", C.c_void_p),
                 ("ldr", C.c_int64), ("accumulate", C.c_int),
                 ("fmt", C.c_int), ("p_fmt", C.c_int), ("a_sexp", C.c_void_p), ("b_sexp", C.c_void_p),
-                ("a_rnorm", C.c_void_p), ("b_bound", C.c_void_p), ("p_sexp", C.c_void_p)]
+                ("a_rnorm", C.c_void_p), ("b_bound", C.c_void_p), ("p_sexp", C.c_void_p),
+                ("sets_out", C.c_void_p), ("sets_T", C.c_int), ("sets_H", C.c_int), ("sets_Tp", C.c_int),
+                ("sets_exps", C.c_void_p)]
 
 
 class CeDesc(C.Structure):
@@ -174,6 +176,9 @@
     "svl_attention_bwd_h2": (_I, [_P, _P, _P, _P, _I, _I, _I, _P, _P, _P, _L, _P, _L, _P]),
     "svl_attention_h2_tr_sets": (_I, [_I]),
     "svl_attention_bwd_h2_sets": (_I, [_P, _P, _P, _P, _I, _I, _I, _P, _P, _P, _L, _P, _L, _P]),
+    "svl_attn_slice_bounds_f32": (_I, [_P, _P, _I, _P, _P]),
+    "svl_attn_sets_prepare": (_I, [_P, _P, _I, _I, _I, _P, _L, _P]),
+    "svl_attention_fwd_h2_packed": (_I, [_I, _I, _I, _P, _P, _P, _L, _P]),
     "svl_conv_cout1_fwd": (_I, [_P, _L, _I, _I, _I, _I, _I, _I, _I, _I, _P, _P, _P, _P, _P]),
     "svl_conv_cout1_wgrad_blocks": (_I, [_I, _I, _I]),
     "svl_conv_cout1_wgrad": (_I, [_P, _P, _L, _I, _I, _I, _I, _I, _I, _P, _P, _P]),
diff --git a/semivl_amd/model/vit.py b/semivl_amd/model/vit.py
--- a/semivl_amd/model/vit.py
+++ b/semivl_amd/model/vit.py
@@ -112,6 +112,9 @@
     if skip_x:
         vproj = ops.linear(y1a, p["win"][2 * E:], p["bin"][2 * E:])
         qkv = None
+    elif pp and D == 64 and not want_v and ops.attn_epi_sets_ok():
+        qkv = ops.linear(y1a, p["win"], p["bin"], attn_sets=(Bn, T, heads))
+        vproj = None
     else:
         qkv = ops.linear(y1a, p["win"], p["bin"])
         vproj = qkv[:, 2 * E:]
diff --git a/semivl_amd/ops.py b/semivl_amd/ops.py
--- a/semivl_amd/ops.py
+++ b/semivl_amd/ops.py
@@ -424,8 +424,65 @@
 PLANES_PATH = not os.environ.get("SVL_GEMM_NO_PLANES")
 
 
+class AttnSets:
+    __slots__ = ("ws", "nbytes", "Bn", "T", "H", "shape", "device", "dtype")
+
+    def __init__(self, Bn, T, H, device):
+        self.Bn, self.T, self.H, self.device, self.dtype = Bn, T, H, device, torch.float32
+        self.shape = (Bn * T, 3 * H * 64)
+        self.ws, self.nbytes = _attn_ws(Bn, T, H, 0, device)
+
+    def exps_ptr(self):
+        return _ws_ptr(self.ws) + 3 * self.Bn * self.H * ((self.T + 63) // 64 * 64) * 256
+
+
+EPI_SETS_DEFAULT = True
+_EPI_SETS = [(EPI_SETS_DEFAULT or bool(os.environ.get("SVL_ATTN_EPI_SETS"))) and not os.environ.get("SVL_ATTN_NO_EPI_SETS")]
+
+
+def attn_epi_sets(on=None):
+    prev = _EPI_SETS[0]
+    if on is not None:
+        _EPI_SETS[0] = bool(on)
+    return prev
+
+
+def attn_epi_sets_ok():
+    return _EPI_SETS[0] and PLANES_FMT == "h2" and attention_planes_ok() and not attention_tr_sets()
+
+
+def _slice_bounds(B, bias):
+    key = ("slices", None if bias is None else (bias.data_ptr(), bias._version, WEIGHT_EPOCH if bias.requires_grad else 0),
+           torch.cuda.current_stream().cuda_stream)
+    if B._bd is None:
+        B._bd = {}
+    hit = B._bd.get(key)
+    if hit is not None:
+        return hit
+    assert B.rows % 64 == 0 and B.rnorm is not None
+    sb = torch.empty(B.rows // 64, 4, dtype=torch.float32, device=B.buf.device)
+    bflat = bias.detach().view(-1) if bias is not None else None
+    assert bflat is None or bflat.numel() == B.rows
+    L.check(L.load().svl_attn_slice_bounds_f32(_p(B.rnorm), _p(bflat), B.rows // 64, _p(sb), _st()), "svl_attn_slice_bounds_f32")
+    if len(B._bd) > 8:
+        B._bd.clear()
+    B._bd[key] = sb
+    return sb
+
+
+def linear_attn_sets(xa, wb, bias, Bn, T, H, out=None):
+    assert isinstance(xa, Planes) and xa.fmt == "h2" and xa.rnorm is not None and wb.fmt == "h2"
+    M, N = Bn * T, 3 * H * 64
+    assert xa.rows == M and wb.rows == N
+    s = AttnSets(Bn, T, H, xa.buf.device)
+    sb = _slice_bounds(wb, bias)
+    L.check(L.load().svl_attn_sets_prepare(_p(xa.rnorm), _p(sb), Bn, T, H, _ws_ptr(s.ws), s.nbytes, _st()), "svl_attn_sets_prepare")
+    pgemm(xa, wb, M, N, out, None, bias, sets=s)
+    return s
+
+
 def pgemm(A, B, M, N, out=None, planes_out=None, bias=None, act=ACT_NONE, preact=None, resid=None, accumulate=False,
-          m_off=0):
+          m_off=0, sets=None):
     K = A.K
     assert B.K == K and A.rows >= m_off + M and B.rows >= N and A.fmt == B.fmt
     d = L.PGemmDesc()
@@ -445,6 +502,8 @@
             assert A.fmt == "h2" and A.rnorm is not None
             keep = _out_bound(B, bias)
             d.p_fmt, d.a_rnorm, d.b_bound, d.p_sexp = 1, _p(A.rnorm), _p(keep), _p(planes_out.sexp)
+    if sets is not None:
+        d.sets_out, d.sets_T, d.sets_H, d.sets_Tp, d.sets_exps = _ws_ptr(sets.ws), sets.T, sets.H, (sets.T + 63) // 64 * 64, sets.exps_ptr()
     d.bias, d.act, d.preact = _p(bias), act, _p(preact)
     if resid is not None:
         assert resid.stride(1) == 1
@@ -460,10 +519,18 @@
     return Planes(M, N, device=xa.buf.device, fmt="h2" if h2 else "b3")
 
 
-def linear(x, W, bias=None, act=ACT_NONE, resid=None, out=None, accumulate=False, preact=None, planes_only=False):
+def linear(x, W, bias=None, act=ACT_NONE, resid=None, out=None, accumulate=False, preact=None, planes_only=False,
+           attn_sets=None):
     M, K = x.shape
     N = W.shape[0]
     assert W.shape[1] == K and W.stride(1) == 1
+    if attn_sets is not None:
+        if not (attn_epi_sets_ok() and isinstance(x, Planes) and x.fmt == "h2" and x.rnorm is not None):
+            raise RuntimeError("linear(attn_sets=): needs attn_epi_sets_ok() and an fp16 x 2 Planes input with row norms")
+        assert act == ACT_NONE and resid is None and out is None and preact is None and not accumulate
+        Bn, T, H = attn_sets
+        assert M == Bn * T and N == 3 * H * 64
+        return linear_attn_sets(x, weight_planes(W, fmt="h2"), bias, Bn, T, H)
     if isinstance(x, Planes) or planes_eligible(M, N, K):
         xa = x if isinstance(x, Planes) else split_planes(x)
         wb = weight_planes(W, fmt=xa.fmt)
@@ -964,7 +1031,15 @@
     lse = empty(Bn * H * T, device=qkv.device) if want_lse else None
     e0 = _prof_begin()
     sets = None
-    if attention_h2():
+    if isinstance(qkv, AttnSets):
+        assert (qkv.Bn, qkv.T, qkv.H) == (Bn, T, H)
+        if not attention_h2() or attention_tr_sets():
+            raise RuntimeError("attention_fwd: AttnSets operands need the fp16 x 2 attention on row-major sets")
+        L.check(L.load().svl_attention_fwd_h2_packed(Bn, T, H, _p(out), _p(lse), _ws_ptr(qkv.ws), qkv.nbytes, _st()),
+                "svl_attention_fwd_h2_packed")
+        if keep_sets:
+            sets = qkv.ws
+    elif attention_h2():
         ws, n = _attn_ws(Bn, T, H, 0, qkv.device)
         L.check(L.load().svl_attention_fwd_h2(_p(qkv), Bn, T, H, _p(out), _p(lse), None, 0, _ws_ptr(ws), n, _st()),
                 "svl_attention_fwd_h2")
@@ -982,16 +1057,21 @@
 def attention_bwd(dout, qkv, out, lse, Bn, T, H, planes=False, sets=None):
     if planes and not attention_planes_ok():
         raise RuntimeError("attention_bwd: planes outputs need emulation mode 6 (attention_planes_ok())")
-    dqkv = torch.empty_like(qkv)
-    ws = empty(Bn * H * T, device=qkv.device)
+    if isinstance(qkv, AttnSets):
+        if not attention_h2() or attention_tr_sets():
+            raise RuntimeError("attention_bwd: AttnSets operands need the fp16 x 2 attention on row-major sets")
+        dqkv, sets, qkv = empty(*qkv.shape, device=qkv.device), qkv.ws, None
+    else:
+        dqkv = torch.empty_like(qkv)
+    ws = empty(Bn * H * T, device=dqkv.device)
     e0 = _prof_begin()
     if attention_h2() and sets is not None and not attention_tr_sets():
-        wsb, n = _attn_ws(Bn, T, H, 2, qkv.device)
+        wsb, n = _attn_ws(Bn, T, H, 2, dqkv.device)
         L.check(L.load().svl_attention_bwd_h2_sets(_p(qkv), _p(out), _p(dout), _p(lse), Bn, T, H, _p(ws), _p(dqkv), _ws_ptr(sets),
                                                    sets.numel() - (_ws_ptr(sets) - sets.data_ptr()), _ws_ptr(wsb), n, _st()),
                 "svl_attention_bwd_h2_sets")
     elif attention_h2():
-        wsb, n = _attn_ws(Bn, T, H, 1, qkv.device)
+        wsb, n = _attn_ws(Bn, T, H, 1, dqkv.device)
         L.check(L.load().svl_attention_bwd_h2(_p(qkv), _p(out), _p(dout), _p(lse), Bn, T, H, _p(ws), _p(dqkv), None, 0,
                                               _ws_ptr(wsb), n, _st()), "svl_attention_bwd_h2")
     else:
```

New measurement: 108.6 images/s (median of 6 runs). Within noise of the previous version (+0.8%).
